# gnlpfjh/Scalable-E3-GNN

Hardware: AMD Instinct MI355X
Metric: particles/sec (octree build + SEGNN fwd), 1M pts l_max=2, 1/2/4/8 MI355X (higher is better)
Workload: dtype f32; 1 GPU; 1000000 particles/GPU uniform in unit box, radius graph k~24 (E=23519616), SEGNN l_max=2 4 layers H=32 f32 storage; particles_per_gpu=1000000, edges_per_gpu=23519616, hidden=32, layers=4, lmax=2, parallelism=single GPU

## Files before the change

include/e3gnn.h:

```cpp
#ifndef E3GNN_H
#define E3GNN_H

#include <stdint.h>

#ifdef __cplusplus
extern "C" {
#endif

#define E3GNN_ABI_VERSION 3

enum {
  E3_OK = 0,
  E3_ERR_INVALID_ARG = 1,
  E3_ERR_BAD_IRREPS = 2,
  E3_ERR_MISSING_WEIGHT = 3,
  E3_ERR_UNSUPPORTED = 4,
  E3_ERR_HIP = 5,
  E3_ERR_NO_DEVICE = 6
};

enum { E3_F32 = 0, E3_F64 = 1, E3_BF16 = 2 };

enum { E3_CLS_0E = 0, E3_CLS_0O = 1, E3_CLS_1E = 2, E3_CLS_1O = 3 };

typedef struct e3_l1tp_plan e3_l1tp_plan;

int         e3_abi_version(void);
const char* e3_status_string(int status);
const char* e3_last_hip_error(void);

int e3_l1tp_plan_create(const int32_t* in1_blocks, int n_in1,
                        const int32_t* out_blocks, int n_out,
                        e3_l1tp_plan** plan);
int e3_l1tp_plan_destroy(e3_l1tp_plan* plan);

int e3_l1tp_in1_dim(const e3_l1tp_plan* plan);
int e3_l1tp_out_dim(const e3_l1tp_plan* plan);
int e3_l1tp_weight_shape(const e3_l1tp_plan* plan, int cls, int* rows, int* cols);
int e3_l1tp_norm_len(const e3_l1tp_plan* plan, int cls);

int64_t e3_l1tp_packed_bytes(const e3_l1tp_plan* plan, int dtype);
int e3_l1tp_pack_weights(const e3_l1tp_plan* plan,
                         const void* const weights[4], const void* const norms[4],
                         int dtype, void* packed, void* stream);

int e3_l1tp_forward(const e3_l1tp_plan* plan,
                    const void* in1, int64_t ld_in1,
                    const void* in2, int64_t ld_in2,
                    const void* packed,
                    void* out, int64_t ld_out,
                    int64_t B, int dtype, int kernel, void* stream);

int64_t e3_l1tp_backward_workspace_bytes(const e3_l1tp_plan* plan, int64_t B, int dtype);
int e3_l1tp_backward(const e3_l1tp_plan* plan,
                     const void* in1, int64_t ld_in1,
                     const void* in2, int64_t ld_in2,
                     const void* const weights[4], const void* const norms[4],
                     const void* grad_out, int64_t ld_gout,
                     void* grad_in1, int64_t ld_gin1,
                     void* grad_in2,
                     void* const grad_weights[4],
                     void* workspace,
                     int64_t B, int dtype, void* stream);

typedef struct e3_rg_params {
  float lo[3], hi[3];
  float r;
  int32_t n[3];
  float inv[3];
  int32_t bits;
} e3_rg_params;

int     e3_rg_grid(e3_rg_params* prm);
int64_t e3_rg_workspace_bytes(int64_t N, const e3_rg_params* prm);
int e3_rg_sort_count(const float* pos, int64_t N, const e3_rg_params* prm,
                     int32_t* perm, float* sorted_pos4, int32_t* rowptr,
                     void* workspace, int64_t workspace_bytes, void* stream);
int e3_rg_fill(int64_t N, const e3_rg_params* prm, const float* sorted_pos4, const int32_t* rowptr,
               int32_t* src, void* workspace, int64_t workspace_bytes, void* stream);

int e3_rg_sort_count_pbc(const float* pos, int64_t N, const e3_rg_params* prm, int32_t periodic,
                         int32_t* perm, float* sorted_pos4, int32_t* rowptr,
                         void* workspace, int64_t workspace_bytes, void* stream);
int e3_rg_fill_pbc(int64_t N, const e3_rg_params* prm, int32_t periodic, const float* sorted_pos4,
                   const int32_t* rowptr, int32_t* src, void* workspace, int64_t workspace_bytes, void* stream);

int e3_cell_derive(const float cell[9], float ginv[9], float heights[3], float* volume);
int e3_rg_sort_count_cell(const float* pos, int64_t N, const e3_rg_params* prm, const float cell[9], const float origin[3],
                          int32_t* perm, float* sorted_pos4, int32_t* rowptr,
                          void* workspace, int64_t workspace_bytes, void* stream);
int e3_rg_fill_cell(int64_t N, const e3_rg_params* prm, const float cell[9], const float origin[3],
                    const float* sorted_pos4, const int32_t* rowptr, int32_t* src,
                    void* workspace, int64_t workspace_bytes, void* stream);

int e3_edge_geometry(const float* pos4, const int32_t* rowptr, const int32_t* src, int64_t N,
                     float* edge_y, float* edge_d, float* node_a, void* stream);
int e3_edge_geometry_pbc(const float* pos4, const int32_t* rowptr, const int32_t* src, int64_t N, const float box[3],
                         float* edge_y, float* edge_d, float* node_a, void* stream);
int e3_edge_geometry_cell(const float* pos4, const int32_t* rowptr, const int32_t* src, int64_t N, const float cell[9],
                          float* edge_y, float* edge_d, float* node_a, void* stream);
int e3_gather_concat(const float* h, int64_t ld_h, int D, const int32_t* rowptr, const int32_t* src, int64_t N,
                     const float* extra, int n_extra, float* out, int64_t ld_out, void* stream);
int e3_gate(const float* in, int64_t ld_in, float* out, int64_t ld_out, int64_t B, int ns, int nv, void* stream);
int e3_segment_sum(const float* msg, int64_t ld_msg, const int32_t* rowptr, int64_t N, int D,
                   float* agg, int64_t ld_agg, void* stream);

int64_t e3_split_edges_workspace_bytes(int64_t N);
int e3_split_edges(const int32_t* rowptr, const int32_t* src, const uint8_t* is_ghost, int64_t N, int64_t E,
                   int32_t* rowptr_kept, int32_t* src_kept, int32_t* dst_kept, int32_t* src_interior, int32_t* dst_interior,
                   int32_t* src_boundary, int32_t* dst_boundary, int32_t* counts, void* workspace, void* stream);

#define E3_HALO_MAX_ENTRIES 26
typedef struct e3_halo_entry {
  float lo[3], hi[3], shift[3];
} e3_halo_entry;
int64_t e3_halo_select_workspace_bytes(int64_t n, int n_entries);
int e3_halo_select_count(const float* pos, int64_t n, const float lo[3], const float hi[3], int32_t periodic, float r,
                         const e3_halo_entry* entries, int n_entries, float* pos_wrapped, int32_t* counts, void* workspace,
                         int64_t workspace_bytes, void* stream);
int e3_halo_select_fill(const float* pos_wrapped, int64_t n, const float lo[3], const float hi[3], int32_t periodic, float r,
                        const e3_halo_entry* entries, int n_entries, int64_t total, int32_t* idx, float* ghost_pos,
                        void* workspace, int64_t workspace_bytes, void* stream);

#define E3_MORTON_MAX_RANKS 64
int e3_morton_keys(const float* pos, int64_t n, const float lo[3], const float hi[3], const int32_t n_cells[3], int32_t* keys,
                   void* stream);
int64_t e3_morton_select_workspace_bytes(int64_t n, int n_ranks);
int e3_morton_select_count(const float* pos, int64_t n, const float lo[3], const float hi[3], const int32_t n_cells[3], float r,
                           const int32_t* splitters, int n_ranks, int self_rank, int32_t* counts, void* workspace,
                           int64_t workspace_bytes, void* stream);
int e3_morton_select_fill(const float* pos, int64_t n, const float lo[3], const float hi[3], const int32_t n_cells[3], float r,
                          const int32_t* splitters, int n_ranks, int self_rank, int64_t total, int32_t* idx, void* workspace,
                          int64_t workspace_bytes, void* stream);

typedef struct e3_tp_plan e3_tp_plan;
typedef struct e3_tp_segment {
  const void* base;
  int64_t ld;
  const int32_t* row_index;
  int32_t ncols;
  int32_t reserved;
} e3_tp_segment;
int e3_tp_plan_create(const int32_t* in1_blocks, int n_in1, int lmax_sh,
                      const int32_t* out_blocks, int n_out, e3_tp_plan** plan);
int e3_tp_plan_destroy(e3_tp_plan* plan);
int e3_tp_in1_dim(const e3_tp_plan* plan);
int e3_tp_in2_dim(const e3_tp_plan* plan);
int e3_tp_out_dim(const e3_tp_plan* plan);
int e3_tp_weight_shape(const e3_tp_plan* plan, int cls, int* rows, int* cols);
int e3_tp_norm_len(const e3_tp_plan* plan, int cls);
int64_t e3_tp_packed_bytes(const e3_tp_plan* plan, int dtype);
int e3_tp_pack_weights(const e3_tp_plan* plan, const void* const weights[6], const void* const norms[6],
                       int dtype, void* packed, void* stream);
int e3_tp_forward(const e3_tp_plan* plan, const void* in1, int64_t ld_in1, const void* in2, int64_t ld_in2,
                  const void* packed, void* out, int64_t ld_out, int64_t B, int dtype, const float* in_scale,
                  int exact, void* stream);
int e3_pow2_scale(const e3_tp_segment* segs, const int64_t* nrows, int nseg, int target_log2, float* out4,
                  void* stream);
int e3_add_pow2_scale(const float* h, const float* u, float* out, int64_t n, int target_log2, float* out4,
                      void* stream);
int e3_tp_forward_fused(const e3_tp_plan* plan, const e3_tp_segment* segs, int nseg,
                        const void* in2, int64_t ld_in2, const void* packed, void* out, int64_t ld_out,
                        int64_t B, int dtype, int gate, const float* in_scale, void* stream);
int e3_tp_forward_fused_epilogue(const e3_tp_plan* plan, const e3_tp_segment* segs, int nseg, const void* in2,
                                 int64_t ld_in2, const void* packed, void* out, int64_t ld_out, int64_t B, int dtype,
                                 int gate, const float* in_scale, const void* residual, int64_t ld_residual,
                                 float* out_scale4, int target_log2, void* stream);
int e3_tp_forward_update_pair(const e3_tp_plan* plan1, const e3_tp_plan* plan2, const e3_tp_segment* segs, int nseg,
                              const void* in2, int64_t ld_in2, const void* packed1, const void* packed2,
                              const float* in_scale, const void* residual, int64_t ld_residual, void* out,
                              int64_t ld_out, int64_t B, int dtype, float* out_scale4, int target_log2, void* stream);
int e3_tp_backward(const e3_tp_plan* plan, const void* in1, int64_t ld_in1, const void* in2, int64_t ld_in2,
                   const void* packed, const void* grad_out, int64_t ld_gout, void* grad_in1, int64_t ld_gin1,
                   void* grad_in2, int64_t ld_gin2, void* const grad_weights[6], int64_t B, int dtype, void* stream);
int e3_tp_backward_weights(const e3_tp_plan* plan, const void* in1, int64_t ld_in1, const void* in2, int64_t ld_in2,
                           const void* packed, const void* grad_out, int64_t ld_gout, void* const grad_weights[6],
                           int64_t B, int dtype, void* stream);
int e3_tp_backward_operands(const e3_tp_plan* plan, const void* in1, int64_t ld_in1, const void* in2, int64_t ld_in2,
                            const void* packed, const void* grad_out, int64_t ld_gout, void* const features[6],
                            void* const gout[6], int64_t B, int dtype, void* stream);
int e3_tp_backward_contract(const e3_tp_plan* plan, const void* in1, int64_t ld_in1, const void* in2, int64_t ld_in2,
                            void* const t[6], void* grad_in1, int64_t ld_gin1, void* grad_in2, int64_t ld_gin2,
                            int64_t B, int dtype, void* stream);
int e3_tp_fused_supported(const e3_tp_plan* plan, int gate);
const char* e3_tp_last_fused_kernel(void);
int e3_tp_forward_fused_scatter(const e3_tp_plan* plan, const e3_tp_segment* segs, int nseg,
                                const void* in2, int64_t ld_in2, const void* packed, const int32_t* row_node,
                                void* out_nodes, int64_t ld_out, int64_t B, int dtype, int gate,
                                const float* in_scale, void* stream);
typedef struct e3_msg_plan e3_msg_plan;
int e3_msg_plan_create(int lmax, int hidden, e3_msg_plan** plan);
int e3_msg_plan_destroy(e3_msg_plan* plan);
int64_t e3_msg_packed_bytes(const e3_msg_plan* plan);
int64_t e3_msg_premix_floats_per_node(const e3_msg_plan* plan);
int e3_msg_weight_shape(const e3_msg_plan* plan, int tp , int l3, int* rows, int* cols);
int e3_msg_supports(const e3_msg_plan* plan, int dtype);
int e3_msg_pack_weights(e3_msg_plan* plan, const void* const w1[3], const void* const n1[3],
                        const void* const w2[3], const void* const n2[3], int dtype, void* packed, void* stream);
int e3_msg_premix(e3_msg_plan* plan, const void* h, int64_t ld_h, int64_t N, const void* packed,
                  const float* in_scale, float* premix, int dtype, void* stream);
int e3_msg_forward(e3_msg_plan* plan, const void* h, int64_t ld_h, int64_t N, const float* pos4,
                   const int32_t* src, const int32_t* dst, int64_t E, const void* packed, const float* in_scale,
                   const float* premix, float* out, int64_t ld_out, int dtype, int accumulate, int tiles_per_block,
                   void* stream);
int e3_msg_forward_pbc(e3_msg_plan* plan, const void* h, int64_t ld_h, int64_t N, const float* pos4,
                       const int32_t* src, const int32_t* dst, int64_t E, const void* packed, const float* in_scale,
                       const float* premix, float* out, int64_t ld_out, int dtype, int accumulate, int tiles_per_block,
                       const float box[3], void* stream);
int e3_msg_forward_cell(e3_msg_plan* plan, const void* h, int64_t ld_h, int64_t N, const float* pos4,
                        const int32_t* src, const int32_t* dst, int64_t E, const void* packed, const float* in_scale,
                        const float* premix, float* out, int64_t ld_out, int dtype, int accumulate, int tiles_per_block,
                        const float cell[9], void* stream);
int e3_segment_sum_bf16(const void* msg, int64_t ld_msg, const int32_t* rowptr, int64_t N, int D,
                        void* agg, int64_t ld_agg, void* stream);
int e3_edge_geometry_l2(const float* pos4, const int32_t* rowptr, const int32_t* src, int64_t N,
                        float* edge_y, float* edge_d, float* node_a, void* stream);
int e3_edge_geometry_l2_pbc(const float* pos4, const int32_t* rowptr, const int32_t* src, int64_t N, const float box[3],
                            float* edge_y, float* edge_d, float* node_a, void* stream);
int e3_edge_geometry_l2_cell(const float* pos4, const int32_t* rowptr, const int32_t* src, int64_t N, const float cell[9],
                             float* edge_y, float* edge_d, float* node_a, void* stream);
int e3_gate_blocks(const float* in, int64_t ld_in, float* out, int64_t ld_out, int64_t B, int ns,
                   int nblocks, const int32_t* ls, const int32_t* muls, void* stream);

int e3_edge_geometry_backward(const float* pos4, const int32_t* rowptr, const int32_t* src, int64_t N, int lmax,
                              const float* g_edge_y, const float* g_edge_d, const float* g_node_a, float* g_pos,
                              void* stream);
int e3_edge_geometry_backward_pbc(const float* pos4, const int32_t* rowptr, const int32_t* src, int64_t N, int lmax,
                                  const float box[3], const float* g_edge_y, const float* g_edge_d,
                                  const float* g_node_a, float* g_pos, void* stream);
int e3_edge_geometry_backward_cell(const float* pos4, const int32_t* rowptr, const int32_t* src, int64_t N, int lmax,
                                   const float cell[9], const float* g_edge_y, const float* g_edge_d,
                                   const float* g_node_a, float* g_pos, void* stream);
int e3_gather_concat_backward(const float* g_out, int64_t ld_gout, int D, const int32_t* rowptr, const int32_t* src,
                              int64_t N, int n_extra, float* g_h, int64_t ld_gh, float* g_extra, void* stream);

int e3_edge_geometry_strained(const float* pos4, const int32_t* rowptr, const int32_t* src, int64_t N, int lmax,
                              const float* box, const float* strain, const int32_t* structure, int S, float* edge_y,
                              float* edge_d, float* node_a, void* stream);
int64_t e3_edge_geometry_backward_strained_workspace_bytes(int64_t N);
int e3_edge_geometry_backward_strained(const float* pos4, const int32_t* rowptr, const int32_t* src, int64_t N, int lmax,
                                       const float* box, const float* strain, const int32_t* structure, int S,
                                       const float* g_edge_y, const float* g_edge_d, const float* g_node_a, float* g_pos,
                                       float* g_strain, void* workspace, int64_t workspace_bytes, void* stream);
int e3_edge_geometry_strained_cell(const float* pos4, const int32_t* rowptr, const int32_t* src, int64_t N, int lmax,
                                   const float cell[9], const float* strain, const int32_t* structure, int S,
                                   float* edge_y, float* edge_d, float* node_a, void* stream);
int e3_edge_geometry_backward_strained_cell(const float* pos4, const int32_t* rowptr, const int32_t* src, int64_t N,
                                            int lmax, const float cell[9], const float* strain, const int32_t* structure,
                                            int S, const float* g_edge_y, const float* g_edge_d, const float* g_node_a,
                                            float* g_pos, float* g_strain, void* workspace, int64_t workspace_bytes,
                                            void* stream);
int e3_gate_blocks_backward(const float* in, int64_t ld_in, const float* g_out, int64_t ld_gout, float* g_in,
                            int64_t ld_gin, int64_t B, int ns, int nblocks, const int32_t* ls, const int32_t* muls,
                            void* stream);
int e3_segment_sum_backward(const float* g_agg, int64_t ld_gagg, const int32_t* rowptr, int64_t N, int D, float* g_msg,
                            int64_t ld_gmsg, void* stream);

int e3_cutoff_envelope(const float* edge_d, int64_t E, float r_c, int p, float* w, void* stream);
int e3_cutoff_envelope_backward(const float* edge_d, const float* g_w, int64_t E, float r_c, int p, float* g_d,
                                void* stream);
int e3_segment_sum_weighted(const float* msg, int64_t ld_msg, const float* w, const int32_t* rowptr, int64_t N, int D,
                            float* agg, int64_t ld_agg, void* stream);
int e3_segment_sum_weighted_backward(const float* g_agg, int64_t ld_gagg, const float* msg, int64_t ld_msg, const float* w,
                                     const int32_t* rowptr, int64_t N, int D, float* g_msg, int64_t ld_gmsg, float* g_w,
                                     void* stream);

int64_t e3_nl_workspace_bytes(int64_t N);
int e3_nl_update(const float* pos, const int32_t* perm, const float* ref_pos4, const int32_t* rowptr, const int32_t* src,
                 int64_t N, int64_t E, float r, float* pos4_out, int32_t* rowptr_out, int32_t* src_out, int32_t* dst_out,
                 uint32_t* stats, void* workspace, void* stream);
int e3_nl_update_pbc(const float* pos, const int32_t* perm, const float* ref_pos4, const int32_t* rowptr, const int32_t* src,
                     int64_t N, int64_t E, float r, const float box[3], float* pos4_out, int32_t* rowptr_out,
                     int32_t* src_out, int32_t* dst_out, uint32_t* stats, void* workspace, void* stream);
int e3_nl_update_cell(const float* pos, const int32_t* perm, const float* ref_pos4, const int32_t* rowptr, const int32_t* src,
                      int64_t N, int64_t E, float r, const float cell[9], float* pos4_out, int32_t* rowptr_out,
                      int32_t* src_out, int32_t* dst_out, uint32_t* stats, void* workspace, void* stream);

#ifdef __cplusplus
}
#endif
#endif
```

scalable-e3-gnn_amd/_lib.py:

```python
from __future__ import annotations

import ctypes
import os
from ctypes import POINTER, c_char_p, c_int, c_int32, c_int64, c_void_p

_HERE = os.path.dirname(os.path.abspath(__file__))
LIB_PATH = os.path.join(_HERE, "lib", "libe3gnn_hip.so")

E3_OK = 0
E3_F32, E3_F64, E3_BF16 = 0, 1, 2
CLS_NAMES = ("l0e", "l0o", "l1e", "l1o")

_lib = None

VoidP4 = c_void_p * 4
Float3 = ctypes.c_float * 3
Float9 = ctypes.c_float * 9
Int3 = c_int32 * 3


class HaloEntry(ctypes.Structure):
    _fields_ = [("lo", ctypes.c_float * 3), ("hi", ctypes.c_float * 3), ("shift", ctypes.c_float * 3)]


SIGNATURES = {
    "e3_abi_version": (c_int, []),
    "e3_status_string": (c_char_p, [c_int]),
    "e3_last_hip_error": (c_char_p, []),
    "e3_l1tp_plan_create": (c_int, [POINTER(c_int32), c_int, POINTER(c_int32), c_int, POINTER(c_void_p)]),
    "e3_l1tp_plan_destroy": (c_int, [c_void_p]),
    "e3_l1tp_in1_dim": (c_int, [c_void_p]),
    "e3_l1tp_out_dim": (c_int, [c_void_p]),
    "e3_l1tp_weight_shape": (c_int, [c_void_p, c_int, POINTER(c_int), POINTER(c_int)]),
    "e3_l1tp_norm_len": (c_int, [c_void_p, c_int]),
    "e3_l1tp_packed_bytes": (c_int64, [c_void_p, c_int]),
    "e3_l1tp_pack_weights": (c_int, [c_void_p, VoidP4, VoidP4, c_int, c_void_p, c_void_p]),
    "e3_l1tp_forward": (c_int, [c_void_p, c_void_p, c_int64, c_void_p, c_int64, c_void_p, c_void_p, c_int64,
                                c_int64, c_int, c_int, c_void_p]),
    "e3_l1tp_backward_workspace_bytes": (c_int64, [c_void_p, c_int64, c_int]),
    "e3_rg_grid": (c_int, [c_void_p]),
    "e3_rg_workspace_bytes": (c_int64, [c_int64, c_void_p]),
    "e3_rg_sort_count": (c_int, [c_void_p, c_int64, c_void_p, c_void_p, c_void_p, c_void_p, c_void_p, c_int64,
                                 c_void_p]),
    "e3_rg_fill": (c_int, [c_int64, c_void_p, c_void_p, c_void_p, c_void_p, c_void_p, c_int64, c_void_p]),
    "e3_edge_geometry": (c_int, [c_void_p, c_void_p, c_void_p, c_int64, c_void_p, c_void_p, c_void_p, c_void_p]),
    "e3_gather_concat": (c_int, [c_void_p, c_int64, c_int, c_void_p, c_void_p, c_int64, c_void_p, c_int, c_void_p,
                                 c_int64, c_void_p]),
    "e3_gate": (c_int, [c_void_p, c_int64, c_void_p, c_int64, c_int64, c_int, c_int, c_void_p]),
    "e3_segment_sum": (c_int, [c_void_p, c_int64, c_void_p, c_int64, c_int, c_void_p, c_int64, c_void_p]),
    "e3_split_edges_workspace_bytes": (c_int64, [c_int64]),
    "e3_split_edges": (c_int, [c_void_p, c_void_p, c_void_p, c_int64, c_int64, c_void_p, c_void_p, c_void_p, c_void_p,
                               c_void_p, c_void_p, c_void_p, c_void_p, c_void_p, c_void_p]),
    "e3_halo_select_workspace_bytes": (c_int64, [c_int64, c_int]),
    "e3_halo_select_count": (c_int, [c_void_p, c_int64, Float3, Float3, c_int32, ctypes.c_float, c_void_p, c_int, c_void_p,
                                     c_void_p, c_void_p, c_int64, c_void_p]),
    "e3_halo_select_fill": (c_int, [c_void_p, c_int64, Float3, Float3, c_int32, ctypes.c_float, c_void_p, c_int, c_int64,
                                    c_void_p, c_void_p, c_void_p, c_int64, c_void_p]),
    "e3_morton_keys": (c_int, [c_void_p, c_int64, Float3, Float3, Int3, c_void_p, c_void_p]),
    "e3_morton_select_workspace_bytes": (c_int64, [c_int64, c_int]),
    "e3_morton_select_count": (c_int, [c_void_p, c_int64, Float3, Float3, Int3, ctypes.c_float, POINTER(c_int32), c_int,
                                       c_int, c_void_p, c_void_p, c_int64, c_void_p]),
    "e3_morton_select_fill": (c_int, [c_void_p, c_int64, Float3, Float3, Int3, ctypes.c_float, POINTER(c_int32), c_int,
                                      c_int, c_int64, c_void_p, c_void_p, c_int64, c_void_p]),
    "e3_tp_plan_create": (c_int, [POINTER(c_int32), c_int, c_int, POINTER(c_int32), c_int, POINTER(c_void_p)]),
    "e3_tp_plan_destroy": (c_int, [c_void_p]),
    "e3_tp_in1_dim": (c_int, [c_void_p]),
    "e3_tp_in2_dim": (c_int, [c_void_p]),
    "e3_tp_out_dim": (c_int, [c_void_p]),
    "e3_tp_weight_shape": (c_int, [c_void_p, c_int, POINTER(c_int), POINTER(c_int)]),
    "e3_tp_norm_len": (c_int, [c_void_p, c_int]),
    "e3_tp_packed_bytes": (c_int64, [c_void_p, c_int]),
    "e3_tp_pack_weights": (c_int, [c_void_p, c_void_p * 6, c_void_p * 6, c_int, c_void_p, c_void_p]),
    "e3_tp_forward": (c_int, [c_void_p, c_void_p, c_int64, c_void_p, c_int64, c_void_p, c_void_p, c_int64, c_int64,
                              c_int, c_void_p, c_int, c_void_p]),
    "e3_tp_forward_fused": (c_int, [c_void_p, c_void_p, c_int, c_void_p, c_int64, c_void_p, c_void_p, c_int64, c_int64,
                                    c_int, c_int, c_void_p, c_void_p]),
    "e3_msg_plan_create": (c_int, [c_int, c_int, POINTER(c_void_p)]),
    "e3_msg_plan_destroy": (c_int, [c_void_p]),
    "e3_msg_packed_bytes": (c_int64, [c_void_p]),
    "e3_msg_premix_floats_per_node": (c_int64, [c_void_p]),
    "e3_msg_weight_shape": (c_int, [c_void_p, c_int, c_int, POINTER(c_int), POINTER(c_int)]),
    "e3_msg_supports": (c_int, [c_void_p, c_int]),
    "e3_msg_pack_weights": (c_int, [c_void_p, c_void_p * 3, c_void_p * 3, c_void_p * 3, c_void_p * 3, c_int, c_void_p,
                                    c_void_p]),
    "e3_msg_premix": (c_int, [c_void_p, c_void_p, c_int64, c_int64, c_void_p, c_void_p, c_void_p, c_int, c_void_p]),
    "e3_msg_forward": (c_int, [c_void_p, c_void_p, c_int64, c_int64, c_void_p, c_void_p, c_void_p, c_int64, c_void_p,
                               c_void_p, c_void_p, c_void_p, c_int64, c_int, c_int, c_int, c_void_p]),
    "e3_edge_geometry_backward": (c_int, [c_void_p, c_void_p, c_void_p, c_int64, c_int, c_void_p, c_void_p, c_void_p,
                                          c_void_p, c_void_p]),
    "e3_rg_sort_count_pbc": (c_int, [c_void_p, c_int64, c_void_p, c_int32, c_void_p, c_void_p, c_void_p, c_void_p,
                                     c_int64, c_void_p]),
    "e3_rg_fill_pbc": (c_int, [c_int64, c_void_p, c_int32, c_void_p, c_void_p, c_void_p, c_void_p, c_int64, c_void_p]),
    "e3_edge_geometry_pbc": (c_int, [c_void_p, c_void_p, c_void_p, c_int64, Float3, c_void_p, c_void_p, c_void_p,
                                     c_void_p]),
    "e3_edge_geometry_l2_pbc": (c_int, [c_void_p, c_void_p, c_void_p, c_int64, Float3, c_void_p, c_void_p, c_void_p,
                                        c_void_p]),
    "e3_edge_geometry_backward_pbc": (c_int, [c_void_p, c_void_p, c_void_p, c_int64, c_int, Float3, c_void_p, c_void_p,
                                              c_void_p, c_void_p, c_void_p]),
    "e3_msg_forward_pbc": (c_int, [c_void_p, c_void_p, c_int64, c_int64, c_void_p, c_void_p, c_void_p, c_int64,
                                   c_void_p, c_void_p, c_void_p, c_void_p, c_int64, c_int, c_int, c_int, Float3,
                                   c_void_p]),
    "e3_cell_derive": (c_int, [Float9, Float9, Float3, POINTER(ctypes.c_float)]),
    "e3_rg_sort_count_cell": (c_int, [c_void_p, c_int64, c_void_p, Float9, Float3, c_void_p, c_void_p, c_void_p, c_void_p,
                                      c_int64, c_void_p]),
    "e3_rg_fill_cell": (c_int, [c_int64, c_void_p, Float9, Float3, c_void_p, c_void_p, c_void_p, c_void_p, c_int64,
                                c_void_p]),
    "e3_edge_geometry_cell": (c_int, [c_void_p, c_void_p, c_void_p, c_int64, Float9, c_void_p, c_void_p, c_void_p,
                                      c_void_p]),
    "e3_edge_geometry_l2_cell": (c_int, [c_void_p, c_void_p, c_void_p, c_int64, Float9, c_void_p, c_void_p, c_void_p,
                                         c_void_p]),
    "e3_edge_geometry_backward_cell": (c_int, [c_void_p, c_void_p, c_void_p, c_int64, c_int, Float9, c_void_p, c_void_p,
                                               c_void_p, c_void_p, c_void_p]),
    "e3_msg_forward_cell": (c_int, [c_void_p, c_void_p, c_int64, c_int64, c_void_p, c_void_p, c_void_p, c_int64,
                                    c_void_p, c_void_p, c_void_p, c_void_p, c_int64, c_int, c_int, c_int, Float9,
                                    c_void_p]),
    "e3_edge_geometry_strained_cell": (c_int, [c_void_p, c_void_p, c_void_p, c_int64, c_int, Float9, c_void_p, c_void_p,
                                               c_int, c_void_p, c_void_p, c_void_p, c_void_p]),
    "e3_edge_geometry_backward_strained_cell": (c_int, [c_void_p, c_void_p, c_void_p, c_int64, c_int, Float9, c_void_p,
                                                        c_void_p, c_int, c_void_p, c_void_p, c_void_p, c_void_p, c_void_p,
                                                        c_void_p, c_int64, c_void_p]),
    "e3_gather_concat_backward": (c_int, [c_void_p, c_int64, c_int, c_void_p, c_void_p, c_int64, c_int, c_void_p, c_int64,
                                          c_void_p, c_void_p]),
    "e3_gate_blocks_backward": (c_int, [c_void_p, c_int64, c_void_p, c_int64, c_void_p, c_int64, c_int64, c_int, c_int,
                                        POINTER(c_int32), POINTER(c_int32), c_void_p]),
    "e3_segment_sum_backward": (c_int, [c_void_p, c_int64, c_void_p, c_int64, c_int, c_void_p, c_int64, c_void_p]),
    "e3_pow2_scale": (c_int, [c_void_p, POINTER(c_int64), c_int, c_int, c_void_p, c_void_p]),
    "e3_add_pow2_scale": (c_int, [c_void_p, c_void_p, c_void_p, c_int64, c_int, c_void_p, c_void_p]),
    "e3_tp_backward": (c_int, [c_void_p, c_void_p, c_int64, c_void_p, c_int64, c_void_p, c_void_p, c_int64, c_void_p,
                               c_int64, c_void_p, c_int64, c_void_p * 6, c_int64, c_int, c_void_p]),
    "e3_tp_backward_weights": (c_int, [c_void_p, c_void_p, c_int64, c_void_p, c_int64, c_void_p, c_void_p, c_int64, c_void_p,
                                       c_int64, c_int, c_void_p]),
    "e3_tp_backward_operands": (c_int, [c_void_p, c_void_p, c_int64, c_void_p, c_int64, c_void_p, c_void_p, c_int64, c_void_p,
                                        c_void_p, c_int64, c_int, c_void_p]),
    "e3_tp_backward_contract": (c_int, [c_void_p, c_void_p, c_int64, c_void_p, c_int64, c_void_p, c_void_p, c_int64, c_void_p,
                                        c_int64, c_int64, c_int, c_void_p]),
    "e3_tp_forward_fused_epilogue": (c_int, [c_void_p, c_void_p, c_int, c_void_p, c_int64, c_void_p, c_void_p, c_int64,
                                             c_int64, c_int, c_int, c_void_p, c_void_p, c_int64, c_void_p, c_int, c_void_p]),
    "e3_tp_forward_update_pair": (c_int, [c_void_p, c_void_p, c_void_p, c_int, c_void_p, c_int64, c_void_p, c_void_p,
                                          c_void_p, c_void_p, c_int64, c_void_p, c_int64, c_int64, c_int, c_void_p, c_int,
                                          c_void_p]),
    "e3_tp_fused_supported": (c_int, [c_void_p, c_int]),
    "e3_tp_last_fused_kernel": (ctypes.c_char_p, []),
    "e3_tp_forward_fused_scatter": (c_int, [c_void_p, c_void_p, c_int, c_void_p, c_int64, c_void_p, c_void_p, c_void_p,
                                            c_int64, c_int64, c_int, c_int, c_void_p, c_void_p]),
    "e3_segment_sum_bf16": (c_int, [c_void_p, c_int64, c_void_p, c_int64, c_int, c_void_p, c_int64, c_void_p]),
    "e3_edge_geometry_l2": (c_int, [c_void_p, c_void_p, c_void_p, c_int64, c_void_p, c_void_p, c_void_p, c_void_p]),
    "e3_gate_blocks": (c_int, [c_void_p, c_int64, c_void_p, c_int64, c_int64, c_int, c_int, POINTER(c_int32),
                               POINTER(c_int32), c_void_p]),
    "e3_l1tp_backward": (c_int, [c_void_p, c_void_p, c_int64, c_void_p, c_int64, VoidP4, VoidP4, c_void_p, c_int64,
                                 c_void_p, c_int64, c_void_p, VoidP4, c_void_p, c_int64, c_int, c_void_p]),
    "e3_edge_geometry_strained": (c_int, [c_void_p, c_void_p, c_void_p, c_int64, c_int, POINTER(ctypes.c_float), c_void_p,
                                          c_void_p, c_int, c_void_p, c_void_p, c_void_p, c_void_p]),
    "e3_edge_geometry_backward_strained_workspace_bytes": (c_int64, [c_int64]),
    "e3_edge_geometry_backward_strained": (c_int, [c_void_p, c_void_p, c_void_p, c_int64, c_int, POINTER(ctypes.c_float),
                                                   c_void_p, c_void_p, c_int, c_void_p, c_void_p, c_void_p, c_void_p,
                                                   c_void_p, c_void_p, c_int64, c_void_p]),
    "e3_cutoff_envelope": (c_int, [c_void_p, c_int64, ctypes.c_float, c_int, c_void_p, c_void_p]),
    "e3_cutoff_envelope_backward": (c_int, [c_void_p, c_void_p, c_int64, ctypes.c_float, c_int, c_void_p, c_void_p]),
    "e3_segment_sum_weighted": (c_int, [c_void_p, c_int64, c_void_p, c_void_p, c_int64, c_int, c_void_p, c_int64,
                                        c_void_p]),
    "e3_segment_sum_weighted_backward": (c_int, [c_void_p, c_int64, c_void_p, c_int64, c_void_p, c_void_p, c_int64, c_int,
                                                 c_void_p, c_int64, c_void_p, c_void_p]),
    "e3_nl_workspace_bytes": (c_int64, [c_int64]),
    "e3_nl_update": (c_int, [c_void_p, c_void_p, c_void_p, c_void_p, c_void_p, c_int64, c_int64, ctypes.c_float, c_void_p,
                             c_void_p, c_void_p, c_void_p, c_void_p, c_void_p, c_void_p]),
    "e3_nl_update_pbc": (c_int, [c_void_p, c_void_p, c_void_p, c_void_p, c_void_p, c_int64, c_int64, ctypes.c_float, Float3,
                                 c_void_p, c_void_p, c_void_p, c_void_p, c_void_p, c_void_p, c_void_p]),
    "e3_nl_update_cell": (c_int, [c_void_p, c_void_p, c_void_p, c_void_p, c_void_p, c_int64, c_int64, ctypes.c_float, Float9,
                                  c_void_p, c_void_p, c_void_p, c_void_p, c_void_p, c_void_p, c_void_p]),
}


def load():
    global _lib
    if _lib is not None:
        return _lib
    if not os.path.exists(LIB_PATH):
        raise RuntimeError(
            f"{LIB_PATH} is missing: the HIP library has not been built. Run "
            "`python -c 'import __graft_entry__ as g; g.build()'` (or `make -C scalable-e3-gnn_amd/csrc`). "
            "There is no CPU fallback.")
    import torch

    lib = ctypes.CDLL(LIB_PATH)
    for name, (res, args) in SIGNATURES.items():
        fn = getattr(lib, name, None)
        if fn is None:
            continue
        fn.restype = res
        fn.argtypes = args
    _lib = lib
    return lib


def check(status: int, what: str = ""):
    if status != E3_OK:
        lib = load()
        msg = lib.e3_status_string(status).decode()
        if status == 5:
            msg += " — " + lib.e3_last_hip_error().decode()
        raise RuntimeError(f"libe3gnn_hip: {what}: {msg} (status {status})")


def blocks_array(blocks):
    flat = [int(v) for b in blocks for v in b]
    return (c_int32 * len(flat))(*flat), len(blocks)


def ptr4(tensors):
    return VoidP4(*[(t.data_ptr() if (t is not None and t.numel() > 0) else None) for t in tensors])


def dtype_code(dtype) -> int:
    import torch

    try:
        return {torch.float32: E3_F32, torch.float64: E3_F64, torch.bfloat16: E3_BF16}[dtype]
    except KeyError:
        raise RuntimeError(f"libe3gnn_hip supports float32 / float64 / bfloat16, got {dtype}") from None


class DevicePlans:

    def __init__(self, create_name: str, destroy_name: str, *args):
        self._create, self._destroy_name, self._args = create_name, destroy_name, args
        self._handles = {}

    def _make(self):
        lib = load()
        cargs = []
        for a in self._args:
            if isinstance(a, (list, tuple)):
                arr, n = blocks_array(a)
                cargs += [arr, n]
            else:
                cargs.append(int(a))
        h = c_void_p()
        check(getattr(lib, self._create)(*cargs, ctypes.byref(h)), self._create)
        return h

    def handle(self, device=None) -> c_void_p:
        key = -1
        if device is not None:
            import torch
            key = torch.device(device).index
            if key is None:
                key = torch.cuda.current_device()
        h = self._handles.get(key)
        if h is None:
            h = self._handles[key] = self._make()
        return h

    def __deepcopy__(self, memo):
        return DevicePlans(self._create, self._destroy_name, *self._args)

    def __reduce__(self):
        return (DevicePlans, (self._create, self._destroy_name) + tuple(self._args))

    def __del__(self):
        try:
            lib = load()
            for h in self._handles.values():
                if h:
                    getattr(lib, self._destroy_name)(h)
            self._handles = {}
        except Exception:
            pass
```

scalable-e3-gnn_amd/csrc/e3_msg_common.h:

```cpp
#pragma once

template <int LMAX, int TT>
struct MsgGeom {
  static constexpr int H = 16 * TT;
  static constexpr int KS = (H + 31) / 32;
  static constexpr int D = H * (LMAX + 1) * (LMAX + 1);
  static constexpr int T(int l3) { return l3 == 0 ? TT * (1 + LMAX) : TT; }
  static constexpr int col0(int l) { return H * l * l; }
  static constexpr bool ok(int l1, int l2, int l3) {
    return l1 >= 0 && l2 >= 0 && l3 >= 0 && l1 <= LMAX && l2 <= LMAX && l3 <= LMAX && ((l1 + l2 + l3) % 2 == 0) &&
           l3 >= (l1 > l2 ? l1 - l2 : l2 - l1) && l3 <= l1 + l2;
  }
  static constexpr int blk(int l1, int l2, int l3) {
    int n = 0;
    for (int a = 0; a <= LMAX; ++a)
      for (int c = 0; c <= LMAX; ++c)
        for (int b = 0; b <= LMAX; ++b) {
          if (a == l1 && b == l2 && c == l3) return n;
          if (ok(a, b, c)) n += KS * T(c);
        }
    return n;
  }
  static constexpr int nblk() { return blk(LMAX + 1, 0, 0); }
  static constexpr int uoff(int l1, int l2, int l3) {
    int n = 0;
    for (int a = 0; a <= LMAX; ++a)
      for (int c = 0; c <= LMAX; ++c)
        for (int b = 0; b <= LMAX; ++b) {
          if (a == l1 && b == l2 && c == l3) return n;
          if (ok(a, b, c)) n += (2 * a + 1) * T(c) * 16;
        }
    return n;
  }
  static constexpr int UD = uoff(LMAX + 1, 0, 0);
  static constexpr int slot0(int l3) { return l3 == 0 ? 0 : l3 == 1 ? T(0) : T(0) + 3 * TT; }
  static constexpr int NS = T(0) + 3 * TT + (LMAX == 2 ? 5 * TT : 0);
  static constexpr int wdoff(int l) { return l == 0 ? 0 : l == 1 ? T(0) * 16 : (T(0) + TT) * 16; }
  static constexpr int WD = (T(0) + LMAX * TT) * 16;
  static constexpr int o_norm1 = 64, o_norm2 = o_norm1 + NS * 16, o_wd = o_norm2 + NS * 16;
  static constexpr int o_w = (o_wd + WD + 63) / 64 * 64;
  static constexpr int blk_floats = 64 * 8;
  static constexpr int64_t total_floats = (int64_t)o_w + 3LL * nblk() * blk_floats;
  static constexpr int lds_tab = 2 * NS * 16 + WD;
  static constexpr int lds_wave = 16 * (D + 4);
};

__host__ __device__ constexpr int kperm(int g, int jj) { return 16 * (jj >> 2) + 4 * g + (jj & 3); }


template <int L1, int L2, int L3>
__device__ __forceinline__ void make_z(const float (&y)[9], float (&z)[2 * L1 + 1][2 * L3 + 1]) {
  using C = CG<L1, L2, L3>;
#pragma unroll
  for (int a = 0; a < 2 * L1 + 1; ++a)
#pragma unroll
    for (int c = 0; c < 2 * L3 + 1; ++c) {
      float s = 0.f;
      bool have = false;
#pragma unroll
      for (int b = 0; b < 2 * L2 + 1; ++b)
        if (C::v[a][b][c] != 0.0) {
          s = have ? __builtin_fmaf((float)C::v[a][b][c], y[L2 * L2 + b], s) : (float)C::v[a][b][c] * y[L2 * L2 + b];
          have = true;
        }
      z[a][c] = s;
    }
}
template <int L1, int L2, int L3>
__host__ __device__ constexpr bool z_nonzero(int a, int c) {
  for (int b = 0; b < 2 * L2 + 1; ++b)
    if (CG<L1, L2, L3>::v[a][b][c] != 0.0) return true;
  return false;
}

template <bool IO16>
__device__ __forceinline__ f32x4 mma3(const uint4 ah, const uint4 al, const uint4 bh, const uint4 bl, f32x4 c) {
  if constexpr (IO16) {
    return mfma16(__builtin_bit_cast(bf16x8, ah), __builtin_bit_cast(bf16x8, bh), c);
  } else {
    c = mfma16h(__builtin_bit_cast(f16x8, ah), __builtin_bit_cast(f16x8, bh), c);
    c = mfma16h(__builtin_bit_cast(f16x8, ah), __builtin_bit_cast(f16x8, bl), c);
    c = mfma16h(__builtin_bit_cast(f16x8, al), __builtin_bit_cast(f16x8, bh), c);
    return c;
  }
}

template <bool IO16>
__device__ __forceinline__ void split8(const float (&f)[8], uint4& bh, uint4& bl) {
  uint32_t ph[4], pl[4] = {0, 0, 0, 0};
#pragma unroll
  for (int q = 0; q < 4; ++q) {
    if constexpr (IO16) ph[q] = __builtin_bit_cast(uint32_t, __builtin_convertvector(f32x2_t{f[2 * q], f[2 * q + 1]}, bf16x2_t));
    else split2_f16(f[2 * q], f[2 * q + 1], ph[q], pl[q]);
  }
  bh = uint4{ph[0], ph[1], ph[2], ph[3]};
  bl = uint4{pl[0], pl[1], pl[2], pl[3]};
}

template <int PBC = kOpen>
__device__ __forceinline__ void edge_sh(const float4 ps, const float4 pd, float (&y)[9], float& dist,
                                        const typename PbcArg<PBC>::type& box = {}) {
  float rx, ry, rz;
  edge_rel<PBC>(ps, pd, box, rx, ry, rz);
  const float d = sqrtf(rx * rx + ry * ry + rz * rz);
  const float inv = d > 0.f ? 1.0f / d : 0.f;
  const float x = rx * inv, yy = ry * inv, z = rz * inv;
  constexpr float s3 = 1.7320508075688772f, s5 = 2.2360679774997896f;
  y[0] = 1.0f;
  y[1] = s3 * x; y[2] = s3 * yy; y[3] = s3 * z;
  y[4] = s5 * s3 * x * yy;
  y[5] = s5 * s3 * yy * z;
  y[6] = s5 * 0.5f * (2.f * z * z - x * x - yy * yy);
  y[7] = s5 * s3 * z * x;
  y[8] = s5 * 0.5f * s3 * (x * x - yy * yy);
  dist = d;
}
template <int PBC = kOpen>
__device__ __forceinline__ void edge_sh1(const float4 ps, const float4 pd, float (&y)[9], float& dist,
                                        const typename PbcArg<PBC>::type& box = {}) {
  float rx, ry, rz;
  edge_rel<PBC>(ps, pd, box, rx, ry, rz);
  const float d = sqrtf(rx * rx + ry * ry + rz * rz);
  const float s = d > 0.f ? 1.7320508075688772f / d : 0.f;
  y[0] = 1.0f; y[1] = s * rx; y[2] = s * ry; y[3] = s * rz;
#pragma unroll
  for (int q = 4; q < 9; ++q) y[q] = 0.f;
  dist = d;
}

template <int D1, bool IO16>
__device__ __forceinline__ void read_piece(const void* piece, const int p, const float xs, float (&x)[8][D1]) {
  float q[4 * D1];
  if constexpr (IO16) {
    const uint2* sp = reinterpret_cast<const uint2*>(piece);
#pragma unroll
    for (int u = 0; u < D1; ++u) {
      const uint2 v = sp[u];
      q[4 * u + 0] = __builtin_bit_cast(float, v.x << 16); q[4 * u + 1] = __builtin_bit_cast(float, v.x & 0xffff0000u);
      q[4 * u + 2] = __builtin_bit_cast(float, v.y << 16); q[4 * u + 3] = __builtin_bit_cast(float, v.y & 0xffff0000u);
    }
  } else {
    const float4* sp = reinterpret_cast<const float4*>(piece);
#pragma unroll
    for (int u = 0; u < D1; ++u) {
      const float4 v = sp[u];
      q[4 * u] = v.x * xs; q[4 * u + 1] = v.y * xs; q[4 * u + 2] = v.z * xs; q[4 * u + 3] = v.w * xs;
    }
  }
#pragma unroll
  for (int r = 0; r < 4; ++r)
#pragma unroll
    for (int a = 0; a < D1; ++a) x[4 * p + r][a] = q[r * D1 + a];
}
template <int D1>
__device__ __forceinline__ void zero_piece(const int p, float (&x)[8][D1]) {
#pragma unroll
  for (int r = 0; r < 4; ++r)
#pragma unroll
    for (int a = 0; a < D1; ++a) x[4 * p + r][a] = 0.f;
}
```

scalable-e3-gnn_amd/csrc/e3_msg_fused.hip:

```cpp
#include "e3_common.h"
#include "cg_tables.h"
#include "e3_msg_ws.h"

#include <algorithm>
#include <cstddef>
#include <mutex>
#include <type_traits>
#include <utility>
#include <vector>

#ifndef E3_MSG_WD
#define E3_MSG_WD 1
#endif
#ifndef E3_MSG_UDP
#define E3_MSG_UDP 1
#endif
#ifndef E3_MSG_WPS
#define E3_MSG_WPS 2
#endif

#ifndef E3_MSG_STAMP
#define E3_MSG_STAMP 0
#endif

namespace e3 {
#if E3_MSG_STAMP
__device__ unsigned long long g_msg_stamps[8];
#endif

#include "e3_tp_mfma_core.h"

#include "e3_msg_common.h"

struct MsgPackDesc {
  int role;
  int mat;
  int rowbase;
  int nvalid;
  int M, colbase;
  int blk;
};
struct MsgPackArgs {
  const void* w1[3];
  const void* w2[3];
  const void* n1[3];
  const void* n2[3];
  int64_t nw1[3], nw2[3];
  int rowd[3];
  int M0, H, LMAX, TT, NS, WD, o_norm1, o_norm2, o_wd, o_w, nblk;
};

__global__ void msg_absmax_kernel(MsgPackArgs a, uint32_t* hdr) {
  float m1 = 0.f, m2 = 0.f;
  for (int c = 0; c < 3; ++c) {
    for (int64_t i = blockIdx.x * (int64_t)blockDim.x + threadIdx.x; i < a.nw1[c]; i += (int64_t)gridDim.x * blockDim.x)
      m1 = fmax_finite(m1, static_cast<const float*>(a.w1[c])[i]);
    for (int64_t i = blockIdx.x * (int64_t)blockDim.x + threadIdx.x; i < a.nw2[c]; i += (int64_t)gridDim.x * blockDim.x)
      m2 = fmax_finite(m2, static_cast<const float*>(a.w2[c])[i]);
  }
  for (int o = 32; o > 0; o >>= 1) { m1 = fmaxf(m1, __shfl_xor(m1, o)); m2 = fmaxf(m2, __shfl_xor(m2, o)); }
  if ((threadIdx.x & 63) == 0) {
    if (m1 > 0.f) atomicMax(hdr + 0, __builtin_bit_cast(uint32_t, m1));
    if (m2 > 0.f) atomicMax(hdr + 3, __builtin_bit_cast(uint32_t, m2));
  }
}

template <typename T>
__global__ void msg_pack_kernel(MsgPackArgs a, const MsgPackDesc* desc, int ndesc, float* packed) {
  constexpr bool IO16 = std::is_same<T, bf16>::value;
  const uint32_t* hb = reinterpret_cast<const uint32_t*>(packed);
  const float sw1 = IO16 ? 1.0f : pow2_scale_from_bits(hb[0], 13), sw2 = IO16 ? 1.0f : pow2_scale_from_bits(hb[3], 13);
  auto rd = [](const void* p, int64_t i) { return to_acc(static_cast<const T*>(p)[i]); };
  for (int r = blockIdx.x; r < ndesc; r += gridDim.x) {
    const MsgPackDesc q = desc[r];
    const void* W = q.role == 1 ? a.w2[q.mat] : a.w1[q.mat];
    const float sw = q.role == 1 ? sw2 : sw1;
    uint16_t* dst = reinterpret_cast<uint16_t*>(packed + a.o_w + ((size_t)q.role * a.nblk + q.blk) * 512);
    for (int i = threadIdx.x; i < 512; i += blockDim.x) {
      const int lane = i >> 3, jj = i & 7, ch = lane & 15, g = lane >> 4;
      const int k = kperm(g, jj);
      float v = 0.f;
      if (k < q.nvalid && q.colbase + ch < q.M) v = rd(W, (int64_t)(q.rowbase + k) * q.M + q.colbase + ch) * sw;
      if constexpr (IO16) {
        dst[lane * 8 + jj] = __builtin_bit_cast(uint16_t, (__bf16)v);
        dst[512 + lane * 8 + jj] = 0;
      } else {
        const _Float16 hi = (_Float16)v;
        const _Float16 lo = (_Float16)(v - (float)hi);
        dst[lane * 8 + jj] = __builtin_bit_cast(uint16_t, hi);
        dst[512 + lane * 8 + jj] = __builtin_bit_cast(uint16_t, lo);
      }
    }
  }
  if (blockIdx.x == 0) {
    for (int i = threadIdx.x; i < a.NS * 16; i += blockDim.x) {
      const int s = i >> 4, ch = i & 15;
      const int T0 = a.TT * (1 + a.LMAX);
      int l3, t, c;
      if (s < T0) { l3 = 0; t = s; c = 0; }
      else if (s < T0 + 3 * a.TT) { l3 = 1; t = (s - T0) / 3; c = (s - T0) % 3; }
      else { l3 = 2; t = (s - T0 - 3 * a.TT) / 5; c = (s - T0 - 3 * a.TT) % 5; }
      const int idx = (16 * t + ch) * (2 * l3 + 1) + c;
      packed[a.o_norm1 + i] = (a.n1[l3] ? rd(a.n1[l3], idx) : 1.0f) / sw1;
      packed[a.o_norm2 + i] = (a.n2[l3] ? rd(a.n2[l3], idx) : 1.0f) / sw2;
    }
    for (int i = threadIdx.x; i < a.WD; i += blockDim.x) {
      const int T0 = a.TT * (1 + a.LMAX);
      int l, rem;
      if (i < T0 * 16) { l = 0; rem = i; }
      else if (i < (T0 + a.TT) * 16) { l = 1; rem = i - T0 * 16; }
      else { l = 2; rem = i - (T0 + a.TT) * 16; }
      const int M = l == 0 ? a.M0 : a.H;
      packed[a.o_wd + i] = rd(a.w1[l], (int64_t)a.rowd[l] * M + rem) * sw1;
    }
    if (threadIdx.x == 0) {
      packed[1] = sw1; packed[2] = 1.0f / sw1;
      packed[4] = sw2; packed[5] = 1.0f / sw2;
    }
    __shared__ uint32_t red[2];
    float bw = 0.f;
    for (int l = 0; l <= a.LMAX; ++l) {
      const int M = l == 0 ? a.M0 : a.H;
      const int rows = (int)(a.nw1[l] / M);
      if (threadIdx.x < 2) red[threadIdx.x] = 0u;
      __syncthreads();
      float cs = 0.f, nm = 0.f;
      for (int col = threadIdx.x; col < M; col += blockDim.x) {
        float sum = 0.f;
        for (int r = 0; r < rows; ++r) sum += fabsf(rd(a.w1[l], (int64_t)r * M + col));
        cs = fmaxf(cs, sum);
      }
      for (int i = threadIdx.x; i < M * (2 * l + 1); i += blockDim.x) nm = fmaxf(nm, a.n1[l] ? fabsf(rd(a.n1[l], i)) : 1.0f);
      if (cs > 0.f && cs < INFINITY) atomicMax(&red[0], __builtin_bit_cast(uint32_t, cs));
      if (nm > 0.f && nm < INFINITY) atomicMax(&red[1], __builtin_bit_cast(uint32_t, nm));
      __syncthreads();
      bw = fmaxf(bw, 5.0f * __builtin_bit_cast(float, red[0]) * __builtin_bit_cast(float, red[1]));
      __syncthreads();
    }
    if (threadIdx.x == 0) packed[6] = bw;
  }
}


typedef uint32_t u32x4 __attribute__((ext_vector_type(4)));
struct TpCtx {
  __amdgpu_buffer_rsrc_t w;
  uint32_t wrole;
  uint32_t woff;
  const float* ud;
  const float* wd;
  float dsc;
};

template <bool IO16>
__device__ __forceinline__ void load_w(const TpCtx& cx, const int blk, uint4& hi, uint4& lo) {
  const uint32_t so = cx.wrole + (uint32_t)blk * 2048u;
  const u32x4 h = __builtin_amdgcn_raw_buffer_load_b128(cx.w, cx.woff, so, 0);
  hi = uint4{h[0], h[1], h[2], h[3]};
  if constexpr (!IO16) {
    const u32x4 l = __builtin_amdgcn_raw_buffer_load_b128(cx.w, cx.woff + 1024u, so, 0);
    lo = uint4{l[0], l[1], l[2], l[3]};
  }
}

struct BlkDesc {
  int l1, l2, l3, t;
  bool ff;
  bool first_of_l1;
  bool first_of_path;
};
template <int LMAX, int TT>
struct BlkList {
  using G = MsgGeom<LMAX, TT>;
  static constexpr BlkDesc at(int idx) {
    int n = 0;
    for (int l1 = 0; l1 <= LMAX; ++l1) {
      bool first = true;
      for (int pass = 0; pass < 2; ++pass)
        for (int l3 = 0; l3 <= LMAX; ++l3)
          for (int l2 = 0; l2 <= LMAX; ++l2) {
            if (!G::ok(l1, l2, l3)) continue;
            const bool ff = l3 == 0 && l1 > 0;
            if (ff != (pass == 0)) continue;
            for (int t = 0; t < G::T(l3); ++t) {
              if (n == idx) return BlkDesc{l1, l2, l3, t, ff, first, t == 0};
              first = false;
              ++n;
            }
          }
    }
    return BlkDesc{-1, 0, 0, 0, false, false, false};
  }
  static constexpr int count() {
    int n = 0;
    while (at(n).l1 >= 0) ++n;
    return n;
  }
};

template <int KS>
struct TpState {
  uint4 xh[KS][5], xl[KS][5];
  uint4 fh[KS], fl[KS];
  float z[5][5];
  uint4 wh[E3_MSG_WD + 1][KS], wl[E3_MSG_WD + 1][KS];
  f32x4 uin[E3_MSG_UDP + 1][5];
};

template <int LMAX, int TT, bool IO16, int IDX>
__device__ __forceinline__ void tp_prefetch_w(const TpCtx& cx, uint4 (&wh)[MsgGeom<LMAX, TT>::KS],
                                              uint4 (&wl)[MsgGeom<LMAX, TT>::KS]) {
  using G = MsgGeom<LMAX, TT>;
  if constexpr (IDX < BlkList<LMAX, TT>::count()) {
    constexpr BlkDesc B = BlkList<LMAX, TT>::at(IDX);
    constexpr int T = G::T(B.l3), B0 = G::blk(B.l1, B.l2, B.l3);
#pragma unroll
    for (int ks = 0; ks < G::KS; ++ks) load_w<IO16>(cx, B0 + ks * T + B.t, wh[ks], wl[ks]);
  }
}
template <int LMAX, int TT, bool FIRST, int IDX>
__device__ __forceinline__ void tp_prefetch_u(const TpCtx& cx, f32x4 (&uin)[5]) {
  using G = MsgGeom<LMAX, TT>;
  if constexpr (FIRST && IDX < BlkList<LMAX, TT>::count()) {
    constexpr BlkDesc B = BlkList<LMAX, TT>::at(IDX);
    constexpr int T = G::T(B.l3), U0 = G::uoff(B.l1, B.l2, B.l3);
#pragma unroll
    for (int a = 0; a < 2 * B.l1 + 1; ++a) uin[a] = *reinterpret_cast<const f32x4*>(cx.ud + U0 + (a * T + B.t) * 16);
  }
}

template <int LMAX, int TT, bool FIRST, bool IO16, int IDX, class XLOAD>
__device__ __forceinline__ void tp_block(const TpCtx& cx, const float (&y)[9], XLOAD& xload,
                                         TpState<MsgGeom<LMAX, TT>::KS>& st, f32x4 (&acc0)[MsgGeom<LMAX, TT>::T(0)],
                                         f32x4 (&acc1)[TT][3], f32x4 (&acc2)[LMAX == 2 ? TT : 1][5]) {
  using G = MsgGeom<LMAX, TT>;
  using BL = BlkList<LMAX, TT>;
  constexpr int KS = G::KS;
  constexpr BlkDesc B = BL::at(IDX);
  constexpr int L1 = B.l1, L2 = B.l2, L3 = B.l3, t = B.t;
  constexpr int D1 = 2 * L1 + 1, D3 = 2 * L3 + 1;
  tp_prefetch_w<LMAX, TT, IO16, IDX + E3_MSG_WD>(cx, st.wh[(IDX + E3_MSG_WD) % (E3_MSG_WD + 1)], st.wl[(IDX + E3_MSG_WD) % (E3_MSG_WD + 1)]);
  tp_prefetch_u<LMAX, TT, FIRST, IDX + E3_MSG_UDP>(cx, st.uin[(IDX + E3_MSG_UDP) % (E3_MSG_UDP + 1)]);
  const uint4 (&wh)[KS] = st.wh[IDX % (E3_MSG_WD + 1)];
  const uint4 (&wl)[KS] = st.wl[IDX % (E3_MSG_WD + 1)];
  const f32x4 (&uin)[5] = st.uin[IDX % (E3_MSG_UDP + 1)];
  if constexpr (B.first_of_l1) {
    float x[KS][8][D1];
#pragma unroll
    for (int ks = 0; ks < KS; ++ks) xload(std::integral_constant<int, L1>{}, ks, x[ks]);
    if constexpr (L1 > 0 && G::ok(L1, L1, 0)) {
      float zz[D1][1];
      make_z<L1, L1, 0>(y, zz);
#pragma unroll
      for (int a = 0; a < D1; ++a) st.z[a][0] = zz[a][0];
#pragma unroll
      for (int ks = 0; ks < KS; ++ks) {
        float f[8];
#pragma unroll
        for (int i = 0; i < 8; ++i) {
          float sum = zz[0][0] * x[ks][i][0];
#pragma unroll
          for (int a = 1; a < D1; ++a) sum = __builtin_fmaf(zz[a][0], x[ks][i][a], sum);
          f[i] = sum;
        }
        split8<IO16>(f, st.fh[ks], st.fl[ks]);
      }
    }
#pragma unroll
    for (int ks = 0; ks < KS; ++ks)
#pragma unroll
      for (int a = 0; a < D1; ++a) {
        float f[8];
#pragma unroll
        for (int i = 0; i < 8; ++i) f[i] = x[ks][i][a];
        split8<IO16>(f, st.xh[ks][a], st.xl[ks][a]);
      }
  }
  if constexpr (B.first_of_path && !B.ff) {
    float zz[D1][D3];
    make_z<L1, L2, L3>(y, zz);
#pragma unroll
    for (int a = 0; a < D1; ++a)
#pragma unroll
      for (int c = 0; c < D3; ++c) st.z[a][c] = zz[a][c];
  }
  if constexpr (B.ff) {
    f32x4 o = acc0[t];
#pragma unroll
    for (int ks = 0; ks < KS; ++ks) o = mma3<IO16>(wh[ks], wl[ks], st.fh[ks], st.fl[ks], o);
    if constexpr (FIRST) {
#pragma unroll
      for (int a = 0; a < D1; ++a)
#pragma unroll
        for (int r = 0; r < 4; ++r) o[r] = __builtin_fmaf(uin[a][r], st.z[a][0], o[r]);
    }
    acc0[t] = o;
  } else {
    f32x4 u[D1];
#pragma unroll
    for (int a = 0; a < D1; ++a) {
      if constexpr (FIRST) u[a] = uin[a];
      else u[a] = f32x4{0.f, 0.f, 0.f, 0.f};
    }
    if constexpr (FIRST && L1 == 0) {
      const f32x4 wdv = *reinterpret_cast<const f32x4*>(cx.wd + G::wdoff(L3) + t * 16);
#pragma unroll
      for (int r = 0; r < 4; ++r) u[0][r] = __builtin_fmaf(wdv[r], cx.dsc, u[0][r]);
    }
#pragma unroll
    for (int ks = 0; ks < KS; ++ks)
#pragma unroll
      for (int a = 0; a < D1; ++a) u[a] = mma3<IO16>(wh[ks], wl[ks], st.xh[ks][a], st.xl[ks][a], u[a]);
#pragma unroll
    for (int c = 0; c < D3; ++c)
#pragma unroll
      for (int a = 0; a < D1; ++a)
        if (z_nonzero<L1, L2, L3>(a, c)) {
#pragma unroll
          for (int r = 0; r < 4; ++r) {
            if constexpr (L3 == 0) acc0[t][r] = __builtin_fmaf(u[a][r], st.z[a][c], acc0[t][r]);
            else if constexpr (L3 == 1) acc1[t][c][r] = __builtin_fmaf(u[a][r], st.z[a][c], acc1[t][c][r]);
            else acc2[t][c][r] = __builtin_fmaf(u[a][r], st.z[a][c], acc2[t][c][r]);
          }
        }
  }
  if constexpr (IDX + 1 < BL::count())
    tp_block<LMAX, TT, FIRST, IO16, IDX + 1>(cx, y, xload, st, acc0, acc1, acc2);
}

template <int LMAX, int TT, bool FIRST, bool IO16, class XLOAD>
__device__ __forceinline__ void tp_core(const TpCtx& cx, const float (&y)[9], XLOAD&& xload,
                                        f32x4 (&acc0)[MsgGeom<LMAX, TT>::T(0)], f32x4 (&acc1)[TT][3],
                                        f32x4 (&acc2)[LMAX == 2 ? TT : 1][5]) {
  constexpr int KS = MsgGeom<LMAX, TT>::KS;
  TpState<KS> st;
  auto prime = [&](auto itag) {
    constexpr int I = decltype(itag)::value;
    if constexpr (I < E3_MSG_WD) tp_prefetch_w<LMAX, TT, IO16, I>(cx, st.wh[I % (E3_MSG_WD + 1)], st.wl[I % (E3_MSG_WD + 1)]);
    if constexpr (I < E3_MSG_UDP) tp_prefetch_u<LMAX, TT, FIRST, I>(cx, st.uin[I % (E3_MSG_UDP + 1)]);
  };
  prime(std::integral_constant<int, 0>{}); prime(std::integral_constant<int, 1>{});
  prime(std::integral_constant<int, 2>{}); prime(std::integral_constant<int, 3>{});
  static_assert(E3_MSG_WD <= 4 && E3_MSG_UDP <= 4, "ring prologue");
  tp_block<LMAX, TT, FIRST, IO16, 0>(cx, y, xload, st, acc0, acc1, acc2);
}


template <int LMAX, int TT, bool IO16>
__global__ __launch_bounds__(256) void msg_premix_kernel(const void* __restrict__ hv, int64_t ldh, int64_t N,
                                                         const float* __restrict__ packed,
                                                         const float* __restrict__ in_scale, float* __restrict__ U,
                                                         float* __restrict__ hmax) {
  using G = MsgGeom<LMAX, TT>;
  constexpr int ES = IO16 ? 2 : 4;
  const int lane = threadIdx.x & 63, j = lane & 15, g = lane >> 4;
  const int64_t wave0 = (blockIdx.x * (int64_t)blockDim.x + threadIdx.x) >> 6;
  const int64_t nw = ((int64_t)gridDim.x * blockDim.x) >> 6;
  const float xs = (!IO16 && in_scale) ? in_scale[0] : 1.0f;
  constexpr bool STAGE = G::KS == 1;
  __shared__ __align__(16) float stage_all[STAGE ? 4 * 16 * (6 * 16 + 4) : 4];
  float* stage = stage_all + (STAGE ? ((threadIdx.x >> 6) * 16 * (6 * 16 + 4)) : 0);
  TpCtx cx;
  cx.w = __builtin_amdgcn_make_buffer_rsrc(const_cast<float*>(packed + G::o_w), 0, 3 * G::nblk() * 2048, 0x00020000);
  cx.wrole = 2 * G::nblk() * 2048;
  cx.woff = lane * 16; cx.ud = nullptr; cx.wd = nullptr; cx.dsc = 0.f;
  const int64_t ntiles = (N + 15) / 16;
  for (int64_t tile = wave0; tile < ntiles; tile += nw) {
    const int64_t n = tile * 16 + j;
    const bool ok = n < N;
    const char* row = reinterpret_cast<const char*>(hv) + (ok ? n : N - 1) * ldh * ES;
    float* urow = U + (ok ? n : N - 1) * (int64_t)G::UD + 4 * g;
    float rowmax = 0.f;
    auto per_l1 = [&](auto l1tag) {
      constexpr int L1 = decltype(l1tag)::value, D1 = 2 * L1 + 1;
      uint4 xh[G::KS][D1], xl[G::KS][D1];
#pragma unroll
      for (int ks = 0; ks < G::KS; ++ks) {
        float x[8][D1];
#pragma unroll
        for (int p = 0; p < 2; ++p) {
          if (16 * (2 * ks + p) < G::H)
            read_piece<D1, IO16>(row + (G::col0(L1) + (32 * ks + 16 * p + 4 * g) * D1) * ES, p, xs, x);
          else
            zero_piece<D1>(p, x);
        }
#pragma unroll
        for (int i = 0; i < 8; ++i)
#pragma unroll
          for (int aa = 0; aa < D1; ++aa) rowmax = fmaxf(rowmax, fabsf(x[i][aa]));
#pragma unroll
        for (int a = 0; a < D1; ++a) {
          float f[8];
#pragma unroll
          for (int i = 0; i < 8; ++i) f[i] = x[i][a];
          split8<IO16>(f, xh[ks][a], xl[ks][a]);
        }
      }
      auto per_path = [&](auto l2tag, auto l3tag) {
        constexpr int L2 = decltype(l2tag)::value, L3 = decltype(l3tag)::value;
        if constexpr (G::ok(L1, L2, L3)) {
          constexpr int T = G::T(L3), B0 = G::blk(L1, L2, L3), U0 = G::uoff(L1, L2, L3);
          if constexpr (STAGE) {
            uint4 wh[T][G::KS], wl[T][G::KS];
#pragma unroll
            for (int t = 0; t < T; ++t)
#pragma unroll
              for (int ks = 0; ks < G::KS; ++ks) load_w<IO16>(cx, B0 + ks * T + t, wh[t][ks], wl[t][ks]);
            constexpr int RSP = T * 16 + 4, UPR = T * 4;
#pragma unroll
            for (int a = 0; a < D1; ++a) {
#pragma unroll
              for (int t = 0; t < T; ++t) {
                f32x4 u = f32x4{0.f, 0.f, 0.f, 0.f};
#pragma unroll
                for (int ks = 0; ks < G::KS; ++ks) u = mma3<IO16>(wh[t][ks], wl[t][ks], xh[ks][a], xl[ks][a], u);
                *reinterpret_cast<f32x4*>(stage + j * RSP + t * 16 + 4 * g) = u;
              }
              wave_sync_lds();
#pragma unroll
              for (int it = 0; it < (16 * UPR + 63) / 64; ++it) {
                const int unit = it * 64 + lane, row = unit / UPR, col = unit - row * UPR;
                const int64_t nn = tile * 16 + row;
                if (unit < 16 * UPR && nn < N)
                  *reinterpret_cast<f32x4*>(U + nn * (int64_t)G::UD + U0 + a * T * 16 + col * 4) =
                      *reinterpret_cast<const f32x4*>(stage + row * RSP + col * 4);
              }
              wave_sync_lds();
            }
          } else {
#pragma unroll
            for (int t = 0; t < T; ++t) {
              f32x4 u[D1];
#pragma unroll
              for (int a = 0; a < D1; ++a) u[a] = f32x4{0.f, 0.f, 0.f, 0.f};
#pragma unroll
              for (int ks = 0; ks < G::KS; ++ks) {
                uint4 ah, al;
                load_w<IO16>(cx, B0 + ks * T + t, ah, al);
#pragma unroll
                for (int a = 0; a < D1; ++a) u[a] = mma3<IO16>(ah, al, xh[ks][a], xl[ks][a], u[a]);
              }
              if (ok) {
#pragma unroll
                for (int a = 0; a < D1; ++a) *reinterpret_cast<f32x4*>(urow + U0 + (a * T + t) * 16) = u[a];
              }
            }
          }
        }
      };
      using I0 = std::integral_constant<int, 0>;
      using I1 = std::integral_constant<int, 1>;
      using I2 = std::integral_constant<int, 2>;
      per_path(I0{}, I0{}); per_path(I1{}, I0{}); per_path(I2{}, I0{});
      per_path(I0{}, I1{}); per_path(I1{}, I1{}); per_path(I2{}, I1{});
      per_path(I0{}, I2{}); per_path(I1{}, I2{}); per_path(I2{}, I2{});
    };
    per_l1(std::integral_constant<int, 0>{});
    per_l1(std::integral_constant<int, 1>{});
    if constexpr (LMAX == 2) per_l1(std::integral_constant<int, 2>{});
    rowmax = fmaxf(rowmax, __shfl_xor(rowmax, 16));
    rowmax = fmaxf(rowmax, __shfl_xor(rowmax, 32));
    if (hmax && ok && lane < 16) hmax[n] = rowmax;
  }
}

constexpr int msg_waves_per_simd(int lmax, int tt) {
  return (lmax == 2 ? 44 : 20) * tt <= 96 ? ((lmax == 2 && tt == 2) ? E3_MSG_WPS : 2) : 1;
}

struct MsgFusedKernarg {
  const void* hv; int64_t ldh; const float4* pos4; const int32_t *src, *dst; int64_t E; const float *packed, *U, *in_scale;
  float* out; int64_t ldo; int blk;
  PbcCell cell;
};
template <int LMAX, int TT, bool IO16, int PBC>
__global__ __launch_bounds__(256, msg_waves_per_simd(LMAX, TT))
__attribute__((amdgpu_waves_per_eu(msg_waves_per_simd(LMAX, TT), msg_waves_per_simd(LMAX, TT)))) void msg_fused_kernel(
    const void* __restrict__ hv, int64_t ldh, const float4* __restrict__ pos4, const int32_t* __restrict__ src,
    const int32_t* __restrict__ dst, int64_t E, const float* __restrict__ packed, const float* __restrict__ U,
    const float* __restrict__ in_scale, float* __restrict__ out, int64_t ldo, int blk,
    const typename PbcArg<PBC>::type box) {
  using G = MsgGeom<LMAX, TT>;
  constexpr int H = G::H, D = G::D, T0 = G::T(0), NS = G::NS;
  extern __shared__ __align__(16) unsigned char smem_raw[];
  float* lds = reinterpret_cast<float*>(smem_raw);
  const int tid = threadIdx.x, lane = tid & 63;
  const int wave = __builtin_amdgcn_readfirstlane(tid >> 6);

  float* n1tab = lds;
  float* n2tab = n1tab + NS * 16;
  float* wdtab = n2tab + NS * 16;
  float* wbuf = wdtab + G::WD + (size_t)wave * G::lds_wave;
  int* idbuf = reinterpret_cast<int*>(wdtab + G::WD + (size_t)4 * G::lds_wave) + wave * 64;
  constexpr int ES = IO16 ? 2 : 4;
  const char* h = reinterpret_cast<const char*>(hv);
  const float xs = (!IO16 && in_scale) ? in_scale[0] : 1.0f, ixs = (!IO16 && in_scale) ? in_scale[1] : 1.0f;
  for (int i = tid; i < NS * 16; i += blockDim.x) {
    n1tab[i] = packed[G::o_norm1 + i] * ixs;
    n2tab[i] = packed[G::o_norm2 + i];
  }
  for (int i = tid; i < G::WD; i += blockDim.x) wdtab[i] = packed[G::o_wd + i];
  __syncthreads();

  const __amdgpu_buffer_rsrc_t wrsrc = __builtin_amdgcn_make_buffer_rsrc(
      const_cast<float*>(packed + G::o_w), 0, 3 * G::nblk() * 2048, 0x00020000);

  const int ntiles = (int)((E + 15) / 16);
  const int per_xcd = (int)(gridDim.x >> 3);
  const int tiles_per_xcd = (ntiles + 7) / 8;
  const int xcd_lo = (int)(blockIdx.x & 7) * tiles_per_xcd;
  const int xcd_hi = xcd_lo + tiles_per_xcd < ntiles ? xcd_lo + tiles_per_xcd : ntiles;
  const int wg_idx = (int)(blockIdx.x >> 3);
  const int Ei = (int)E;

  constexpr int NQ = (D + 63) / 64;
  constexpr int RS = D + 4;
#if E3_MSG_STAMP
  uint32_t st_acc[8] = {0, 0, 0, 0, 0, 0, 0, 0}, st_t = (uint32_t)__builtin_readcyclecounter();
#define E3_STAMP(i) { const uint32_t t_ = (uint32_t)__builtin_readcyclecounter(); st_acc[i] += t_ - st_t; st_t = t_; }
#else
#define E3_STAMP(i)
#endif
  int cur = -1;
  float carry[NQ];
#pragma unroll
  for (int q = 0; q < NQ; ++q) carry[q] = 0.f;
  auto flush = [&]() {
    if (cur >= 0) {
      int ln;
      asm volatile("v_mbcnt_lo_u32_b32 %0, -1, 0\n\tv_mbcnt_hi_u32_b32 %0, -1, %0" : "=v"(ln));
      float* o = out + (int64_t)cur * ldo;
#pragma unroll
      for (int q = 0; q < NQ; ++q)
        if (64 * q + ln < D) __builtin_amdgcn_global_atomic_fadd_f32(o + (64 * q + ln), carry[q]);
    }
#pragma unroll
    for (int q = 0; q < NQ; ++q) carry[q] = 0.f;
  };

  auto copy_ids = [&](int tile, int ln) {
    const int row0 = __builtin_amdgcn_readfirstlane(tile * 16);
    const int nrows = __builtin_amdgcn_readfirstlane(Ei - row0 < 16 ? Ei - row0 : 16);
    const int jl = ln & 15;
    const int e = row0 + (jl < nrows ? jl : nrows - 1);
    if (ln < 16) __builtin_amdgcn_global_load_lds((glb_void_t*)(src + e), (lds_void_t*)idbuf, 4, 0, 0);
    else if (ln < 32) __builtin_amdgcn_global_load_lds((glb_void_t*)(dst + e), (lds_void_t*)idbuf, 4, 0, 0);
  };
  const int chunk = 4 * blk;
  const int n_outer = (tiles_per_xcd + chunk * per_xcd - 1) / (chunk * per_xcd);
  for (int ob = 0; ob < n_outer; ++ob) {
    const int b0 = __builtin_amdgcn_readfirstlane(xcd_lo + (ob * per_xcd + wg_idx) * chunk + wave * blk);
    const int b1 = __builtin_amdgcn_readfirstlane(b0 + blk < xcd_hi ? b0 + blk : xcd_hi);
    if (b0 < b1) {
      asm volatile("s_waitcnt lgkmcnt(0)" ::: "memory");
      wave_sync_lds();
      copy_ids(b0, lane);
      wait_vm0();
      wave_sync_lds();
    }
    for (int tile = b0; tile < b1; ++tile) {
      const int row0 = __builtin_amdgcn_readfirstlane(tile * 16);
      const int nrows = __builtin_amdgcn_readfirstlane(Ei - row0 < 16 ? Ei - row0 : 16);
      int lt;
      asm volatile("v_mbcnt_lo_u32_b32 %0, -1, 0\n\tv_mbcnt_hi_u32_b32 %0, -1, %0" : "=v"(lt));
      const int sid = idbuf[lt & 15], did = idbuf[16 + (lt & 15)];
      uint32_t woff = lt * 16;
      int tab0 = 0;
      asm volatile("" : "+v"(woff), "+v"(tab0));
      const float *n1p = n1tab + tab0, *n2p = n2tab + tab0, *wdp = wdtab + tab0;
      const int sd = (lt & 15) < nrows ? did : -1;

      asm volatile("s_waitcnt lgkmcnt(0)" ::: "memory");
      wave_sync_lds();
      E3_STAMP(5)
      {
        int ls;
        asm volatile("v_mbcnt_lo_u32_b32 %0, -1, 0\n\tv_mbcnt_hi_u32_b32 %0, -1, %0" : "=v"(ls));
        auto stage_region = [&](auto utag, auto otag, char* dstb) {
          constexpr int UNITS = decltype(utag)::value, SRCOFF = decltype(otag)::value;
          if constexpr (UNITS >= 64) {
#pragma unroll
            for (int r = 0; r < 16; ++r) {
              const int rid = __builtin_amdgcn_readlane(sid, r);
              const char* rowp = h + ((int64_t)rid * ldh + SRCOFF) * ES;
#pragma unroll
              for (int k = 0; k < UNITS / 64; ++k)
                __builtin_amdgcn_global_load_lds((glb_void_t*)(rowp + (k * 64 + ls) * 16),
                                                 (lds_void_t*)(dstb + (r * UNITS + k * 64) * 16), 16, 0, 0);
            }
          } else {
            constexpr int RPI = 64 / UNITS;
            static_assert(RPI <= 16, "region rows shorter than 4 units are not supported");
            const int u = ls & (UNITS - 1), rl = ls / UNITS;
            int rid[16 / RPI];
#pragma unroll
            for (int it = 0; it < 16 / RPI; ++it) rid[it] = __shfl(sid, it * RPI + rl);
#pragma unroll
            for (int it = 0; it < 16 / RPI; ++it)
              __builtin_amdgcn_global_load_lds((glb_void_t*)(h + ((int64_t)rid[it] * ldh + SRCOFF) * ES + u * 16),
                                               (lds_void_t*)(dstb + it * 1024), 16, 0, 0);
          }
        };
        char* wb = reinterpret_cast<char*>(wbuf);
        if (tile + 1 < b1) copy_ids(tile + 1, ls);
        if constexpr (LMAX == 2) {
          stage_region(std::integral_constant<int, 8 * H * ES / 16>{}, std::integral_constant<int, H>{}, wb);
          stage_region(std::integral_constant<int, H * ES / 16>{}, std::integral_constant<int, 0>{}, wb + 16 * 8 * H * ES);
        } else {
          stage_region(std::integral_constant<int, 4 * H * ES / 16>{}, std::integral_constant<int, 0>{}, wb);
        }
      }
      float y[9], dist;
      {
        const float4 ps = pos4[sid], pd = pos4[did];
        if constexpr (PBC == kCell) {
          typedef const __attribute__((address_space(4))) char* karg_ptr_t;
          const karg_ptr_t ka = (karg_ptr_t)__builtin_amdgcn_kernarg_segment_ptr();
          int off = offsetof(MsgFusedKernarg, cell);
          asm volatile("" : "+s"(off));
          const __attribute__((address_space(4))) float* cp = (const __attribute__((address_space(4))) float*)(ka + off);
          PbcCell c;
#pragma unroll
          for (int k = 0; k < 9; ++k) {
            c.h[k] = cp[k];
            c.g[k] = cp[9 + k];
          }
          if constexpr (LMAX == 2) edge_sh<PBC>(ps, pd, y, dist, c); else edge_sh1<PBC>(ps, pd, y, dist, c);
        } else {
          if constexpr (LMAX == 2) edge_sh<PBC>(ps, pd, y, dist, box); else edge_sh1<PBC>(ps, pd, y, dist, box);
        }
      }
      f32x4 a0[T0], a1[TT][3], a2[LMAX == 2 ? TT : 1][5];
      const f32x4 zero4 = {0.f, 0.f, 0.f, 0.f};
#pragma unroll
      for (int t = 0; t < T0; ++t) a0[t] = zero4;
#pragma unroll
      for (int t = 0; t < TT; ++t)
#pragma unroll
        for (int c = 0; c < 3; ++c) a1[t][c] = zero4;
#pragma unroll
      for (int t = 0; t < (LMAX == 2 ? TT : 1); ++t)
#pragma unroll
        for (int c = 0; c < 5; ++c) a2[t][c] = zero4;

      E3_STAMP(0)
      wait_vm0();
      wave_sync_lds();
      E3_STAMP(1)

      {
        int LL;
        asm volatile("v_mbcnt_lo_u32_b32 %0, -1, 0\n\tv_mbcnt_hi_u32_b32 %0, -1, %0" : "=v"(LL));
        const int j = LL & 15, g = LL >> 4;
        TpCtx cx;
        cx.w = wrsrc;
        cx.wrole = 0;
        cx.woff = woff;
        cx.ud = U + (int64_t)did * G::UD + 4 * g;
        cx.wd = wdp + 4 * g;
        cx.dsc = dist * xs;
        auto xload = [&](auto l1tag, int ks, auto& x) {
          constexpr int L1 = decltype(l1tag)::value, D1 = 2 * L1 + 1;
          const int e0 = LMAX == 2 ? (L1 == 0 ? 16 * 8 * H + j * H : j * 8 * H + (L1 == 1 ? 0 : 3 * H))
                                   : j * 4 * H + (L1 == 0 ? 0 : H);
          const char* xrow = reinterpret_cast<const char*>(wbuf) + e0 * ES;
#pragma unroll
          for (int p = 0; p < 2; ++p) {
            if (16 * (2 * ks + p) < H) read_piece<D1, IO16>(xrow + (32 * ks + 16 * p + 4 * g) * D1 * ES, p, xs, x);
            else zero_piece<D1>(p, x);
          }
        };
        tp_core<LMAX, TT, true, IO16>(cx, y, xload, a0, a1, a2);
      }

      E3_STAMP(2)
      float amax = 0.f;
      {
        int LL;
        asm volatile("v_mbcnt_lo_u32_b32 %0, -1, 0\n\tv_mbcnt_hi_u32_b32 %0, -1, %0" : "=v"(LL));
        const int g = LL >> 4;
        const f32x4* nt = reinterpret_cast<const f32x4*>(n1p) + g;
        auto gate_block = [&](auto dtag, auto& acc, const int slot, const int gslot) {
          constexpr int Dc = decltype(dtag)::value;
#pragma unroll
          for (int t = 0; t < TT; ++t) {
            const f32x4 gn = nt[4 * (gslot + t)];
            float gt[4];
#pragma unroll
            for (int r = 0; r < 4; ++r) gt[r] = sigmoid_(a0[gslot + t][r] * gn[r]);
#pragma unroll
            for (int c = 0; c < Dc; ++c) {
              const f32x4 nv = nt[4 * (slot + Dc * t + c)];
#pragma unroll
              for (int r = 0; r < 4; ++r) {
                const float v = acc[t][c][r] * nv[r] * gt[r];
                acc[t][c][r] = v;
                amax = fmaxf(amax, fabsf(v));
              }
            }
          }
        };
#pragma unroll
        for (int t = 0; t < TT; ++t) {
          const f32x4 nv = nt[4 * t];
#pragma unroll
          for (int r = 0; r < 4; ++r) {
            const float sv = a0[t][r] * nv[r];
            const float v = sv * sigmoid_(sv);
            a0[t][r] = v;
            amax = fmaxf(amax, fabsf(v));
          }
        }
        gate_block(std::integral_constant<int, 3>{}, a1, G::slot0(1), TT);
        if constexpr (LMAX == 2) gate_block(std::integral_constant<int, 5>{}, a2, G::slot0(2), 2 * TT);
      }
      float srow = 1.0f, isrow = 1.0f;
      if constexpr (!IO16) {
        amax = fmaxf(amax, __shfl_xor(amax, 16));
        amax = fmaxf(amax, __shfl_xor(amax, 32));
        srow = pow2_scale_from_bits(__builtin_bit_cast(uint32_t, amax), 10);
        isrow = 1.0f / srow;
      }

      wave_sync_lds();
      {
        int LL;
        asm volatile("v_mbcnt_lo_u32_b32 %0, -1, 0\n\tv_mbcnt_hi_u32_b32 %0, -1, %0" : "=v"(LL));
        f32x4* pk = reinterpret_cast<f32x4*>(wbuf) + LL;
        auto sc4 = [&](const f32x4 v) {
          if constexpr (IO16) {
            f32x4 o;
            for (int r = 0; r < 4; ++r) o[r] = (float)(__bf16)v[r];
            return o;
          } else {
            return f32x4{v[0] * srow, v[1] * srow, v[2] * srow, v[3] * srow};
          }
        };
#pragma unroll
        for (int t = 0; t < TT; ++t) pk[64 * t] = sc4(a0[t]);
#pragma unroll
        for (int t = 0; t < TT; ++t)
#pragma unroll
          for (int c = 0; c < 3; ++c) pk[64 * (TT + 3 * t + c)] = sc4(a1[t][c]);
        if constexpr (LMAX == 2) {
#pragma unroll
          for (int t = 0; t < TT; ++t)
#pragma unroll
            for (int c = 0; c < 5; ++c) pk[64 * (4 * TT + 5 * t + c)] = sc4(a2[t][c]);
        }
      }
      wave_sync_lds();

      E3_STAMP(3)
#pragma unroll
      for (int t = 0; t < T0; ++t) a0[t] = zero4;
#pragma unroll
      for (int t = 0; t < TT; ++t)
#pragma unroll
        for (int c = 0; c < 3; ++c) a1[t][c] = zero4;
#pragma unroll
      for (int t = 0; t < (LMAX == 2 ? TT : 1); ++t)
#pragma unroll
        for (int c = 0; c < 5; ++c) a2[t][c] = zero4;
      {
        TpCtx cx;
        cx.w = wrsrc; cx.wrole = G::nblk() * 2048; cx.woff = woff; cx.ud = nullptr; cx.wd = nullptr; cx.dsc = 0.f;
        int LL;
        asm volatile("v_mbcnt_lo_u32_b32 %0, -1, 0\n\tv_mbcnt_hi_u32_b32 %0, -1, %0" : "=v"(LL));
        const f32x4* pk = reinterpret_cast<const f32x4*>(wbuf) + LL;
        auto xload = [&](auto l1tag, int ks, auto& x) {
          constexpr int L1 = decltype(l1tag)::value, D1 = 2 * L1 + 1;
          constexpr int S0 = L1 == 0 ? 0 : L1 == 1 ? TT : 4 * TT;
#pragma unroll
          for (int p = 0; p < 2; ++p) {
            const int t = 2 * ks + p;
#pragma unroll
            for (int a = 0; a < D1; ++a) {
              f32x4 v = zero4;
              if (t < TT) v = pk[64 * (S0 + D1 * t + a)];
#pragma unroll
              for (int r = 0; r < 4; ++r) x[4 * p + r][a] = v[r];
            }
          }
        };
        tp_core<LMAX, TT, false, IO16>(cx, y, xload, a0, a1, a2);
      }

      E3_STAMP(4)
      {
        int LL;
        asm volatile("v_mbcnt_lo_u32_b32 %0, -1, 0\n\tv_mbcnt_hi_u32_b32 %0, -1, %0" : "=v"(LL));
        const int j = LL & 15, g = LL >> 4;
        const f32x4* nt2 = reinterpret_cast<const f32x4*>(n2p) + g;
        wave_sync_lds();
        float* wp = wbuf + j * RS + 4 * g;
#pragma unroll
        for (int t = 0; t < TT; ++t) {
          const f32x4 nv = nt2[4 * t];
          f32x4 o;
#pragma unroll
          for (int r = 0; r < 4; ++r) {
            const float sv = a0[t][r] * nv[r] * isrow;
            o[r] = sv * sigmoid_(sv);
          }
          *reinterpret_cast<f32x4*>(wp + 16 * t) = o;
        }
        auto put_block = [&](auto dtag, auto& acc, const int slot, const int gslot, float* wq) {
          constexpr int Dc = decltype(dtag)::value;
#pragma unroll
          for (int t = 0; t < TT; ++t) {
            const f32x4 gn = nt2[4 * (gslot + t)];
            float gt[4];
#pragma unroll
            for (int r = 0; r < 4; ++r) gt[r] = sigmoid_(a0[gslot + t][r] * gn[r] * isrow) * isrow;
            float o[4 * Dc];
#pragma unroll
            for (int c = 0; c < Dc; ++c) {
              const f32x4 nv = nt2[4 * (slot + Dc * t + c)];
#pragma unroll
              for (int r = 0; r < 4; ++r) o[r * Dc + c] = acc[t][c][r] * nv[r] * gt[r];
            }
            f32x4* dq = reinterpret_cast<f32x4*>(wq + 16 * t * Dc);
#pragma unroll
            for (int k = 0; k < Dc; ++k) dq[k] = f32x4{o[4 * k], o[4 * k + 1], o[4 * k + 2], o[4 * k + 3]};
          }
        };
        put_block(std::integral_constant<int, 3>{}, a1, G::slot0(1), TT, wbuf + j * RS + H + 12 * g);
        if constexpr (LMAX == 2) put_block(std::integral_constant<int, 5>{}, a2, G::slot0(2), 2 * TT, wbuf + j * RS + 4 * H + 20 * g);
        wave_sync_lds();
        E3_STAMP(6)
        int ln;
        asm volatile("v_mbcnt_lo_u32_b32 %0, -1, 0\n\tv_mbcnt_hi_u32_b32 %0, -1, %0" : "=v"(ln));
        const float* sp = wbuf + ln;
#pragma unroll
        for (int rb = 0; rb < 16; rb += 4) {
          float v[4][NQ];
#pragma unroll
          for (int rr = 0; rr < 4; ++rr)
#pragma unroll
            for (int q = 0; q < NQ; ++q) v[rr][q] = (64 * q + ln < D) ? sp[(rb + rr) * RS + 64 * q] : 0.f;
#pragma unroll
          for (int rr = 0; rr < 4; ++rr) {
            const int dn = __builtin_amdgcn_readlane(sd, rb + rr);
            if (dn >= 0) {
              if (dn != cur) {
                flush();
                cur = dn;
              }
#pragma unroll
              for (int q = 0; q < NQ; ++q) carry[q] += v[rr][q];
            }
          }
        }
      }
      E3_STAMP(7)
    }
    flush();
    cur = -1;
  }
#if E3_MSG_STAMP
  if (lane == 0)
    for (int i = 0; i < 8; ++i) atomicAdd(&g_msg_stamps[i], (unsigned long long)st_acc[i]);
#endif
#undef E3_STAMP
}

static_assert(std::is_same_v<decltype(&msg_fused_kernel<1, 1, false, kCell>),
                             void (*)(decltype(MsgFusedKernarg::hv), decltype(MsgFusedKernarg::ldh), decltype(MsgFusedKernarg::pos4),
                                      decltype(MsgFusedKernarg::src), decltype(MsgFusedKernarg::dst), decltype(MsgFusedKernarg::E),
                                      decltype(MsgFusedKernarg::packed), decltype(MsgFusedKernarg::U),
                                      decltype(MsgFusedKernarg::in_scale), decltype(MsgFusedKernarg::out),
                                      decltype(MsgFusedKernarg::ldo), decltype(MsgFusedKernarg::blk),
                                      decltype(MsgFusedKernarg::cell))>,
              "MsgFusedKernarg must list the parameters of msg_fused_kernel in order");
static_assert(offsetof(MsgFusedKernarg, cell) == 92 && sizeof(PbcCell) == 72, "the cell follows `int blk` at byte 92");

struct MsgKernels {
  int lmax, tt;
  const void* fused[2];
  const void* fused_pbc[2];
  const void* fused_cell[2];
  const void* premix[2];
  int64_t total_floats;
  int UD, D, lds_tab, lds_wave, nblk, NS, WD, o_norm1, o_norm2, o_wd, o_w, waves_per_simd;
};
template <int LMAX, int TT>
static MsgKernels make_entry() {
  using G = MsgGeom<LMAX, TT>;
  MsgKernels k = {LMAX, TT, {(const void*)msg_fused_kernel<LMAX, TT, false, kOpen>, nullptr},
                  {(const void*)msg_fused_kernel<LMAX, TT, false, kBox>, nullptr},
                  {(const void*)msg_fused_kernel<LMAX, TT, false, kCell>, nullptr},
                  {(const void*)msg_premix_kernel<LMAX, TT, false>, nullptr}, G::total_floats,
                  G::UD, G::D, G::lds_tab, G::lds_wave, G::nblk(), G::NS, G::WD, G::o_norm1, G::o_norm2, G::o_wd, G::o_w,
                  msg_waves_per_simd(LMAX, TT)};
  if constexpr (TT >= 2) {
    k.fused[1] = (const void*)msg_fused_kernel<LMAX, TT, true, kOpen>;
    k.fused_pbc[1] = (const void*)msg_fused_kernel<LMAX, TT, true, kBox>;
    k.fused_cell[1] = (const void*)msg_fused_kernel<LMAX, TT, true, kCell>;
    k.premix[1] = (const void*)msg_premix_kernel<LMAX, TT, true>;
  }
  return k;
}
static const std::vector<MsgKernels>& msg_kernels() {
  static const std::vector<MsgKernels> k = {make_entry<2, 2>(), make_entry<1, 2>(), make_entry<2, 1>(), make_entry<1, 1>(),
                                            make_entry<2, 4>(), make_entry<1, 4>()};
  return k;
}

}

using namespace e3;

struct e3_msg_plan {
  int lmax, H;
  const MsgKernels* k;
  std::vector<MsgPackDesc> desc;
  int rowd[3];
  int K1[3], K2[3], M[3];
  MsgPackDesc* d_desc = nullptr;
  int device = -1;
  int grid[2] = {0, 0};
  int grid_pbc[2] = {0, 0};
  int grid_cell[2] = {0, 0};
  std::mutex mu;
};

static int msg_ensure_device(e3_msg_plan* P) {
  std::lock_guard<std::mutex> lock(P->mu);
  int cur = -1;
  if (hipGetDevice(&cur) != hipSuccess) return E3_ERR_NO_DEVICE;
  if (P->d_desc) return cur == P->device ? E3_OK : E3_ERR_INVALID_ARG;
  MsgPackDesc* d = nullptr;
  E3_HIP_CHECK(hipMalloc((void**)&d, P->desc.size() * sizeof(MsgPackDesc)));
  if (hipMemcpy(d, P->desc.data(), P->desc.size() * sizeof(MsgPackDesc), hipMemcpyHostToDevice) != hipSuccess) {
    (void)hipFree(d);
    return E3_ERR_HIP;
  }
  const size_t lds = (size_t)(P->k->lds_tab + 4 * P->k->lds_wave) * 4 + 4 * 256;
  int cus = 0;
  if (hipDeviceGetAttribute(&cus, hipDeviceAttributeMultiprocessorCount, cur) != hipSuccess || cus <= 0) cus = 256;
  for (int io = 0; io < 2; ++io) {
    if (!P->k->fused[io]) continue;
    for (int pb = 0; pb < 2; ++pb) {
      const void* kern = pb ? P->k->fused_pbc[io] : P->k->fused[io];
      int per_cu = 0;
      if (hipFuncSetAttribute(kern, hipFuncAttributeMaxDynamicSharedMemorySize, (int)lds) != hipSuccess ||
          hipOccupancyMaxActiveBlocksPerMultiprocessor(&per_cu, kern, 256, lds) != hipSuccess || per_cu < 1) {
        (void)hipFree(d);
        return E3_ERR_HIP;
      }
      (pb ? P->grid_pbc : P->grid)[io] = cus * (per_cu < 4 ? per_cu : 4);
    }
  }
  P->device = cur;
  P->d_desc = d;
  return E3_OK;
}

static int msg_ensure_cell(e3_msg_plan* P, int io) {
  std::lock_guard<std::mutex> lock(P->mu);
  if (P->grid_cell[io]) return E3_OK;
  const size_t lds = (size_t)(P->k->lds_tab + 4 * P->k->lds_wave) * 4 + 4 * 256;
  int cus = 0, per_cu = 0;
  if (hipDeviceGetAttribute(&cus, hipDeviceAttributeMultiprocessorCount, P->device) != hipSuccess || cus <= 0) cus = 256;
  const void* kern = P->k->fused_cell[io];
  if (!kern || hipFuncSetAttribute(kern, hipFuncAttributeMaxDynamicSharedMemorySize, (int)lds) != hipSuccess ||
      hipOccupancyMaxActiveBlocksPerMultiprocessor(&per_cu, kern, 256, lds) != hipSuccess || per_cu < 1)
    return E3_ERR_HIP;
  P->grid_cell[io] = cus * (per_cu < 4 ? per_cu : 4);
  return E3_OK;
}

extern "C" {

int e3_msg_plan_create(int lmax, int hidden, e3_msg_plan** plan_out) {
  if (!plan_out || lmax < 1 || lmax > 2) return E3_ERR_INVALID_ARG;
  const MsgKernels* k = nullptr;
  for (auto& e : msg_kernels())
    if (e.lmax == lmax && 16 * e.tt == hidden) k = &e;
  if (!k) return E3_ERR_UNSUPPORTED;
  auto* P = new e3_msg_plan();
  P->lmax = lmax; P->H = hidden; P->k = k;
  const int H = hidden, TT = k->tt, KS = (H + 31) / 32;
  auto ok = [&](int l1, int l2, int l3) {
    return l1 <= lmax && l2 <= lmax && l3 <= lmax && ((l1 + l2 + l3) % 2 == 0) && l3 >= std::abs(l1 - l2) && l3 <= l1 + l2;
  };
  auto T = [&](int l3) { return l3 == 0 ? TT * (1 + lmax) : TT; };
  const int n1[3] = {2 * H + 1, 2 * H, 2 * H}, n2[3] = {H, H, H};
  int wrow1[3][3][3], wrow2[3][3][3];
  for (int l3 = 0; l3 <= 2; ++l3) {
    int r1 = 0, r2 = 0;
    for (int l1 = 0; l1 <= 2; ++l1)
      for (int l2 = 0; l2 <= 2; ++l2) {
        wrow1[l1][l2][l3] = wrow2[l1][l2][l3] = -1;
        if (l3 > lmax || !ok(l1, l2, l3)) continue;
        wrow1[l1][l2][l3] = r1; r1 += n1[l1];
        wrow2[l1][l2][l3] = r2; r2 += n2[l1];
      }
    P->K1[l3] = l3 <= lmax ? r1 : 0;
    P->K2[l3] = l3 <= lmax ? r2 : 0;
    P->M[l3] = l3 <= lmax ? 16 * T(l3) : 0;
    P->rowd[l3] = (l3 <= lmax) ? wrow1[0][l3][l3] + 2 * H : 0;
  }
  int b = 0;
  for (int l1 = 0; l1 <= lmax; ++l1)
    for (int l3 = 0; l3 <= lmax; ++l3)
      for (int l2 = 0; l2 <= lmax; ++l2) {
        if (!ok(l1, l2, l3)) continue;
        for (int ks = 0; ks < KS; ++ks)
          for (int t = 0; t < T(l3); ++t) {
            const int nvalid = std::min(32, H - 32 * ks);
            const int M = 16 * T(l3);
            P->desc.push_back({0, l3, wrow1[l1][l2][l3] + H + 32 * ks, nvalid, M, 16 * t, b + ks * T(l3) + t});
            P->desc.push_back({2, l3, wrow1[l1][l2][l3] + 32 * ks, nvalid, M, 16 * t, b + ks * T(l3) + t});
            P->desc.push_back({1, l3, wrow2[l1][l2][l3] + 32 * ks, nvalid, M, 16 * t, b + ks * T(l3) + t});
          }
        b += KS * T(l3);
      }
  if (b != k->nblk) { delete P; return E3_ERR_INVALID_ARG; }
  *plan_out = P;
  return E3_OK;
}

int e3_msg_plan_destroy(e3_msg_plan* P) {
  if (!P) return E3_OK;
  if (P->d_desc) (void)hipFree(P->d_desc);
  delete P;
  return E3_OK;
}

int64_t e3_msg_packed_bytes(const e3_msg_plan* P) { return P ? (P->k->total_floats * 4 + 255) / 256 * 256 : -1; }
int64_t e3_msg_premix_floats_per_node(const e3_msg_plan* P) { return P ? P->k->UD + 1 : -1; }
int e3_msg_weight_shape(const e3_msg_plan* P, int tp, int l3, int* rows, int* cols) {
  if (!P || !rows || !cols || l3 < 0 || l3 > 2 || (tp != 1 && tp != 2)) return E3_ERR_INVALID_ARG;
  *rows = tp == 1 ? P->K1[l3] : P->K2[l3];
  *cols = P->M[l3];
  return E3_OK;
}

int e3_msg_supports(const e3_msg_plan* P, int dtype) {
  if (!P) return 0;
  return dtype == E3_F32 ? 1 : (dtype == E3_BF16 && P->k->fused[1] != nullptr) ? 1 : 0;
}

int e3_msg_pack_weights(e3_msg_plan* P, const void* const w1[3], const void* const n1[3], const void* const w2[3],
                        const void* const n2[3], int dtype, void* packed, void* stream) {
  if (!P || !w1 || !w2 || !packed) return E3_ERR_INVALID_ARG;
  if (!e3_msg_supports(P, dtype)) return E3_ERR_UNSUPPORTED;
  for (int l = 0; l <= P->lmax; ++l)
    if (!w1[l] || !w2[l]) return E3_ERR_MISSING_WEIGHT;
  int st = msg_ensure_device(P);
  if (st != E3_OK) return st;
  const MsgKernels& k = *P->k;
  MsgPackArgs a;
  for (int l = 0; l < 3; ++l) {
    const bool on = l <= P->lmax;
    a.w1[l] = on ? w1[l] : nullptr; a.w2[l] = on ? w2[l] : nullptr;
    a.n1[l] = (on && n1) ? n1[l] : nullptr; a.n2[l] = (on && n2) ? n2[l] : nullptr;
    a.nw1[l] = on ? (int64_t)P->K1[l] * P->M[l] : 0;
    a.nw2[l] = on ? (int64_t)P->K2[l] * P->M[l] : 0;
    a.rowd[l] = P->rowd[l];
  }
  a.M0 = P->M[0]; a.H = P->H; a.LMAX = P->lmax; a.TT = k.tt; a.NS = k.NS; a.WD = k.WD;
  a.o_norm1 = k.o_norm1; a.o_norm2 = k.o_norm2; a.o_wd = k.o_wd; a.o_w = k.o_w; a.nblk = k.nblk;
  hipStream_t s = (hipStream_t)stream;
  E3_HIP_CHECK(hipMemsetAsync(packed, 0, 256, s));
  const dim3 grid(std::min<int>((int)P->desc.size(), 512));
  if (dtype == E3_F32) {
    hipLaunchKernelGGL(msg_absmax_kernel, dim3(64), dim3(256), 0, s, a, (uint32_t*)packed);
    hipLaunchKernelGGL(msg_pack_kernel<float>, grid, dim3(256), 0, s, a, P->d_desc, (int)P->desc.size(), (float*)packed);
  } else {
    hipLaunchKernelGGL(msg_pack_kernel<bf16>, grid, dim3(256), 0, s, a, P->d_desc, (int)P->desc.size(), (float*)packed);
  }
  E3_HIP_CHECK(hipGetLastError());
  return E3_OK;
}

int e3_msg_premix(e3_msg_plan* P, const void* h, int64_t ld_h, int64_t N, const void* packed, const float* in_scale,
                  float* premix, int dtype, void* stream) {
  if (!P || N < 0) return E3_ERR_INVALID_ARG;
  if (!e3_msg_supports(P, dtype)) return E3_ERR_UNSUPPORTED;
  const MsgKernels& k = *P->k;
  const int io = dtype == E3_BF16 ? 1 : 0, es = io ? 2 : 4;
  if (N == 0) return E3_OK;
  if (!h || !packed || !premix || ld_h < k.D) return E3_ERR_INVALID_ARG;
  if ((ld_h * es & 15) || ((uintptr_t)h & 15) || ((uintptr_t)premix & 15)) return E3_ERR_INVALID_ARG;
  int st = msg_ensure_device(P);
  if (st != E3_OK) return st;
  const int64_t ntiles = (N + 15) / 16;
  const int grid = (int)std::min<int64_t>((ntiles + 3) / 4, 2048);
  float* hmax = premix + (size_t)N * k.UD;
  void* args[] = {&h, &ld_h, &N, &packed, &in_scale, &premix, &hmax};
  if (hipLaunchKernel(k.premix[io], dim3(grid), dim3(256), args, 0, (hipStream_t)stream) != hipSuccess) return E3_ERR_HIP;
  return E3_OK;
}

}

static int msg_forward(e3_msg_plan* P, const void* h, int64_t ld_h, int64_t N, const float* pos4, const int32_t* src,
                       const int32_t* dst, int64_t E, const void* packed, const float* in_scale, const float* premix,
                       float* out, int64_t ld_out, int dtype, int accumulate, int tiles_per_block, void* stream,
                       const float* box, const PbcCell* cell = nullptr) {
  if (!P || N < 0 || E < 0 || E > 0x7fffffffLL - 16) return E3_ERR_INVALID_ARG;
  if (!e3_msg_supports(P, dtype)) return E3_ERR_UNSUPPORTED;
  const MsgKernels& k = *P->k;
  const int io = dtype == E3_BF16 ? 1 : 0, es = io ? 2 : 4;
  if (N == 0) return E3_OK;
  if (!h || !pos4 || !packed || !premix || !out || ld_h < k.D || ld_out < k.D || (E > 0 && (!src || !dst)))
    return E3_ERR_INVALID_ARG;
  if ((ld_h * es & 15) || ((uintptr_t)h & 15) || ((uintptr_t)premix & 15)) return E3_ERR_INVALID_ARG;
  int st = msg_ensure_device(P);
  if (st != E3_OK) return st;
  hipStream_t s = (hipStream_t)stream;
  if (!accumulate) E3_HIP_CHECK(hipMemset2DAsync(out, (size_t)ld_out * 4, 0, (size_t)k.D * 4, (size_t)N, s));
  if (E == 0) return E3_OK;
  if (tiles_per_block >= 0 && msg_ws_supported(P->lmax, P->H, dtype)) {
    st = msg_ws_launch(P->lmax, P->H, dtype, h, ld_h, N, pos4, src, dst, E, packed, in_scale, premix, out, ld_out,
                       tiles_per_block > (1 << 20) ? (1 << 24) : tiles_per_block * 16, s, box, cell);
    if (st != E3_ERR_UNSUPPORTED) return st;
  }
  if (tiles_per_block < 0) tiles_per_block = -tiles_per_block;
  if (cell && (st = msg_ensure_cell(P, io)) != E3_OK) return st;
  const int64_t ntiles = (E + 15) / 16;
  int nwg = (cell ? P->grid_cell : (box ? P->grid_pbc : P->grid))[io];
  nwg = (int)std::min<int64_t>(nwg, (ntiles + 3) / 4);
  nwg = std::max(8, (nwg + 7) / 8 * 8);
  int blk = tiles_per_block > 0 ? tiles_per_block : 4;
  if (blk > (1 << 16)) blk = 1 << 16;
  const size_t lds = (size_t)(k.lds_tab + 4 * k.lds_wave) * 4 + 4 * 256;
  PbcBox pbox;
  if (!cell) pbox = make_box(box);
  void* args[] = {&h, &ld_h, &pos4, &src, &dst, &E, &packed, &premix, &in_scale, &out, &ld_out, &blk,
                  cell ? (void*)cell : (void*)&pbox};
  if (hipLaunchKernel(cell ? k.fused_cell[io] : (box ? k.fused_pbc[io] : k.fused[io]), dim3(nwg), dim3(256), args, lds,
                      s) != hipSuccess)
    return E3_ERR_HIP;
  return E3_OK;
}

extern "C" {

int e3_msg_forward(e3_msg_plan* P, const void* h, int64_t ld_h, int64_t N, const float* pos4, const int32_t* src,
                   const int32_t* dst, int64_t E, const void* packed, const float* in_scale, const float* premix,
                   float* out, int64_t ld_out, int dtype, int accumulate, int tiles_per_block, void* stream) {
  return msg_forward(P, h, ld_h, N, pos4, src, dst, E, packed, in_scale, premix, out, ld_out, dtype, accumulate,
                     tiles_per_block, stream, nullptr);
}

int e3_msg_forward_pbc(e3_msg_plan* P, const void* h, int64_t ld_h, int64_t N, const float* pos4, const int32_t* src,
                       const int32_t* dst, int64_t E, const void* packed, const float* in_scale, const float* premix,
                       float* out, int64_t ld_out, int dtype, int accumulate, int tiles_per_block, const float box[3],
                       void* stream) {
  if (!box_valid(box, 0.0f)) return E3_ERR_INVALID_ARG;
  return msg_forward(P, h, ld_h, N, pos4, src, dst, E, packed, in_scale, premix, out, ld_out, dtype, accumulate,
                     tiles_per_block, stream, box);
}

int e3_msg_forward_cell(e3_msg_plan* P, const void* h, int64_t ld_h, int64_t N, const float* pos4, const int32_t* src,
                        const int32_t* dst, int64_t E, const void* packed, const float* in_scale, const float* premix,
                        float* out, int64_t ld_out, int dtype, int accumulate, int tiles_per_block, const float cell[9],
                        void* stream) {
  PbcCell c;
  if (!make_cell(cell, 0.0f, &c)) return E3_ERR_INVALID_ARG;
  return msg_forward(P, h, ld_h, N, pos4, src, dst, E, packed, in_scale, premix, out, ld_out, dtype, accumulate,
                     tiles_per_block, stream, nullptr, &c);
}

#if E3_MSG_STAMP
int e3_msg_debug_stamps(unsigned long long* out8, int reset) {
  if (out8 && hipMemcpyFromSymbol(out8, HIP_SYMBOL(e3::g_msg_stamps), 64) != hipSuccess) return E3_ERR_HIP;
  if (reset) {
    unsigned long long z[8] = {0, 0, 0, 0, 0, 0, 0, 0};
    if (hipMemcpyToSymbol(HIP_SYMBOL(e3::g_msg_stamps), z, 64) != hipSuccess) return E3_ERR_HIP;
  }
  return E3_OK;
}
#endif
}
```

scalable-e3-gnn_amd/csrc/e3_msg_ws.h:

```cpp
#pragma once
#include <hip/hip_runtime.h>
#include <stdint.h>
namespace e3 {
struct PbcCell;
bool msg_ws_supported(int lmax, int hidden, int dtype);
int msg_ws_launch(int lmax, int hidden, int dtype, const void* h, int64_t ldh, int64_t N, const float* pos4, const int32_t* src,
                  const int32_t* dst, int64_t E, const void* packed, const float* in_scale, const float* premix, float* out,
                  int64_t ldo, int chunk_edges, hipStream_t stream, const float* box = nullptr,
                  const PbcCell* cell = nullptr);
}
```

scalable-e3-gnn_amd/csrc/e3_msg_ws.hip:

```cpp
#include "e3_common.h"
#include "cg_tables.h"
#include "e3_msg_ws.h"

#include <algorithm>
#include <type_traits>

#ifndef E3_WS_STAMP
#define E3_WS_STAMP 0
#endif

namespace e3 {
#include "e3_tp_mfma_core.h"
#include "e3_msg_common.h"

#if E3_WS_STAMP
__device__ unsigned long long g_ws_stamps[8][4];
__device__ unsigned long long g_ws_tp[8][8];
#define WS_TPMARK(i) { if (tpm) { const uint32_t t_ = (uint32_t)__builtin_readcyclecounter(); tpm[i] += t_ - tpm0; tpm0 = t_; } }
#else
#define WS_TPMARK(i)
#endif

template <int LMAX, int TT, bool IO16>
struct Ws {
  using G = MsgGeom<LMAX, TT>;
  static_assert(TT == 2 && (LMAX == 1 || LMAX == 2), "instantiated for H = 32, l_max = 1 / 2");
  static constexpr int H = G::H, D = G::D, NS = G::NS, UD = G::UD;
  static constexpr int ES = IO16 ? 2 : 4;
  static constexpr int NC = (LMAX + 1) * (LMAX + 1);
  static constexpr int NFR = NC + LMAX;
  static constexpr int FRB = IO16 ? 1024 : 2048;
  static constexpr int frag(int l, int a) { return l * l + a; }
  static constexpr int frag_ff(int l) { return NC + l - 1; }
  static constexpr int GA_ROW = (NC - 1) * H * ES;
  static constexpr int GA_STRIDE = GA_ROW + 16;
  static constexpr int GA_BYTES = 16 * GA_STRIDE;
  static constexpr int GB_ROW = H * ES;
  static constexpr int GB_BYTES = 16 * GB_ROW;
  static constexpr int G_BYTES = GA_BYTES + GB_BYTES;
  static constexpr int RS = D + 4;
  static constexpr int U_ROW = UD * 4;
  static constexpr int U_PIECES = (U_ROW + 1023) / 1024, U_LAST = (U_ROW - (U_PIECES - 1) * 1024) / 16;
  static_assert(U_ROW % 16 == 0, "pre-mix rows are copied in 16-byte units");
  static constexpr int o_tab = 0;
  static constexpr int o_tinfo = (o_tab + (2 * NS * 16 + G::WD) * 4 + 15) / 16 * 16;
  static constexpr int o_ids = o_tinfo + 4 * 32;
  static constexpr int o_idok = o_ids + 4 * 128;
  static constexpr int o_pos = o_idok + 16;
  static constexpr int o_hmx = o_pos + 2 * 512;
  static constexpr int o_srow = o_hmx + 2 * 128;
  static constexpr int z_y = 0, z_112 = 12, z_121 = 28, z_211 = 40, z_222 = 56, ZT = LMAX == 2 ? 84 : 12;
  static constexpr int o_zt = o_srow + 2 * 64;
  static constexpr int o_init = o_zt + 2 * 16 * ZT * 4;
  static constexpr int o_g = o_init + G::T(0) * 1024;
  static constexpr int o_b1 = o_g + G_BYTES;
  static constexpr int o_b2 = o_b1 + NFR * FRB;
  static constexpr int o_o = o_b2 + NFR * FRB;
  static constexpr int o_u = o_o + 16 * RS * 4;
  static constexpr int total = o_u + 4 * U_ROW;
  static_assert(total <= 160 * 1024, "LDS image exceeds the CU");
};

struct TileInfo { int e0, n, n0, node0, node1, sl0, sl1; };

__device__ __forceinline__ void dma16(const void* gsrc, uint32_t lds_dst) {
  uint32_t keep;
  asm volatile("s_mov_b32 %0, m0\n\ts_mov_b32 m0, %2\n\ts_nop 0\n\tglobal_load_lds_dwordx4 %1, off\n\ts_mov_b32 m0, %0"
               : "=&s"(keep) : "v"(gsrc), "s"(lds_dst) : "memory");
}
#ifndef WS_UNT
#define WS_UNT 1
#endif
__device__ __forceinline__ void dma16_stream(const void* gsrc, uint32_t lds_dst) {
#if WS_UNT
  uint32_t keep;
  asm volatile("s_mov_b32 %0, m0\n\ts_mov_b32 m0, %2\n\ts_nop 0\n\tglobal_load_lds_dwordx4 %1, off nt\n\ts_mov_b32 m0, %0"
               : "=&s"(keep) : "v"(gsrc), "s"(lds_dst) : "memory");
#else
  dma16(gsrc, lds_dst);
#endif
}
__device__ __forceinline__ void dma4(const void* gsrc, uint32_t lds_dst) {
  uint32_t keep;
  asm volatile("s_mov_b32 %0, m0\n\ts_mov_b32 m0, %2\n\ts_nop 0\n\tglobal_load_lds_dword %1, off\n\ts_mov_b32 m0, %0"
               : "=&s"(keep) : "v"(gsrc), "s"(lds_dst) : "memory");
}
__device__ __forceinline__ void ws_wait_vm0() { asm volatile("s_waitcnt vmcnt(0)" ::: "memory"); }
__device__ __forceinline__ void ws_barrier() { asm volatile("s_waitcnt lgkmcnt(0)\n\ts_barrier" ::: "memory"); }
__device__ __forceinline__ int sgpr(int v) { return __builtin_amdgcn_readfirstlane(v); }
__device__ __forceinline__ void split2_f16_scaled(const float v0, const float v1, const float s, uint32_t& hi, uint32_t& lo) {
  uint32_t h, l;
  asm("v_fma_mixlo_f16 %0, %1, %2, 0 op_sel_hi:[0,0,0]" : "=v"(h) : "v"(s), "v"(v0));
  asm("v_fma_mixhi_f16 %0, %1, %2, 0 op_sel_hi:[0,0,0]" : "+v"(h) : "v"(s), "v"(v1));
  asm("v_fma_mixlo_f16 %0, %1, %2, -%3 op_sel:[0,0,0] op_sel_hi:[0,0,1]" : "=v"(l) : "v"(s), "v"(v0), "v"(h));
  asm("v_fma_mixhi_f16 %0, %1, %2, -%3 op_sel:[0,0,1] op_sel_hi:[0,0,1]" : "+v"(l) : "v"(s), "v"(v1), "v"(h));
  hi = h; lo = l;
}
template <bool IO16>
__device__ __forceinline__ void ws_put4(unsigned char* dst, const float (&f)[4], const float s) {
  if constexpr (IO16) {
    const uint32_t a = __builtin_bit_cast(uint32_t, __builtin_convertvector(f32x2_t{f[0], f[1]}, bf16x2_t));
    const uint32_t b = __builtin_bit_cast(uint32_t, __builtin_convertvector(f32x2_t{f[2], f[3]}, bf16x2_t));
    *reinterpret_cast<uint2*>(dst) = uint2{a, b};
  } else {
    uint32_t h0, l0, h1, l1;
    split2_f16_scaled(f[0], f[1], s, h0, l0);
    split2_f16_scaled(f[2], f[3], s, h1, l1);
    *reinterpret_cast<uint2*>(dst) = uint2{h0, h1};
    *reinterpret_cast<uint2*>(dst + 1024) = uint2{l0, l1};
  }
}
template <class F>
__device__ __forceinline__ void sfor3(F&& f) {
  f(std::integral_constant<int, 0>{}); f(std::integral_constant<int, 1>{}); f(std::integral_constant<int, 2>{});
}

template <int LMAX, int TT, int ROLE>
struct Own {
  using G = MsgGeom<LMAX, TT>;
  static constexpr int t = ROLE & 1;
  static constexpr int LV = ROLE < 2 ? LMAX : LMAX - 1;
  static constexpr int tG = LV > 0 ? TT * LV + t : -1;
  static constexpr int tS = ROLE >= 2 ? t : -1;
  static constexpr int sl3(int s) { return s == 0 ? LV : 0; }
  static constexpr int stile(int s) { return s == 0 ? t : s == 1 ? tG : tS; }
  static constexpr bool shas(int s) { return s == 0 ? LV > 0 : stile(s) >= 0; }
  static constexpr bool has(int s, int l1, int l2) { return shas(s) && G::ok(l1, l2, sl3(s)); }
  static constexpr int widx(int s, int l1, int l2) {
    int n = 0;
    for (int ss = 0; ss < 3; ++ss)
      for (int a = 0; a <= LMAX; ++a)
        for (int b = 0; b <= LMAX; ++b) {
          if (ss == s && a == l1 && b == l2) return has(ss, a, b) ? n : -1;
          if (has(ss, a, b)) ++n;
        }
    return n;
  }
  static constexpr int NW = widx(3, 0, 0);
};

template <int NW>
struct RoleW { uint4 h[NW], l[NW]; };

template <int LMAX, int TT, int ROLE, bool IO16>
__device__ __forceinline__ void ws_load_w(const float* packed, const int prod , const int lane,
                                          RoleW<Own<LMAX, TT, ROLE>::NW>& w) {
  using G = MsgGeom<LMAX, TT>;
  using O = Own<LMAX, TT, ROLE>;
  const unsigned char* base = reinterpret_cast<const unsigned char*>(packed + G::o_w) + (size_t)prod * G::nblk() * 2048 + lane * 16;
  auto one = [&](auto stag, auto atag, auto btag) {
    constexpr int s = decltype(stag)::value, l1 = decltype(atag)::value, l2 = decltype(btag)::value;
    if constexpr (l1 <= LMAX && l2 <= LMAX && O::has(s, l1, l2)) {
      constexpr int i = O::widx(s, l1, l2), blk = G::blk(l1, l2, O::sl3(s)) + O::stile(s);
      w.h[i] = *reinterpret_cast<const uint4*>(base + (size_t)blk * 2048);
      if constexpr (!IO16) w.l[i] = *reinterpret_cast<const uint4*>(base + (size_t)blk * 2048 + 1024);
      else w.l[i] = uint4{0, 0, 0, 0};
    }
  };
  using I0 = std::integral_constant<int, 0>; using I1 = std::integral_constant<int, 1>; using I2 = std::integral_constant<int, 2>;
  auto slot = [&](auto stag) {
    one(stag, I0{}, I0{}); one(stag, I0{}, I1{}); one(stag, I0{}, I2{});
    one(stag, I1{}, I0{}); one(stag, I1{}, I1{}); one(stag, I1{}, I2{});
    one(stag, I2{}, I0{}); one(stag, I2{}, I1{}); one(stag, I2{}, I2{});
  };
  slot(I0{}); slot(I1{}); slot(I2{});
}

#ifndef WS_XROT
#define WS_XROT 2
#endif
#ifndef WS_NREG
#define WS_NREG 1
#endif
#ifndef WS_PRIO1
#define WS_PRIO1 WS_PRIO
#endif
#ifndef WS_LMAX1
#define WS_LMAX1 0
#endif
#ifndef WS_INITMAP
#define WS_INITMAP 0
#endif
#ifndef WS_YROT
#define WS_YROT 0
#endif
#ifndef WS_PF
#define WS_PF 2
#endif
#ifndef WS_PKT
#define WS_PKT 15
#endif
#ifndef WS_PKZ
#define WS_PKZ 11
#endif
#ifndef WS_PRIO
#define WS_PRIO 0
#endif
template <int LMAX>
struct TpItems {
  static constexpr int N = (LMAX + 1) * (LMAX + 1) + LMAX;
  static constexpr int len(int l) { return 2 * l + 1 + (l > 0 ? 1 : 0); }
  static constexpr int start(int l) { int n = 0; for (int k = LMAX; k > l; --k) n += len(k); return n; }
  static constexpr int l1(int i) { int l = LMAX; while (l > 0 && i >= start(l) + len(l)) --l; return l; }
  static constexpr int a(int i) { const int l = l1(i), k = i - start(l); return k < 2 * l + 1 ? k : -1; }
  static constexpr bool first(int i) { return i == start(l1(i)); }
};

template <int LMAX, int TT, int ROLE, bool FIRST, bool IO16>
struct TpRun {
  using G = MsgGeom<LMAX, TT>;
  using O = Own<LMAX, TT, ROLE>;
  using L = Ws<LMAX, TT, IO16>;
  using IT = TpItems<LMAX>;
  static constexpr int LV = O::LV, t = O::t, tG = O::tG, tS = O::tS;
  static constexpr bool SC = tG >= 0 || tS >= 0;

  const RoleW<O::NW>& w;
  const unsigned char* bfr;
  const float* zt;
  const float* urow;
  const float* wd;
  const f32x4* init;
  f32x4 (&accV)[5];
  f32x4& accG;
  f32x4& accS;
  float dsc;
  uint4 bh[WS_PF + 1], bl[WS_PF + 1];
  f32x4 uV[3][3][5];
  f32x4 wdV;
  f32x4 yv[3];
  f32x4 zq[3][3][7];
#if E3_WS_STAMP
  uint32_t* tpm = nullptr;
  uint32_t tpm0 = 0;
#endif
  static constexpr int zoff(int l1, int l2) {
    return (l1 == 1 && l2 == 1 && LV == 2) ? L::z_112 : (l1 == 1 && l2 == 2 && LV == 1) ? L::z_121
         : (l1 == 2 && l2 == 1 && LV == 1) ? L::z_211 : (l1 == 2 && l2 == 2 && LV == 2) ? L::z_222 : -1;
  }
  __device__ __forceinline__ float yy(const int i) const { return yv[i >> 2][i & 3]; }

  template <int I>
  __device__ __forceinline__ void request() {
    if constexpr (I < IT::N) {
      constexpr int L1 = IT::l1(I), a = IT::a(I), slot = I % (WS_PF + 1);
      constexpr int fr = a >= 0 ? L::frag(L1, a) : L::frag_ff(L1);
      if constexpr (a >= 0 || SC) {
        bh[slot] = *reinterpret_cast<const uint4*>(bfr + fr * L::FRB);
        if constexpr (!IO16) bl[slot] = *reinterpret_cast<const uint4*>(bfr + fr * L::FRB + 1024);
        else bl[slot] = uint4{0, 0, 0, 0};
      }
      const f32x4 zero4 = {0.f, 0.f, 0.f, 0.f};
      if constexpr (a >= 0) {
        sfor3([&](auto l2tag) {
          constexpr int L2 = decltype(l2tag)::value;
          if constexpr (LV > 0 && G::ok(L1, L2, LV)) {
            if constexpr (FIRST) uV[L1][L2][a] = *reinterpret_cast<const f32x4*>(urow + G::uoff(L1, L2, LV) + (a * G::T(LV) + t) * 16);
            else uV[L1][L2][a] = zero4;
            if constexpr (a == 0 && zoff(L1, L2) >= 0) {
              constexpr int NZ = ((2 * L1 + 1) * (2 * LV + 1) + 3) / 4;
#pragma unroll
              for (int q = 0; q < NZ; ++q) zq[L1][L2][q] = *reinterpret_cast<const f32x4*>(zt + zoff(L1, L2) + 4 * q);
            }
          }
        });
        if constexpr (L1 == 0 && FIRST && LV > 0) wdV = *reinterpret_cast<const f32x4*>(wd + G::wdoff(LV) + t * 16);
      }
    }
  }

  template <int I>
  __device__ __forceinline__ void compute() {
    constexpr int L1 = IT::l1(I), a = IT::a(I), slot = I % (WS_PF + 1);
    const uint4 xh = bh[slot], xl = bl[slot];
    if constexpr (a >= 0) {
      if constexpr (L1 == 0 && FIRST && LV > 0) {
        uV[0][LV][0] = __builtin_elementwise_fma(wdV, f32x4{dsc, dsc, dsc, dsc}, uV[0][LV][0]);
      }
      sfor3([&](auto l2tag) {
        constexpr int L2 = decltype(l2tag)::value;
        if constexpr (LV > 0 && G::ok(L1, L2, LV)) {
          constexpr int i = O::widx(0, L1, L2);
          uV[L1][L2][a] = mma3<IO16>(w.h[i], w.l[i], xh, xl, uV[L1][L2][a]);
        }
      });
      if constexpr (L1 == 0) {
        if constexpr (tG >= 0) accG = mma3<IO16>(w.h[O::widx(1, 0, 0)], w.l[O::widx(1, 0, 0)], xh, xl, accG);
        if constexpr (tS >= 0) accS = mma3<IO16>(w.h[O::widx(2, 0, 0)], w.l[O::widx(2, 0, 0)], xh, xl, accS);
      }
    } else if constexpr (SC) {
      if constexpr (tG >= 0) accG = mma3<IO16>(w.h[O::widx(1, L1, L1)], w.l[O::widx(1, L1, L1)], xh, xl, accG);
      if constexpr (tS >= 0) accS = mma3<IO16>(w.h[O::widx(2, L1, L1)], w.l[O::widx(2, L1, L1)], xh, xl, accS);
    }
  }

  template <int L1>
  __device__ __forceinline__ void fold() {
    constexpr int D1 = 2 * L1 + 1;
    sfor3([&](auto l2tag) {
      constexpr int L2 = decltype(l2tag)::value;
      if constexpr (LV > 0 && G::ok(L1, L2, LV)) {
        constexpr int D3 = 2 * LV + 1;
        if constexpr (zoff(L1, L2) >= 0) {
#pragma unroll
          for (int c = 0; c < D3; ++c)
#pragma unroll
            for (int aa = 0; aa < D1; ++aa)
              if (z_nonzero<L1, L2, LV>(aa, c)) {
                const float z = zq[L1][L2][(aa * D3 + c) >> 2][(aa * D3 + c) & 3];
                constexpr int zi = (L1 == 1 && L2 == 1) ? 0 : (L1 == 1 && L2 == 2) ? 1 : (L1 == 2 && L2 == 1) ? 2 : 3;
                if constexpr (!IO16 && (WS_PKT & 1) && ((WS_PKZ >> zi) & 1)) {
                  accV[c] = __builtin_elementwise_fma(uV[L1][L2][aa], f32x4{z, z, z, z}, accV[c]);
                } else {
#pragma unroll
                  for (int r = 0; r < 4; ++r) accV[c][r] = __builtin_fmaf(uV[L1][L2][aa][r], z, accV[c][r]);
                }
              }
        } else {
          float y9[9];
#pragma unroll
          for (int i = 0; i < 9; ++i) y9[i] = yy(i);
          float zz[D1][D3];
          make_z<L1, L2, LV>(y9, zz);
#pragma unroll
          for (int c = 0; c < D3; ++c)
#pragma unroll
            for (int aa = 0; aa < D1; ++aa)
              if (z_nonzero<L1, L2, LV>(aa, c)) {
                if constexpr (!IO16 && (WS_PKT & 2)) {
                  accV[c] = __builtin_elementwise_fma(uV[L1][L2][aa], f32x4{zz[aa][c], zz[aa][c], zz[aa][c], zz[aa][c]}, accV[c]);
                } else {
#pragma unroll
                  for (int r = 0; r < 4; ++r) accV[c][r] = __builtin_fmaf(uV[L1][L2][aa][r], zz[aa][c], accV[c][r]);
                }
              }
        }
      }
    });
  }

  template <int I>
  __device__ __forceinline__ void step() {
    request<I + WS_PF>();
    __builtin_amdgcn_sched_barrier(0);
    compute<I>();
    if constexpr (IT::first(I) && IT::l1(I) < LMAX) fold<IT::l1(I) + 1>();
    if constexpr (I + 1 < IT::N && IT::first(I + 1)) { WS_TPMARK(1 + LMAX - IT::l1(I)) }
    if constexpr (I + 1 < IT::N) step<I + 1>();
    else { WS_TPMARK(1 + LMAX) fold<0>(); WS_TPMARK(2 + LMAX) }
  }

  __device__ __forceinline__ void run() {
    const f32x4 zero4 = {0.f, 0.f, 0.f, 0.f};
#pragma unroll
    for (int c = 0; c < 5; ++c) accV[c] = zero4;
#pragma unroll
    for (int q = 0; q < 3; ++q) yv[q] = *reinterpret_cast<const f32x4*>(zt + L::z_y + 4 * q);
    accG = zero4; accS = zero4;
    if constexpr (FIRST) {
      if constexpr (tG >= 0) accG = init[64 * tG];
      if constexpr (tS >= 0) accS = init[64 * tS];
    }
    request<0>();
    if constexpr (WS_PF >= 2) request<1>();
    if constexpr (WS_PF >= 3) request<2>();
    static_assert(WS_PF >= 1 && WS_PF <= 3, "prefetch distance");
    __builtin_amdgcn_sched_barrier(0);
    dsc = yv[2][1];
    WS_TPMARK(0)
    step<0>();
  }
};

template <int LMAX, int TT, int ROLE, bool FIRST, bool IO16>
__device__ __forceinline__ void ws_tp(const RoleW<Own<LMAX, TT, ROLE>::NW>& w, const unsigned char* bfr, const float* zt,
                                      const float* urow, const float* wd, const f32x4* init,
                                      f32x4 (&accV)[5], f32x4& accG, f32x4& accS, float (&y)[10], uint32_t* tpmarks = nullptr) {
  TpRun<LMAX, TT, ROLE, FIRST, IO16> r{w, bfr, zt, urow, wd, init, accV, accG, accS};
#if E3_WS_STAMP
  r.tpm = tpmarks;
  r.tpm0 = (uint32_t)__builtin_readcyclecounter();
#endif
  r.run();
#pragma unroll
  for (int i = 0; i < 10; ++i) y[i] = r.yy(i);
}

template <class BOX>
struct WsArgsT {
  const void* h; int64_t ldh;
  const float4* pos4; const int32_t* src; const int32_t* dst; int64_t E;
  const float* packed; const float* U; const float* hmax; const float* in_scale; float* out; int64_t ldo;
  int chunk;
  BOX box;
};
using WsArgs = WsArgsT<PbcBox>;

template <int LMAX, int TT, bool IO16, int W, int PBC>
__device__ __forceinline__ void ws_run(const WsArgsT<typename PbcArg<PBC>::type>& A, unsigned char* smem) {
  using G = MsgGeom<LMAX, TT>;
  using L = Ws<LMAX, TT, IO16>;
  constexpr int H = G::H, D = G::D, ES = L::ES;
  constexpr bool TEAM1 = W >= 4;
  constexpr int ROLE = W & 3;
  constexpr int SX = TEAM1 ? -1 : ((W + WS_XROT) & 3);
  constexpr int ITB = SX < 0 ? 0 : (WS_INITMAP ? (SX == 3 ? 0 : 4) : 2 * SX);
  constexpr int ITE0 = SX < 0 ? 0 : (WS_INITMAP ? (SX == 3 ? 4 : (SX == 2 ? 6 : 4)) : (SX <= 2 ? 2 * SX + 2 : 2 * SX));
  constexpr int ITE = ITE0 < G::T(0) ? ITE0 : G::T(0);
  constexpr int SY = TEAM1 ? ((W + WS_YROT) & 3) : -1;
  using O = Own<LMAX, TT, ROLE>;
  using I0 = std::integral_constant<int, 0>; using I1 = std::integral_constant<int, 1>; using I2 = std::integral_constant<int, 2>;
  const int lane = threadIdx.x & 63, j = lane & 15, g = lane >> 4;
  const uint32_t lds0 = (uint32_t)(uintptr_t)smem;
  const float* n1tab = reinterpret_cast<const float*>(smem + L::o_tab);
  const float* n2tab = n1tab + G::NS * 16;
  const float* wdtab = n2tab + G::NS * 16;
  const float xs = (!IO16 && A.in_scale) ? A.in_scale[0] : 1.0f;
  const float bwx = A.packed[6] * ((!IO16 && A.in_scale) ? A.in_scale[1] : 1.0f);
  const char* hb = reinterpret_cast<const char*>(A.h);

  auto tinfo = [&](const int tile) -> TileInfo {
    TileInfo ti = {0, 0, 0, -1, -1, 0, 0};
    if (tile >= 0) {
      const int4* p = reinterpret_cast<const int4*>(smem + L::o_tinfo + (tile & 3) * 32);
      const int4 a = p[0], b = p[1];
      ti.e0 = sgpr(a.x); ti.n = sgpr(a.y); ti.n0 = sgpr(a.z); ti.node0 = sgpr(a.w);
      ti.node1 = sgpr(b.x); ti.sl0 = sgpr(b.y); ti.sl1 = sgpr(b.z);
    }
    return ti;
  };

  RoleW<O::NW> w;
  ws_load_w<LMAX, TT, ROLE, IO16>(A.packed, TEAM1 ? 1 : 0, lane, w);
  wait_vm0();
  f32x4 nrS = {0.f, 0.f, 0.f, 0.f}, nrG = {0.f, 0.f, 0.f, 0.f}, nrV[5];
  {
    const f32x4* ntq = reinterpret_cast<const f32x4*>(TEAM1 ? n2tab : n1tab) + g;
    if constexpr (O::tS >= 0) nrS = ntq[4 * O::tS];
#pragma unroll
    for (int c = 0; c < 5; ++c) nrV[c] = f32x4{0.f, 0.f, 0.f, 0.f};
    if constexpr (O::LV > 0) {
      nrG = ntq[4 * O::tG];
#pragma unroll
      for (int c = 0; c < 2 * O::LV + 1; ++c) nrV[c] = ntq[4 * (G::slot0(O::LV) + (2 * O::LV + 1) * O::t + c)];
    }
  }

  const int Ei = (int)A.E;
  const int per_xcd = (int)(gridDim.x >> 3), wg_idx = (int)(blockIdx.x >> 3);
  const int e_per_xcd = ((Ei + 7) / 8 + 15) / 16 * 16;
  const int xlo = (int)(blockIdx.x & 7) * e_per_xcd;
  const int xhi = xlo + e_per_xcd < Ei ? xlo + e_per_xcd : Ei;

  auto gather_part = [&](const int tile, const int part) {
    const int* ids = reinterpret_cast<const int*>(smem + L::o_ids) + (tile & 3) * 32;
    const uint32_t gb = lds0 + L::o_g;
    static_assert(L::GA_ROW % 16 == 0 && L::GA_ROW <= 1024 && (L::GB_ROW == 128 || L::GB_ROW == 64), "copy shapes of the image");
    constexpr int LA = L::GA_ROW / 16;
    constexpr int UPR = L::GB_ROW / 16;
    constexpr int RPC = 64 / UPR;
    const int myid = ids[lane & 15];
    const int ridb = ids[(RPC == 8 ? 8 * part : 0) + lane / UPR];
    asm volatile("s_waitcnt lgkmcnt(0)" ::: "memory");
#pragma unroll
    for (int k = 0; k < 8; ++k) {
      const int r = 8 * part + k;
      const int rid = part == 0 ? __builtin_amdgcn_readlane(myid, k) : __builtin_amdgcn_readlane(myid, 8 + k);
      const char* rowp = hb + ((int64_t)rid * A.ldh + H) * ES;
      if (LA >= 64 || lane < LA) dma16(rowp + lane * 16, sgpr((int)(gb + r * L::GA_STRIDE)));
    }
    if (RPC == 8 || part == 0)
      dma16(hb + (int64_t)ridb * A.ldh * ES + (lane % UPR) * 16, sgpr((int)(gb + L::GA_BYTES + (RPC == 8 ? part * 1024 : 0))));
  };
  auto ids_requested = [&](const int tile) -> bool {
    return sgpr(reinterpret_cast<const int*>(smem + L::o_idok)[tile & 3]) != 0;
  };

  int pci = 0, pe0 = 0, pcend = 0, psl0 = -1, psl1 = -1, plast_node = -1, plast_slot = 0, pnext = 0;
  bool pok = false;
  auto chunk_start = [&](const int ci) {
    pe0 = sgpr(xlo + (ci * per_xcd + wg_idx) * A.chunk);
    pok = pe0 < xhi;
    pcend = sgpr(pe0 + A.chunk < xhi ? pe0 + A.chunk : xhi);
  };
  auto issue_ids = [&](const int tile) {
    if (lane == 0) reinterpret_cast<int*>(smem + L::o_idok)[tile & 3] = pok ? 1 : 0;
    if (pok && lane < 32) {
      int e = pe0 + (lane & 15);
      e = e < Ei ? e : Ei - 1;
      const int32_t* p = (lane < 16 ? A.src : A.dst) + e;
      dma4(p, sgpr((int)(lds0 + L::o_ids + (tile & 3) * 128)));
    }
  };
  auto cut = [&](const int tile) {
    int* tip = reinterpret_cast<int*>(smem + L::o_tinfo) + (tile & 3) * 8;
    if (!pok) {
      if (lane < 8) tip[lane] = lane < 3 ? 0 : (lane < 5 ? -1 : 0);
      issue_ids(tile + 1);
      return;
    }
    const int* ids = reinterpret_cast<const int*>(smem + L::o_ids) + (tile & 3) * 32;
    const int nmax = sgpr(pcend - pe0 < 16 ? pcend - pe0 : 16);
    const int did = ids[16 + j], dprev = ids[16 + (j > 0 ? j - 1 : 0)];
    const unsigned long long m = __ballot(lane >= 1 && lane < nmax && did != dprev);
    const unsigned long long m2 = m & (m - 1);
    const int n0 = sgpr(m ? (int)__builtin_ctzll(m) : nmax);
    const int n = sgpr(m2 ? (int)__builtin_ctzll(m2) : nmax);
    const int node0 = __builtin_amdgcn_readlane(did, 0);
    const int node1 = n0 < n ? __builtin_amdgcn_readlane(did, n0) : -1;
    const int myid = ids[(lane & 16) + ((lane & 15) < n ? (lane & 15) : n - 1)];
    asm volatile("s_waitcnt lgkmcnt(0)" ::: "memory");
    auto alloc = [&](const int avoid) {
      int sl = pnext;
#pragma unroll
      for (int k = 0; k < 3; ++k)
        if (sl == psl0 || sl == psl1 || sl == avoid) sl = (sl + 1) & 3;
      pnext = (sl + 1) & 3;
      return sl;
    };
    auto urow_copy = [&](const int node, const int slot) {
      const char* up = reinterpret_cast<const char*>(A.U) + (int64_t)node * L::U_ROW + lane * 16;
      const uint32_t dstb = lds0 + L::o_u + slot * L::U_ROW;
#pragma unroll
      for (int i = 0; i < L::U_PIECES; ++i)
        if (i + 1 < L::U_PIECES || lane < L::U_LAST) dma16_stream(up + i * 1024, sgpr((int)(dstb + i * 1024)));
    };
    int sl0, sl1 = -1;
    if (node0 == plast_node) sl0 = plast_slot;
    else { sl0 = sgpr(alloc(-1)); urow_copy(node0, sl0); }
    if (node1 >= 0) { sl1 = sgpr(alloc(sl0)); urow_copy(node1, sl1); }
    psl0 = sl0; psl1 = sl1;
    plast_node = node1 >= 0 ? node1 : node0;
    plast_slot = node1 >= 0 ? sl1 : sl0;
    if (lane == 0) {
      tip[0] = pe0; tip[1] = n; tip[2] = n0; tip[3] = node0; tip[4] = node1; tip[5] = sl0; tip[6] = sl1 >= 0 ? sl1 : sl0;
    }
    if (lane < 32) {
      dma16(A.pos4 + myid, sgpr((int)(lds0 + L::o_pos + (tile & 1) * 512)));
      dma4(A.hmax + myid, sgpr((int)(lds0 + L::o_hmx + (tile & 1) * 128)));
    }
    pe0 = sgpr(pe0 + n);
    if (pe0 >= pcend) chunk_start(++pci);
    issue_ids(tile + 1);
  };

  if constexpr (SX == 3) {
    chunk_start(0);
    issue_ids(0);
    ws_wait_vm0();
    asm volatile("s_waitcnt lgkmcnt(0)" ::: "memory");
    const bool ok0 = pok;
    cut(0);
    asm volatile("s_waitcnt lgkmcnt(0)" ::: "memory");
    if (ok0) { gather_part(0, 0); gather_part(0, 1); }
    ws_wait_vm0();
  }
  ws_barrier();

  constexpr int NQ = (D + 63) / 64;
  constexpr bool RSW = SY == 0 || SY == 1;
  constexpr int Q0 = !RSW ? 0 : (SY == 0 ? 0 : (NQ + 1) / 2), Q1 = !RSW ? 0 : (SY == 0 ? (NQ + 1) / 2 : NQ);
  constexpr int NQW = Q1 - Q0 > 0 ? Q1 - Q0 : 1;
  int cur = -1;
  float carry[NQW];
#pragma unroll
  for (int q = 0; q < NQW; ++q) carry[q] = 0.f;
  auto flush = [&]() {
    if (cur >= 0) {
      float* o = A.out + (int64_t)cur * A.ldo;
#pragma unroll
      for (int q = 0; q < Q1 - Q0; ++q)
        if (64 * (Q0 + q) + lane < D) __builtin_amdgcn_global_atomic_fadd_f32(o + 64 * (Q0 + q) + lane, carry[q]);
    }
#pragma unroll
    for (int q = 0; q < NQW; ++q) carry[q] = 0.f;
  };
#if E3_WS_STAMP
  uint32_t tpmk[8] = {0, 0, 0, 0, 0, 0, 0, 0};
  uint32_t st_acc[4] = {0, 0, 0, 0}, st_t = (uint32_t)__builtin_readcyclecounter();
#define WS_STAMP(i) { const uint32_t t_ = (uint32_t)__builtin_readcyclecounter(); st_acc[i] += t_ - st_t; st_t = t_; }
  uint32_t pm_t = 0;
#define WS_PM0 { pm_t = (uint32_t)__builtin_readcyclecounter(); }
#define WS_PM(i) { const uint32_t t_ = (uint32_t)__builtin_readcyclecounter(); tpmk[i] += t_ - pm_t; pm_t = t_; }
#else
  uint32_t* const tpmk = nullptr;
#define WS_STAMP(i)
#define WS_PM0
#define WS_PM(i)
#endif
  TileInfo t0 = tinfo(0), t1 = tinfo(-1);
  for (int s = 0;; ++s) {
    if (s >= 1 && t1.n == 0) break;
    WS_STAMP(3)
    WS_PM0
    if constexpr (SX == 3) cut(s + 1);
    if constexpr (!TEAM1) {
      if (SX <= 1 && t0.n > 0) {
        const int j8 = lane & 7, gg = (lane >> 3) & 3, pc = lane >> 5, row = 8 * SX + j8;
        const unsigned char* gimg = smem + L::o_g;
        unsigned char* b1 = smem + L::o_b1 + (16 * gg + row) * 16 + 8 * pc;
        const float4* pp = reinterpret_cast<const float4*>(smem + L::o_pos + (s & 1) * 512);
        const float4 ps = pp[row], pd = pp[16 + row];
        float q2[20], q1[12], q0[4];
        {
          const unsigned char* r2 = gimg + row * L::GA_STRIDE + (LMAX == 2 ? (3 * H + (16 * pc + 4 * gg) * 5) * ES : 0);
          const unsigned char* r1 = gimg + row * L::GA_STRIDE + (16 * pc + 4 * gg) * 3 * ES;
          const unsigned char* r0 = gimg + L::GA_BYTES + row * L::GB_ROW + (16 * pc + 4 * gg) * ES;
          if constexpr (!IO16) {
#pragma unroll
            for (int u = 0; u < (LMAX == 2 ? 5 : 0); ++u) { const f32x4 v = reinterpret_cast<const f32x4*>(r2)[u]; q2[4 * u] = v[0]; q2[4 * u + 1] = v[1]; q2[4 * u + 2] = v[2]; q2[4 * u + 3] = v[3]; }
#pragma unroll
            for (int u = 0; u < 3; ++u) { const f32x4 v = reinterpret_cast<const f32x4*>(r1)[u]; q1[4 * u] = v[0]; q1[4 * u + 1] = v[1]; q1[4 * u + 2] = v[2]; q1[4 * u + 3] = v[3]; }
            { const f32x4 v = reinterpret_cast<const f32x4*>(r0)[0]; q0[0] = v[0]; q0[1] = v[1]; q0[2] = v[2]; q0[3] = v[3]; }
          } else {
            auto widen = [](const uint2 v, float* o) {
              o[0] = __builtin_bit_cast(float, v.x << 16); o[1] = __builtin_bit_cast(float, v.x & 0xffff0000u);
              o[2] = __builtin_bit_cast(float, v.y << 16); o[3] = __builtin_bit_cast(float, v.y & 0xffff0000u);
            };
#pragma unroll
            for (int u = 0; u < (LMAX == 2 ? 5 : 0); ++u) widen(reinterpret_cast<const uint2*>(r2)[u], q2 + 4 * u);
#pragma unroll
            for (int u = 0; u < 3; ++u) widen(reinterpret_cast<const uint2*>(r1)[u], q1 + 4 * u);
            widen(reinterpret_cast<const uint2*>(r0)[0], q0);
          }
        }
        __builtin_amdgcn_sched_barrier(0);
        float y[9], dist;
        if constexpr (LMAX == 2) edge_sh<PBC>(ps, pd, y, dist, A.box); else edge_sh1<PBC>(ps, pd, y, dist, A.box);
        auto put4 = [&](const int fr, const float (&f)[4]) { ws_put4<IO16>(b1 + fr * L::FRB, f, xs); };
        auto degree = [&](auto ltag, float* q) {
          constexpr int L1 = decltype(ltag)::value, D1 = 2 * L1 + 1;
#pragma unroll
          for (int a = 0; a < D1; ++a) {
            const float f[4] = {q[a], q[D1 + a], q[2 * D1 + a], q[3 * D1 + a]};
            put4(L::frag(L1, a), f);
          }
          if constexpr (L1 > 0) {
            float zz[D1][1];
            make_z<L1, L1, 0>(y, zz);
            float f[4];
#pragma unroll
            for (int r = 0; r < 4; ++r) {
              float sum = zz[0][0] * q[r * D1];
#pragma unroll
              for (int a = 1; a < D1; ++a) sum = __builtin_fmaf(zz[a][0], q[r * D1 + a], sum);
              f[r] = sum;
            }
            put4(L::frag_ff(L1), f);
          }
        };
        if constexpr (LMAX == 2) degree(I2{}, q2);
        degree(I1{}, q1);
        degree(I0{}, q0);
      }
      if ((ITB < ITE || SX == 2) && t0.n > 0) {
        const float4* pp = reinterpret_cast<const float4*>(smem + L::o_pos + (s & 1) * 512);
        const float4 ps = pp[j], pd = pp[16 + j];
        const int slot = (j >= t0.n0 && j < t0.n) ? t0.sl1 : t0.sl0;
        const float* urow = reinterpret_cast<const float*>(smem + L::o_u + slot * L::U_ROW) + 4 * g;
        constexpr int T0 = G::T(0);
        float y[9], dist;
        if constexpr (LMAX == 2) edge_sh<PBC>(ps, pd, y, dist, A.box); else edge_sh1<PBC>(ps, pd, y, dist, A.box);
        const float dsc = dist * xs;
        float z110[3][1], z220[5][1];
        make_z<1, 1, 0>(y, z110);
        if constexpr (LMAX == 2) make_z<2, 2, 0>(y, z220);
        f32x4* ip = reinterpret_cast<f32x4*>(smem + L::o_init) + lane;
        static_assert(T0 == 6 || T0 == 4, "two scalar-type tiles per wave (0, 1, 2 / 0, 1)");
#pragma unroll
        for (int t2 = ITB; t2 < ITE; t2 += 2) {
          f32x4 u0[2], u1[3][2], u2[5][2], wv[2];
#pragma unroll
          for (int k = 0; k < 2; ++k) {
            const int tt = t2 + k;
            u0[k] = *reinterpret_cast<const f32x4*>(urow + G::uoff(0, 0, 0) + tt * 16);
            wv[k] = *reinterpret_cast<const f32x4*>(wdtab + 4 * g + G::wdoff(0) + tt * 16);
#pragma unroll
            for (int a = 0; a < 3; ++a) u1[a][k] = *reinterpret_cast<const f32x4*>(urow + G::uoff(1, 1, 0) + (a * T0 + tt) * 16);
            if constexpr (LMAX == 2) {
#pragma unroll
              for (int a = 0; a < 5; ++a) u2[a][k] = *reinterpret_cast<const f32x4*>(urow + G::uoff(2, 2, 0) + (a * T0 + tt) * 16);
            }
          }
          __builtin_amdgcn_sched_barrier(0);
#pragma unroll
          for (int k = 0; k < 2; ++k) {
            f32x4 v = u0[k];
#pragma unroll
            for (int r = 0; r < 4; ++r) {
              v[r] = __builtin_fmaf(wv[k][r], dsc, v[r]);
#pragma unroll
              for (int a = 0; a < 3; ++a) v[r] = __builtin_fmaf(u1[a][k][r], z110[a][0], v[r]);
              if constexpr (LMAX == 2) {
#pragma unroll
                for (int a = 0; a < 5; ++a) v[r] = __builtin_fmaf(u2[a][k][r], z220[a][0], v[r]);
              }
            }
            ip[64 * (t2 + k)] = v;
          }
          __builtin_amdgcn_sched_barrier(0);
        }
        if constexpr (SX == 2) {
        float* zr = reinterpret_cast<float*>(smem + L::o_zt + (s & 1) * 16 * L::ZT * 4) + j * L::ZT;
        auto store_dense = [&](auto atag, auto btag, auto ctag, float* dstp) {
          constexpr int A1 = decltype(atag)::value, B1 = decltype(btag)::value, C1 = decltype(ctag)::value;
          constexpr int Da = 2 * A1 + 1, Dc = 2 * C1 + 1, NE = Da * Dc;
          float zz[Da][Dc];
          make_z<A1, B1, C1>(y, zz);
          float flat[(NE + 3) / 4 * 4];
#pragma unroll
          for (int i = 0; i < (NE + 3) / 4 * 4; ++i) flat[i] = i < NE ? zz[i / Dc][i % Dc] : 0.f;
#pragma unroll
          for (int q = 0; q < (NE + 3) / 4; ++q)
            *reinterpret_cast<f32x4*>(dstp + 4 * q) = f32x4{flat[4 * q], flat[4 * q + 1], flat[4 * q + 2], flat[4 * q + 3]};
        };
        if (g == 0) {
          *reinterpret_cast<f32x4*>(zr + L::z_y) = f32x4{y[0], y[1], y[2], y[3]};
          *reinterpret_cast<f32x4*>(zr + L::z_y + 4) = f32x4{y[4], y[5], y[6], y[7]};
          *reinterpret_cast<f32x4*>(zr + L::z_y + 8) = f32x4{y[8], dsc, 0.f, 0.f};
          if constexpr (LMAX == 2) store_dense(I1{}, I1{}, I2{}, zr + L::z_112);
        } else if constexpr (LMAX == 2) {
          if (g == 1) {
            store_dense(I1{}, I2{}, I1{}, zr + L::z_121);
          } else if (g == 2) {
            store_dense(I2{}, I1{}, I1{}, zr + L::z_211);
          } else {
            store_dense(I2{}, I2{}, I2{}, zr + L::z_222);
          }
        }
        }
      }
    } else {
      if (t1.n > 0) {
        float y[10];
        const float* ztr = reinterpret_cast<const float*>(smem + L::o_zt + ((s - 1) & 1) * 16 * L::ZT * 4) + j * L::ZT;
        const uint32_t sb = reinterpret_cast<const uint32_t*>(smem + L::o_srow)[((s - 1) & 1) * 16 + j];
        const float isrow = IO16 ? 1.0f : __builtin_bit_cast(float, 0x7F000000u - sb);
        f32x4 accV[5], accG, accS;
        __builtin_amdgcn_s_setprio(WS_PRIO);
        WS_PM(5)
        ws_tp<LMAX, TT, ROLE, false, IO16>(w, smem + L::o_b2 + lane * 16, ztr, nullptr, nullptr, nullptr, accV, accG, accS, y, tpmk);
        WS_PM0
        const f32x4* nt = reinterpret_cast<const f32x4*>(n2tab) + g;
        float* orow = reinterpret_cast<float*>(smem + L::o_o) + j * L::RS;
        if constexpr (O::tS >= 0) {
          const f32x4 nv = WS_NREG ? nrS : nt[4 * O::tS];
          f32x4 o;
#pragma unroll
          for (int r = 0; r < 4; ++r) {
            const float sv = accS[r] * nv[r] * isrow;
            o[r] = sv * sigmoid_(sv);
          }
          *reinterpret_cast<f32x4*>(orow + 16 * O::t + 4 * g) = o;
        }
        if constexpr (O::LV > 0) {
          constexpr int Dc = 2 * O::LV + 1;
          const f32x4 gn = WS_NREG ? nrG : nt[4 * O::tG];
          f32x4 gt;
#pragma unroll
          for (int r = 0; r < 4; ++r) gt[r] = sigmoid_(accG[r] * gn[r] * isrow) * isrow;
          float o[4 * Dc];
#pragma unroll
          for (int c = 0; c < Dc; ++c) {
            const f32x4 nv = WS_NREG ? nrV[c] : nt[4 * (G::slot0(O::LV) + Dc * O::t + c)];
            f32x4 oc;
            if constexpr (!IO16 && (WS_PKT & 4)) {
              oc = accV[c] * nv * gt;
            } else {
#pragma unroll
              for (int r = 0; r < 4; ++r) oc[r] = accV[c][r] * nv[r] * gt[r];
            }
#pragma unroll
            for (int r = 0; r < 4; ++r) o[r * Dc + c] = oc[r];
          }
          f32x4* dq = reinterpret_cast<f32x4*>(orow + G::col0(O::LV) + (16 * O::t + 4 * g) * Dc);
#pragma unroll
          for (int k = 0; k < Dc; ++k) dq[k] = f32x4{o[4 * k], o[4 * k + 1], o[4 * k + 2], o[4 * k + 3]};
        }
      }
    }
    if constexpr (TEAM1) __builtin_amdgcn_s_setprio(0);
    WS_PM(6)
    WS_STAMP(0)
    ws_barrier();
    WS_STAMP(1)
    WS_PM0
    if constexpr (!TEAM1) {
      if (t0.n > 0) {
        float y[10];
        const float* ztr = reinterpret_cast<const float*>(smem + L::o_zt + (s & 1) * 16 * L::ZT * 4) + j * L::ZT;
        const float* hm = reinterpret_cast<const float*>(smem + L::o_hmx + (s & 1) * 128);
        const float hs = hm[j], hd = hm[16 + j];
        const int slot = (j >= t0.n0 && j < t0.n) ? t0.sl1 : t0.sl0;
        const float* urow = reinterpret_cast<const float*>(smem + L::o_u + slot * L::U_ROW) + 4 * g;
        f32x4 accV[5], accG, accS;
        __builtin_amdgcn_s_setprio(WS_PRIO1);
        WS_PM(5)
        ws_tp<LMAX, TT, ROLE, true, IO16>(w, smem + L::o_b1 + lane * 16, ztr, urow, wdtab + 4 * g,
                                          reinterpret_cast<const f32x4*>(smem + L::o_init) + lane, accV, accG, accS, y, tpmk);
        WS_PM0
        const float dsc = y[9];
        float srow = 1.0f;
        if constexpr (!IO16) srow = pow2_scale_from_bits(__builtin_bit_cast(uint32_t, bwx * fmaxf(fmaxf(hs, hd), dsc)), 12);
        const f32x4* nt = reinterpret_cast<const f32x4*>(n1tab) + g;
        unsigned char* b2 = smem + L::o_b2 + lane * 16 + 8 * O::t;
        auto put4 = [&](const int fr, const float (&f)[4]) { ws_put4<IO16>(b2 + fr * L::FRB, f, srow); };
        if constexpr (O::tS >= 0) {
          const f32x4 nv = WS_NREG ? nrS : nt[4 * O::tS];
          float f[4];
#pragma unroll
          for (int r = 0; r < 4; ++r) {
            const float sv = accS[r] * nv[r];
            f[r] = sv * sigmoid_(sv);
          }
          put4(L::frag(0, 0), f);
        }
        if constexpr (O::LV > 0) {
          constexpr int Dc = 2 * O::LV + 1;
          const f32x4 gn = WS_NREG ? nrG : nt[4 * O::tG];
          f32x4 gt;
#pragma unroll
          for (int r = 0; r < 4; ++r) gt[r] = sigmoid_(accG[r] * gn[r]);
          float y9[9];
#pragma unroll
          for (int i = 0; i < 9; ++i) y9[i] = y[i];
          float zz[Dc][1];
          make_z<O::LV, O::LV, 0>(y9, zz);
          f32x4 fsv = {0.f, 0.f, 0.f, 0.f};
#pragma unroll
          for (int c = 0; c < Dc; ++c) {
            const f32x4 nv = WS_NREG ? nrV[c] : nt[4 * (G::slot0(O::LV) + Dc * O::t + c)];
            f32x4 fv;
            if constexpr (!IO16 && (WS_PKT & 8)) {
              fv = accV[c] * nv * gt;
              const f32x4 zc = {zz[c][0], zz[c][0], zz[c][0], zz[c][0]};
              fsv = c == 0 ? zc * fv : __builtin_elementwise_fma(zc, fv, fsv);
            } else {
#pragma unroll
              for (int r = 0; r < 4; ++r) {
                fv[r] = accV[c][r] * nv[r] * gt[r];
                fsv[r] = c == 0 ? zz[0][0] * fv[r] : __builtin_fmaf(zz[c][0], fv[r], fsv[r]);
              }
            }
            const float f[4] = {fv[0], fv[1], fv[2], fv[3]};
            put4(L::frag(O::LV, c), f);
          }
          const float fs[4] = {fsv[0], fsv[1], fsv[2], fsv[3]};
          put4(L::frag_ff(O::LV), fs);
        }
        if constexpr (ROLE == 3 && !IO16) {
          if (lane < 16) reinterpret_cast<float*>(smem + L::o_srow)[(s & 1) * 16 + lane] = srow;
        }
      }
      if constexpr (SX == 3) ws_wait_vm0();
    } else if constexpr (RSW) {
      if (t1.n > 0) {
        const float* op = reinterpret_cast<const float*>(smem + L::o_o) + lane;
        float s0[NQW], s1[NQW];
#pragma unroll
        for (int q = 0; q < NQW; ++q) { s0[q] = 0.f; s1[q] = 0.f; }
        float v[16][NQW];
#pragma unroll
        for (int r = 0; r < 16; ++r)
#pragma unroll
          for (int q = 0; q < Q1 - Q0; ++q) v[r][q] = (64 * (Q0 + q) + lane < D) ? op[r * L::RS + 64 * (Q0 + q)] : 0.f;
        __builtin_amdgcn_sched_barrier(0);
        if (t1.n0 == 16) {
#pragma unroll
          for (int r = 0; r < 16; ++r)
#pragma unroll
            for (int q = 0; q < Q1 - Q0; ++q) s0[q] += v[r][q];
        } else {
#pragma unroll
          for (int r = 0; r < 16; ++r) {
#pragma unroll
            for (int q = 0; q < Q1 - Q0; ++q) {
              s0[q] += r < t1.n0 ? v[r][q] : 0.f;
              s1[q] += (r >= t1.n0 && r < t1.n) ? v[r][q] : 0.f;
            }
          }
        }
        if (t1.node0 != cur) { flush(); cur = t1.node0; }
#pragma unroll
        for (int q = 0; q < NQW; ++q) carry[q] += s0[q];
        if (t1.node1 >= 0) {
          flush();
          cur = t1.node1;
#pragma unroll
          for (int q = 0; q < NQW; ++q) carry[q] = s1[q];
        }
      }
    } else {
      if (ids_requested(s + 1)) gather_part(s + 1, SY - 2);
      ws_wait_vm0();
    }
    if constexpr (!TEAM1) __builtin_amdgcn_s_setprio(0);
    const TileInfo tn = tinfo(s + 1);
    WS_PM(7)
    WS_STAMP(2)
    ws_barrier();
    t1 = t0; t0 = tn;
  }
  if constexpr (RSW) flush();
#if E3_WS_STAMP
  if (lane == 0) {
    for (int i = 0; i < 4; ++i) atomicAdd(&g_ws_stamps[W][i], (unsigned long long)st_acc[i]);
    for (int i = 0; i < 8; ++i) atomicAdd(&g_ws_tp[W][i], (unsigned long long)tpmk[i]);
  }
#endif
#undef WS_STAMP
}

template <int LMAX, int TT, bool IO16, int PBC>
__global__ __launch_bounds__(512, 2) __attribute__((amdgpu_waves_per_eu(2, 2))) void msg_ws_kernel(
    const WsArgsT<typename PbcArg<PBC>::type> A) {
  using G = MsgGeom<LMAX, TT>;
  using L = Ws<LMAX, TT, IO16>;
  extern __shared__ __align__(16) unsigned char ws_smem[];
  {
    float* n1tab = reinterpret_cast<float*>(ws_smem + L::o_tab);
    float* n2tab = n1tab + G::NS * 16;
    float* wdtab = n2tab + G::NS * 16;
    const float ixs = (!IO16 && A.in_scale) ? A.in_scale[1] : 1.0f;
    for (int i = threadIdx.x; i < G::NS * 16; i += blockDim.x) {
      n1tab[i] = A.packed[G::o_norm1 + i] * ixs;
      n2tab[i] = A.packed[G::o_norm2 + i];
    }
    for (int i = threadIdx.x; i < G::WD; i += blockDim.x) wdtab[i] = A.packed[G::o_wd + i];
  }
  __syncthreads();
  const int wave = __builtin_amdgcn_readfirstlane((int)(threadIdx.x >> 6));
  switch (wave) {
    case 0: ws_run<LMAX, TT, IO16, 0, PBC>(A, ws_smem); break;
    case 1: ws_run<LMAX, TT, IO16, 1, PBC>(A, ws_smem); break;
    case 2: ws_run<LMAX, TT, IO16, 2, PBC>(A, ws_smem); break;
    case 3: ws_run<LMAX, TT, IO16, 3, PBC>(A, ws_smem); break;
    case 4: ws_run<LMAX, TT, IO16, 4, PBC>(A, ws_smem); break;
    case 5: ws_run<LMAX, TT, IO16, 5, PBC>(A, ws_smem); break;
    case 6: ws_run<LMAX, TT, IO16, 6, PBC>(A, ws_smem); break;
    default: ws_run<LMAX, TT, IO16, 7, PBC>(A, ws_smem); break;
  }
}

bool msg_ws_supported(int lmax, int hidden, int dtype) {
  return (lmax == 2 || (lmax == 1 && WS_LMAX1)) && hidden == 32 && (dtype == E3_F32 || dtype == E3_BF16);
}

int msg_ws_launch(int lmax, int hidden, int dtype, const void* h, int64_t ldh, int64_t N, const float* pos4, const int32_t* src,
                  const int32_t* dst, int64_t E, const void* packed, const float* in_scale, const float* premix, float* out,
                  int64_t ldo, int chunk_edges, hipStream_t stream, const float* box, const PbcCell* cell) {
  if (!msg_ws_supported(lmax, hidden, dtype)) return E3_ERR_UNSUPPORTED;
  const int pb = cell ? kCell : (box ? kBox : kOpen);
  if (E > 0x7fffffffLL - 65536) return E3_ERR_UNSUPPORTED;
  const int io = dtype == E3_BF16 ? 1 : 0;
  const int li = lmax == 2 ? 1 : 0;
#if WS_LMAX1
  const void* kern =
      pb == kCell
          ? (li ? (io ? (const void*)msg_ws_kernel<2, 2, true, kCell> : (const void*)msg_ws_kernel<2, 2, false, kCell>)
                : (io ? (const void*)msg_ws_kernel<1, 2, true, kCell> : (const void*)msg_ws_kernel<1, 2, false, kCell>))
      : pb ? (li ? (io ? (const void*)msg_ws_kernel<2, 2, true, kBox> : (const void*)msg_ws_kernel<2, 2, false, kBox>)
                 : (io ? (const void*)msg_ws_kernel<1, 2, true, kBox> : (const void*)msg_ws_kernel<1, 2, false, kBox>))
           : (li ? (io ? (const void*)msg_ws_kernel<2, 2, true, kOpen> : (const void*)msg_ws_kernel<2, 2, false, kOpen>)
                 : (io ? (const void*)msg_ws_kernel<1, 2, true, kOpen> : (const void*)msg_ws_kernel<1, 2, false, kOpen>));
  const int lds = li ? (io ? Ws<2, 2, true>::total : Ws<2, 2, false>::total) : (io ? Ws<1, 2, true>::total : Ws<1, 2, false>::total);
  const int ud = li ? MsgGeom<2, 2>::UD : MsgGeom<1, 2>::UD;
#else
  const void* kern =
      pb == kCell ? (io ? (const void*)msg_ws_kernel<2, 2, true, kCell> : (const void*)msg_ws_kernel<2, 2, false, kCell>)
      : pb        ? (io ? (const void*)msg_ws_kernel<2, 2, true, kBox> : (const void*)msg_ws_kernel<2, 2, false, kBox>)
                  : (io ? (const void*)msg_ws_kernel<2, 2, true, kOpen> : (const void*)msg_ws_kernel<2, 2, false, kOpen>);
  const int lds = io ? Ws<2, 2, true>::total : Ws<2, 2, false>::total;
  const int ud = MsgGeom<2, 2>::UD;
#endif
  int dev = 0;
  E3_HIP_CHECK(hipGetDevice(&dev));
  static std::mutex mu;
  static int cus_of[64][2][2][3];
  int cus = 0;
  {
    std::lock_guard<std::mutex> lock(mu);
    if (dev < 0 || dev >= 64) return E3_ERR_INVALID_ARG;
    if (cus_of[dev][io][li][pb] == 0) {
      E3_HIP_CHECK(hipFuncSetAttribute(kern, hipFuncAttributeMaxDynamicSharedMemorySize, lds));
      int n = 0;
      if (hipDeviceGetAttribute(&n, hipDeviceAttributeMultiprocessorCount, dev) != hipSuccess || n <= 0) n = 256;
      cus_of[dev][io][li][pb] = n;
    }
    cus = cus_of[dev][io][li][pb];
  }
  int chunk = chunk_edges > 0 ? (chunk_edges + 15) / 16 * 16 : 256;
  const int64_t nchunks = (E + chunk - 1) / chunk;
  int nwg = (int)std::min<int64_t>(cus, nchunks);
  nwg = std::max(8, (nwg + 7) / 8 * 8);
  const float* hmax = premix + (size_t)N * ud;
  auto launch = [&](const auto& pbc) {
    WsArgsT<std::decay_t<decltype(pbc)>> a = {h, ldh, reinterpret_cast<const float4*>(pos4), src, dst, E,
                                              static_cast<const float*>(packed), premix, hmax, in_scale, out, ldo, chunk, pbc};
    void* args[] = {&a};
    return hipLaunchKernel(kern, dim3(nwg), dim3(512), args, lds, stream) == hipSuccess ? E3_OK : E3_ERR_HIP;
  };
  return cell ? launch(*cell) : launch(make_box(box));
}

}

#if E3_WS_STAMP
extern "C" int e3_msg_ws_debug_stamps(unsigned long long* out96, int reset) {
  if (out96 && hipMemcpyFromSymbol(out96, HIP_SYMBOL(e3::g_ws_stamps), 256) != hipSuccess) return E3_ERR_HIP;
  if (out96 && hipMemcpyFromSymbol(out96 + 32, HIP_SYMBOL(e3::g_ws_tp), 512) != hipSuccess) return E3_ERR_HIP;
  if (reset) {
    unsigned long long z[64] = {0};
    if (hipMemcpyToSymbol(HIP_SYMBOL(e3::g_ws_stamps), z, 256) != hipSuccess) return E3_ERR_HIP;
    if (hipMemcpyToSymbol(HIP_SYMBOL(e3::g_ws_tp), z, 512) != hipSuccess) return E3_ERR_HIP;
  }
  return E3_OK;
}
#endif
```

scalable-e3-gnn_amd/message.py:

```python
from __future__ import annotations

import ctypes

import torch

from . import _lib, profiling
from .radius_graph import RadiusGraph

_NAT = ("l0e", "l1o", "l2e")


class FusedMessage:

    def __init__(self, lmax: int, hidden: int):
        self.lmax, self.hidden = int(lmax), int(hidden)
        self._plans = _lib.DevicePlans("e3_msg_plan_create", "e3_msg_plan_destroy", self.lmax, self.hidden)
        self._packed = {}
        self.tiles_per_block = 0

    def __deepcopy__(self, memo):
        return FusedMessage(self.lmax, self.hidden)

    def __reduce__(self):
        return (FusedMessage, (self.lmax, self.hidden))

    @staticmethod
    def supported(lmax: int, hidden: int) -> bool:
        return lmax in (1, 2) and hidden in (16, 32, 64)

    @property
    def width(self) -> int:
        return self.hidden * (self.lmax + 1) ** 2

    def _tensors(self, tp):
        ws = [getattr(tp, "weights_" + c, None) for c in _NAT]
        ns = [getattr(tp, "norm_" + c, None) for c in _NAT]
        return ws, ns

    def supports(self, dtype) -> bool:
        if dtype == torch.float32:
            return True
        return dtype == torch.bfloat16 and bool(_lib.load().e3_msg_supports(self._plans.handle(None), _lib.E3_BF16))

    def packed(self, msg1, msg2, device, dtype=torch.float32) -> torch.Tensor:
        lib = _lib.load()
        w1, n1 = self._tensors(msg1)
        w2, n2 = self._tensors(msg2)
        ts = w1 + n1 + w2 + n2
        key = tuple((t.data_ptr(), t._version) if t is not None else None for t in ts)
        hit = self._packed.get((device, dtype))
        stream = torch.cuda.current_stream(device)
        if hit is not None and hit[0] == key:
            if hit[2] != stream.cuda_stream:
                stream.wait_event(hit[3])
            return hit[1]
        h = self._plans.handle(device)
        for tpi, ws in ((1, w1), (2, w2)):
            for l in range(self.lmax + 1):
                rows, cols = ctypes.c_int(), ctypes.c_int()
                lib.e3_msg_weight_shape(h, tpi, l, ctypes.byref(rows), ctypes.byref(cols))
                w = ws[l]
                if w is None or tuple(w.shape) != (rows.value, cols.value) or w.dtype != dtype or w.device != device:
                    raise RuntimeError(f"fused message: TP #{tpi} weights of degree {l} must be {dtype} "
                                       f"[{rows.value}, {cols.value}] on {device}, got "
                                       f"{None if w is None else (tuple(w.shape), w.dtype, w.device)}")
        P3 = ctypes.c_void_p * 3
        keep = [t.detach().contiguous() if t is not None else None for t in ts]
        ptr = lambda t: t.data_ptr() if (t is not None and t.numel()) else None
        packed = torch.empty(int(lib.e3_msg_packed_bytes(h)), dtype=torch.uint8, device=device)
        with torch.cuda.device(device):
            for t in keep[3:6] + keep[9:12]:
                if t is not None and t.numel() and t.dtype != dtype:
                    raise RuntimeError(f"fused message: norm buffers must be {dtype} (cast the module), got {t.dtype}")
            _lib.check(lib.e3_msg_pack_weights(h, P3(*map(ptr, keep[0:3])), P3(*map(ptr, keep[3:6])),
                                               P3(*map(ptr, keep[6:9])), P3(*map(ptr, keep[9:12])), _lib.dtype_code(dtype),
                                               packed.data_ptr(), stream.cuda_stream), "e3_msg_pack_weights")
        ev = torch.cuda.Event()
        ev.record(stream)
        self._packed[(device, dtype)] = (key, packed, stream.cuda_stream, ev)
        return packed

    def flops_per_edge(self) -> int:
        H, L = self.hidden, self.lmax
        fl = 0
        for tp, n in ((1, [2 * H + 1, 2 * H, 2 * H]), (2, [H, H, H])):
            for l3 in range(L + 1):
                M = H * (1 + L) if l3 == 0 else H
                for l1 in range(L + 1):
                    for l2 in range(L + 1):
                        if abs(l1 - l2) <= l3 <= l1 + l2 and (l1 + l2 + l3) % 2 == 0:
                            fl += 2 * n[l1] * M * min(2 * l1 + 1, 2 * l3 + 1)
        return fl

    def refresh_row_max(self, state, h: torch.Tensor, rows: torch.Tensor, in_scale: torch.Tensor | None):
        premix = state[1]
        N = h.shape[0]
        ud = premix.numel() // N - 1
        hmax = premix[N * ud:]
        if rows.numel():
            a = h[rows].float().abs()
            m = torch.where(a < float("inf"), a, 0.0).amax(1)
        else:
            m = h.new_zeros(0, dtype=torch.float32)
        if in_scale is not None and h.dtype == torch.float32:
            m = m * in_scale[0]
        hmax[rows] = m
        return m.max() if m.numel() else torch.zeros((), device=h.device)

    def executed_flops_per_edge(self) -> int:
        H, L = self.hidden, self.lmax
        fl = 0
        for _tp in (1, 2):
            for l3 in range(L + 1):
                M = H * (1 + L) if l3 == 0 else H
                for l1 in range(L + 1):
                    for l2 in range(L + 1):
                        if abs(l1 - l2) <= l3 <= l1 + l2 and (l1 + l2 + l3) % 2 == 0:
                            groups = 1 if (l3 == 0 and l1 > 0) else (2 * l1 + 1)
                            fl += 2 * H * M * groups
        return fl

    def forward(self, h: torch.Tensor, g: RadiusGraph, msg1, msg2, in_scale: torch.Tensor | None = None, edges=None,
                cont=None, return_state: bool = False):
        if not h.is_cuda or not self.supports(h.dtype):
            raise RuntimeError(f"fused message: ROCm tensor in float32 (or bfloat16 for hidden >= 32) required, got "
                               f"{h.dtype} on {h.device} (no CPU path)")
        io, code, esz = h.dtype, _lib.dtype_code(h.dtype), h.element_size()
        N, W = h.shape
        if W != self.width or N != g.rowptr.numel() - 1:
            raise RuntimeError(f"fused message: h must be [{g.rowptr.numel() - 1}, {self.width}], got {tuple(h.shape)}")
        if h.stride(-1) != 1 or (h.stride(0) * esz) % 16 or h.data_ptr() % 16:
            h = h.contiguous()
        dev = h.device
        lib = _lib.load()
        src, dst = (g.src, g.dst) if edges is None else edges
        E = int(src.numel())
        assert src.dtype == torch.int32 and dst.dtype == torch.int32 and dst.numel() == E
        if cont is None:
            out = torch.empty((N, W), dtype=torch.float32, device=dev)
        else:
            out = cont[0]
        if N == 0:
            return (out.to(io), None) if return_state else out.to(io)
        with torch.cuda.device(dev):
            packed = self.packed(msg1, msg2, dev, io)
            if in_scale is None and io == torch.float32:
                from . import ops
                in_scale = ops.pow2_scale([h])
            sc = in_scale.data_ptr() if (in_scale is not None and io == torch.float32) else None
            hd = self._plans.handle(dev)
            stream = torch.cuda.current_stream(dev).cuda_stream
            mode = "<bf16 storage, bf16 MFMA>" if io == torch.bfloat16 else "<fp16x3 split MFMA>"
            ud = int(lib.e3_msg_premix_floats_per_node(hd))
            if cont is not None:
                premix = cont[1]
            else:
                premix = torch.empty(N * ud, dtype=torch.float32, device=dev)
                t0 = profiling.begin() if profiling.enabled() else None
                _lib.check(lib.e3_msg_premix(hd, h.data_ptr(), h.stride(0), N, packed.data_ptr(), sc,
                                             premix.data_ptr(), code, stream), "e3_msg_premix")
                if t0 is not None:
                    profiling.end(f"msg_premix lmax={self.lmax} H={self.hidden} N={N} {io}", N, N * (esz * W + 4 * ud), t0,
                                  flops=2 * self.hidden * ud * N, kernel="e3::msg_premix_kernel" + mode)
            t0 = profiling.begin() if profiling.enabled() else None
            args = (hd, h.data_ptr(), h.stride(0), N, g.pos4.data_ptr(), src.data_ptr(), dst.data_ptr(), E,
                    packed.data_ptr(), sc, premix.data_ptr(), out.data_ptr(), out.stride(0), code,
                    0 if cont is None else 1, int(self.tiles_per_block))
            if g.cell is not None:
                _lib.check(lib.e3_msg_forward_cell(*args, g.cell_arg, stream), "e3_msg_forward_cell")
            elif g.box is not None:
                _lib.check(lib.e3_msg_forward_pbc(*args, g.box_arg, stream), "e3_msg_forward_pbc")
            else:
                _lib.check(lib.e3_msg_forward(*args, stream), "e3_msg_forward")
            if t0 is not None:
                nb = esz * N * W + 16 * N + 8 * E + 4 * N * W
                ws = bool(self.lmax == 2 and self.hidden == 32 and int(self.tiles_per_block) >= 0)
                profiling.end(f"msg_fused lmax={self.lmax} H={self.hidden} E={E} {io}", E, nb, t0,
                              flops=self.flops_per_edge() * E,
                              kernel=("e3::msg_ws_kernel" if ws else "e3::msg_fused_kernel") + mode,
                              executed_flops=self.executed_flops_per_edge() * E)
        return (out, (out, premix)) if return_state else out
```

Measured before the change: 11.59 million particles/s.

## Precompute per-node fp16 hi/lo split features in premix for the ws message kernel

The premix kernel now also writes a per-node fp16 hi/lo split image of the node features into an extra region of the premix buffer. The warp-specialized message kernel reads these pre-split features and builds its LDS image from them, instead of loading and splitting f32 rows per edge. A row-refresh kernel is added to keep the split region and row maxima in sync when rows change. This trades extra premix memory and writes for less per-edge conversion work and LDS traffic in the message kernel.

```diff
diff --git a/include/e3gnn.h b/include/e3gnn.h
--- a/include/e3gnn.h
+++ b/include/e3gnn.h
@@ -199,6 +199,10 @@
                         const void* const w2[3], const void* const n2[3], int dtype, void* packed, void* stream);
 int e3_msg_premix(e3_msg_plan* plan, const void* h, int64_t ld_h, int64_t N, const void* packed,
                   const float* in_scale, float* premix, int dtype, void* stream);
+int e3_msg_premix_regions(const e3_msg_plan* plan, int64_t N, int64_t* split_offset, int64_t* split_floats_per_node,
+                          int64_t* row_max_offset);
+int e3_msg_refresh_rows(e3_msg_plan* plan, const void* h, int64_t ld_h, int64_t N, const int64_t* rows, int64_t n_rows,
+                        const float* in_scale, float* premix, int dtype, void* stream);
 int e3_msg_forward(e3_msg_plan* plan, const void* h, int64_t ld_h, int64_t N, const float* pos4,
                    const int32_t* src, const int32_t* dst, int64_t E, const void* packed, const float* in_scale,
                    const float* premix, float* out, int64_t ld_out, int dtype, int accumulate, int tiles_per_block,
diff --git a/scalable-e3-gnn_amd/_lib.py b/scalable-e3-gnn_amd/_lib.py
--- a/scalable-e3-gnn_amd/_lib.py
+++ b/scalable-e3-gnn_amd/_lib.py
@@ -84,6 +84,9 @@
     "e3_msg_pack_weights": (c_int, [c_void_p, c_void_p * 3, c_void_p * 3, c_void_p * 3, c_void_p * 3, c_int, c_void_p,
                                     c_void_p]),
     "e3_msg_premix": (c_int, [c_void_p, c_void_p, c_int64, c_int64, c_void_p, c_void_p, c_void_p, c_int, c_void_p]),
+    "e3_msg_premix_regions": (c_int, [c_void_p, c_int64, POINTER(c_int64), POINTER(c_int64), POINTER(c_int64)]),
+    "e3_msg_refresh_rows": (c_int, [c_void_p, c_void_p, c_int64, c_int64, c_void_p, c_int64, c_void_p, c_void_p, c_int,
+                                    c_void_p]),
     "e3_msg_forward": (c_int, [c_void_p, c_void_p, c_int64, c_int64, c_void_p, c_void_p, c_void_p, c_int64, c_void_p,
                                c_void_p, c_void_p, c_void_p, c_int64, c_int, c_int, c_int, c_void_p]),
     "e3_edge_geometry_backward": (c_int, [c_void_p, c_void_p, c_void_p, c_int64, c_int, c_void_p, c_void_p, c_void_p,
diff --git a/scalable-e3-gnn_amd/csrc/e3_msg_common.h b/scalable-e3-gnn_amd/csrc/e3_msg_common.h
--- a/scalable-e3-gnn_amd/csrc/e3_msg_common.h
+++ b/scalable-e3-gnn_amd/csrc/e3_msg_common.h
@@ -44,6 +44,19 @@
   static constexpr int lds_tab = 2 * NS * 16 + WD;
   static constexpr int lds_wave = 16 * (D + 4);
 };
+
+template <int LMAX>
+struct MsgSplit {
+  static constexpr int NC = (LMAX + 1) * (LMAX + 1);
+  static constexpr int UNITS = NC * 8;
+  static constexpr int FLOATS = UNITS * 4;
+  static constexpr int BYTES = UNITS * 16;
+  static constexpr int unit(int f, int half, int g) { return 8 * f + 4 * half + g; }
+};
+struct MsgPremixLayout { int64_t split, hmax, per_node; };
+constexpr MsgPremixLayout msg_premix_layout(int ud, int split_floats, int64_t N) {
+  return {N * ud, N * ((int64_t)ud + split_floats), (int64_t)ud + split_floats + 1};
+}
 
 __host__ __device__ constexpr int kperm(int g, int jj) { return 16 * (jj >> 2) + 4 * g + (jj & 3); }
 
diff --git a/scalable-e3-gnn_amd/csrc/e3_msg_fused.hip b/scalable-e3-gnn_amd/csrc/e3_msg_fused.hip
--- a/scalable-e3-gnn_amd/csrc/e3_msg_fused.hip
+++ b/scalable-e3-gnn_amd/csrc/e3_msg_fused.hip
@@ -346,11 +346,50 @@
 }
 
 
+template <int LMAX, int TT, bool IO16, int L1, bool FINITE>
+__device__ __forceinline__ void split_degree(const char* row, const int g, const float xs, float& rowmax,
+                                             uint4 (&xh)[MsgGeom<LMAX, TT>::KS][2 * L1 + 1],
+                                             uint4 (&xl)[MsgGeom<LMAX, TT>::KS][2 * L1 + 1]) {
+  using G = MsgGeom<LMAX, TT>;
+  constexpr int D1 = 2 * L1 + 1, ES = IO16 ? 2 : 4;
+#pragma unroll
+  for (int ks = 0; ks < G::KS; ++ks) {
+    float x[8][D1];
+#pragma unroll
+    for (int p = 0; p < 2; ++p) {
+      if (16 * (2 * ks + p) < G::H)
+        read_piece<D1, IO16>(row + (G::col0(L1) + (32 * ks + 16 * p + 4 * g) * D1) * ES, p, xs, x);
+      else
+        zero_piece<D1>(p, x);
+    }
+#pragma unroll
+    for (int i = 0; i < 8; ++i)
+#pragma unroll
+      for (int aa = 0; aa < D1; ++aa) rowmax = FINITE ? fmax_finite(rowmax, x[i][aa]) : fmaxf(rowmax, fabsf(x[i][aa]));
+#pragma unroll
+    for (int a = 0; a < D1; ++a) {
+      float f[8];
+#pragma unroll
+      for (int i = 0; i < 8; ++i) f[i] = x[i][a];
+      split8<IO16>(f, xh[ks][a], xl[ks][a]);
+    }
+  }
+}
+template <int LMAX, int L1>
+__device__ __forceinline__ void store_split_degree(uint4* noderow, const int g, const uint4 (&xh)[2 * L1 + 1],
+                                                   const uint4 (&xl)[2 * L1 + 1]) {
+#pragma unroll
+  for (int a = 0; a < 2 * L1 + 1; ++a) {
+    noderow[MsgSplit<LMAX>::unit(L1 * L1 + a, 0, g)] = xh[a];
+    noderow[MsgSplit<LMAX>::unit(L1 * L1 + a, 1, g)] = xl[a];
+  }
+}
+
 template <int LMAX, int TT, bool IO16>
 __global__ __launch_bounds__(256) void msg_premix_kernel(const void* __restrict__ hv, int64_t ldh, int64_t N,
                                                          const float* __restrict__ packed,
                                                          const float* __restrict__ in_scale, float* __restrict__ U,
-                                                         float* __restrict__ hmax) {
+                                                         uint4* __restrict__ split, float* __restrict__ hmax) {
   using G = MsgGeom<LMAX, TT>;
   constexpr int ES = IO16 ? 2 : 4;
   const int lane = threadIdx.x & 63, j = lane & 15, g = lane >> 4;
@@ -374,27 +413,9 @@
     auto per_l1 = [&](auto l1tag) {
       constexpr int L1 = decltype(l1tag)::value, D1 = 2 * L1 + 1;
       uint4 xh[G::KS][D1], xl[G::KS][D1];
-#pragma unroll
-      for (int ks = 0; ks < G::KS; ++ks) {
-        float x[8][D1];
-#pragma unroll
-        for (int p = 0; p < 2; ++p) {
-          if (16 * (2 * ks + p) < G::H)
-            read_piece<D1, IO16>(row + (G::col0(L1) + (32 * ks + 16 * p + 4 * g) * D1) * ES, p, xs, x);
-          else
-            zero_piece<D1>(p, x);
-        }
-#pragma unroll
-        for (int i = 0; i < 8; ++i)
-#pragma unroll
-          for (int aa = 0; aa < D1; ++aa) rowmax = fmaxf(rowmax, fabsf(x[i][aa]));
-#pragma unroll
-        for (int a = 0; a < D1; ++a) {
-          float f[8];
-#pragma unroll
-          for (int i = 0; i < 8; ++i) f[i] = x[i][a];
-          split8<IO16>(f, xh[ks][a], xl[ks][a]);
-        }
+      split_degree<LMAX, TT, IO16, L1, false>(row, g, xs, rowmax, xh, xl);
+      if constexpr (!IO16 && G::KS == 1) {
+        if (split && ok) store_split_degree<LMAX, L1>(split + n * MsgSplit<LMAX>::UNITS, g, xh[0], xl[0]);
       }
       auto per_path = [&](auto l2tag, auto l3tag) {
         constexpr int L2 = decltype(l2tag)::value, L3 = decltype(l3tag)::value;
@@ -462,6 +483,37 @@
     rowmax = fmaxf(rowmax, __shfl_xor(rowmax, 32));
     if (hmax && ok && lane < 16) hmax[n] = rowmax;
   }
+}
+
+template <int LMAX, int TT, bool IO16>
+__global__ __launch_bounds__(256) void msg_refresh_rows_kernel(const void* __restrict__ hv, int64_t ldh, int64_t N,
+                                                               const int64_t* __restrict__ rows, int64_t n_rows,
+                                                               const float* __restrict__ in_scale, uint4* __restrict__ split,
+                                                               float* __restrict__ hmax) {
+  constexpr int ES = IO16 ? 2 : 4;
+  const int lane = threadIdx.x & 63, j = lane & 15, g = lane >> 4;
+  const int64_t tile = (blockIdx.x * (int64_t)blockDim.x + threadIdx.x) >> 6;
+  const int64_t idx = tile * 16 + j;
+  if (tile * 16 >= n_rows) return;
+  const int64_t n = rows[idx < n_rows ? idx : n_rows - 1];
+  const bool ok = idx < n_rows && n >= 0 && n < N;
+  const float xs = (!IO16 && in_scale) ? in_scale[0] : 1.0f;
+  const char* row = reinterpret_cast<const char*>(hv) + (ok ? n : 0) * ldh * ES;
+  float rowmax = 0.f;
+  auto per_l1 = [&](auto l1tag) {
+    constexpr int L1 = decltype(l1tag)::value, D1 = 2 * L1 + 1;
+    uint4 xh[MsgGeom<LMAX, TT>::KS][D1], xl[MsgGeom<LMAX, TT>::KS][D1];
+    split_degree<LMAX, TT, IO16, L1, true>(row, g, xs, rowmax, xh, xl);
+    if constexpr (!IO16 && MsgGeom<LMAX, TT>::KS == 1) {
+      if (split && ok) store_split_degree<LMAX, L1>(split + n * MsgSplit<LMAX>::UNITS, g, xh[0], xl[0]);
+    }
+  };
+  per_l1(std::integral_constant<int, 0>{});
+  per_l1(std::integral_constant<int, 1>{});
+  if constexpr (LMAX == 2) per_l1(std::integral_constant<int, 2>{});
+  rowmax = fmaxf(rowmax, __shfl_xor(rowmax, 16));
+  rowmax = fmaxf(rowmax, __shfl_xor(rowmax, 32));
+  if (ok && lane < 16) hmax[n] = rowmax;
 }
 
 constexpr int msg_waves_per_simd(int lmax, int tt) {
@@ -883,6 +935,7 @@
   const void* premix[2];
   int64_t total_floats;
   int UD, D, lds_tab, lds_wave, nblk, NS, WD, o_norm1, o_norm2, o_wd, o_w, waves_per_simd;
+  const void* refresh[2];
 };
 template <int LMAX, int TT>
 static MsgKernels make_entry() {
@@ -892,12 +945,14 @@
                   {(const void*)msg_fused_kernel<LMAX, TT, false, kCell>, nullptr},
                   {(const void*)msg_premix_kernel<LMAX, TT, false>, nullptr}, G::total_floats,
                   G::UD, G::D, G::lds_tab, G::lds_wave, G::nblk(), G::NS, G::WD, G::o_norm1, G::o_norm2, G::o_wd, G::o_w,
-                  msg_waves_per_simd(LMAX, TT)};
+                  msg_waves_per_simd(LMAX, TT),
+                  {(const void*)msg_refresh_rows_kernel<LMAX, TT, false>, nullptr}};
   if constexpr (TT >= 2) {
     k.fused[1] = (const void*)msg_fused_kernel<LMAX, TT, true, kOpen>;
     k.fused_pbc[1] = (const void*)msg_fused_kernel<LMAX, TT, true, kBox>;
     k.fused_cell[1] = (const void*)msg_fused_kernel<LMAX, TT, true, kCell>;
     k.premix[1] = (const void*)msg_premix_kernel<LMAX, TT, true>;
+    k.refresh[1] = (const void*)msg_refresh_rows_kernel<LMAX, TT, true>;
   }
   return k;
 }
@@ -1030,7 +1085,19 @@
 }
 
 int64_t e3_msg_packed_bytes(const e3_msg_plan* P) { return P ? (P->k->total_floats * 4 + 255) / 256 * 256 : -1; }
-int64_t e3_msg_premix_floats_per_node(const e3_msg_plan* P) { return P ? P->k->UD + 1 : -1; }
+static MsgPremixLayout premix_layout(const e3_msg_plan* P, int64_t N) {
+  return msg_premix_layout(P->k->UD, msg_ws_split_floats(P->lmax, P->H), N);
+}
+int64_t e3_msg_premix_floats_per_node(const e3_msg_plan* P) { return P ? premix_layout(P, 0).per_node : -1; }
+int e3_msg_premix_regions(const e3_msg_plan* P, int64_t N, int64_t* split_offset, int64_t* split_floats_per_node,
+                          int64_t* row_max_offset) {
+  if (!P || N < 0) return E3_ERR_INVALID_ARG;
+  const MsgPremixLayout L = premix_layout(P, N);
+  if (split_offset) *split_offset = L.split;
+  if (split_floats_per_node) *split_floats_per_node = msg_ws_split_floats(P->lmax, P->H);
+  if (row_max_offset) *row_max_offset = L.hmax;
+  return E3_OK;
+}
 int e3_msg_weight_shape(const e3_msg_plan* P, int tp, int l3, int* rows, int* cols) {
   if (!P || !rows || !cols || l3 < 0 || l3 > 2 || (tp != 1 && tp != 2)) return E3_ERR_INVALID_ARG;
   *rows = tp == 1 ? P->K1[l3] : P->K2[l3];
@@ -1089,9 +1156,33 @@
   if (st != E3_OK) return st;
   const int64_t ntiles = (N + 15) / 16;
   const int grid = (int)std::min<int64_t>((ntiles + 3) / 4, 2048);
-  float* hmax = premix + (size_t)N * k.UD;
-  void* args[] = {&h, &ld_h, &N, &packed, &in_scale, &premix, &hmax};
+  const MsgPremixLayout L = premix_layout(P, N);
+  float* hmax = premix + L.hmax;
+  uint4* split = (L.hmax > L.split && msg_ws_supported(P->lmax, P->H, dtype) && !io) ? reinterpret_cast<uint4*>(premix + L.split)
+                                                                                  : nullptr;
+  void* args[] = {&h, &ld_h, &N, &packed, &in_scale, &premix, &split, &hmax};
   if (hipLaunchKernel(k.premix[io], dim3(grid), dim3(256), args, 0, (hipStream_t)stream) != hipSuccess) return E3_ERR_HIP;
+  return E3_OK;
+}
+
+int e3_msg_refresh_rows(e3_msg_plan* P, const void* h, int64_t ld_h, int64_t N, const int64_t* rows, int64_t n_rows,
+                        const float* in_scale, float* premix, int dtype, void* stream) {
+  if (!P || N < 0 || n_rows < 0) return E3_ERR_INVALID_ARG;
+  if (!e3_msg_supports(P, dtype)) return E3_ERR_UNSUPPORTED;
+  const MsgKernels& k = *P->k;
+  const int io = dtype == E3_BF16 ? 1 : 0, es = io ? 2 : 4;
+  if (N == 0 || n_rows == 0) return E3_OK;
+  if (!h || !rows || !premix || ld_h < k.D) return E3_ERR_INVALID_ARG;
+  if ((ld_h * es & 15) || ((uintptr_t)h & 15) || ((uintptr_t)premix & 15)) return E3_ERR_INVALID_ARG;
+  const int64_t nblocks = ((n_rows + 15) / 16 + 3) / 4;
+  if (nblocks > 0x7fffffffLL) return E3_ERR_INVALID_ARG;
+  const MsgPremixLayout L = premix_layout(P, N);
+  float* hmax = premix + L.hmax;
+  uint4* split = (L.hmax > L.split && msg_ws_supported(P->lmax, P->H, dtype) && !io) ? reinterpret_cast<uint4*>(premix + L.split)
+                                                                                  : nullptr;
+  void* args[] = {&h, &ld_h, &N, &rows, &n_rows, &in_scale, &split, &hmax};
+  if (hipLaunchKernel(k.refresh[io], dim3((int)nblocks), dim3(256), args, 0, (hipStream_t)stream) != hipSuccess)
+    return E3_ERR_HIP;
   return E3_OK;
 }
 
diff --git a/scalable-e3-gnn_amd/csrc/e3_msg_ws.h b/scalable-e3-gnn_amd/csrc/e3_msg_ws.h
--- a/scalable-e3-gnn_amd/csrc/e3_msg_ws.h
+++ b/scalable-e3-gnn_amd/csrc/e3_msg_ws.h
@@ -4,6 +4,7 @@
 namespace e3 {
 struct PbcCell;
 bool msg_ws_supported(int lmax, int hidden, int dtype);
+int msg_ws_split_floats(int lmax, int hidden);
 int msg_ws_launch(int lmax, int hidden, int dtype, const void* h, int64_t ldh, int64_t N, const float* pos4, const int32_t* src,
                   const int32_t* dst, int64_t E, const void* packed, const float* in_scale, const float* premix, float* out,
                   int64_t ldo, int chunk_edges, hipStream_t stream, const float* box = nullptr,
diff --git a/scalable-e3-gnn_amd/csrc/e3_msg_ws.hip b/scalable-e3-gnn_amd/csrc/e3_msg_ws.hip
--- a/scalable-e3-gnn_amd/csrc/e3_msg_ws.hip
+++ b/scalable-e3-gnn_amd/csrc/e3_msg_ws.hip
@@ -52,14 +52,94 @@
   static constexpr int z_y = 0, z_112 = 12, z_121 = 28, z_211 = 40, z_222 = 56, ZT = LMAX == 2 ? 84 : 12;
   static constexpr int o_zt = o_srow + 2 * 64;
   static constexpr int o_init = o_zt + 2 * 16 * ZT * 4;
+  static constexpr bool PRE = !IO16;
+  static constexpr int P_AROW = (NC - 1) * 128;
+  static constexpr int P_ASTRIDE = P_AROW + 32;
+  static constexpr int P_ALANES = P_AROW / 16;
+  static constexpr int o_pz = 16 * P_ASTRIDE, o_pf = o_pz + 2048;
+  static constexpr int P_IMG = o_pf + LMAX * 2048;
+  static constexpr int p_asrc(int lane) { return 128 + 16 * lane; }
+  static constexpr int p_alds(int row, int lane) { return row * P_ASTRIDE + 16 * lane; }
+  static constexpr int p_zrow(int piece, int lane) { return 8 * piece + (lane & 7); }
+  static constexpr int p_zsrc(int lane) { return 64 * ((lane >> 5) & 1) + 16 * (2 * ((lane >> 4) & 1) + ((lane >> 3) & 1)); }
+  static constexpr int p_zlds(int piece, int lane) { return o_pz + 1024 * piece + 16 * lane; }
+  static constexpr int p_zpos(int lane) {
+    return 1024 * ((lane & 15) >> 3) + 256 * (lane >> 5) + 128 * ((lane >> 4) & 1) + 16 * (lane & 7);
+  }
+  static constexpr int p_abase(int lane) { return (lane & 15) * P_ASTRIDE + 16 * (lane >> 4); }
+  static constexpr int p_zbase(int lane) { return o_pz + p_zpos(lane); }
+  static constexpr bool p_on_a(int fr) { return fr >= 1 && fr < NC; }
+  static constexpr int p_off(int fr, int half) {
+    return p_on_a(fr) ? 128 * (fr - 1) + 64 * half : (fr == 0 ? 0 : 2048 * (1 + fr - NC)) + 512 * half;
+  }
+  static constexpr int p_read(int fr, int half, int lane) { return (p_on_a(fr) ? p_abase(lane) : p_zbase(lane)) + p_off(fr, half); }
   static constexpr int o_g = o_init + G::T(0) * 1024;
-  static constexpr int o_b1 = o_g + G_BYTES;
-  static constexpr int o_b2 = o_b1 + NFR * FRB;
+  static constexpr int o_b1 = o_g + (PRE ? 2 * P_IMG : G_BYTES);
+  static constexpr int o_b2 = o_b1 + (PRE ? 0 : NFR * FRB);
   static constexpr int o_o = o_b2 + NFR * FRB;
   static constexpr int o_u = o_o + 16 * RS * 4;
   static constexpr int total = o_u + 4 * U_ROW;
   static_assert(total <= 160 * 1024, "LDS image exceeds the CU");
 };
+
+template <int LMAX, int TT>
+struct WsImageCheck {
+  using L = Ws<LMAX, TT, false>;
+  static constexpr int NU = L::o_pf / 16;
+  static constexpr int group_lane(int grp, int i) {
+    const int base = 32 * (grp >> 1), odd = grp & 1;
+    const int k = odd ? (i < 8 ? 4 + i : (i < 12 ? 16 + (i - 8) : 28 + (i - 12))) : (i < 4 ? i : (i < 8 ? 12 + (i - 4) : 20 + (i - 8)));
+    return base + k;
+  }
+  static constexpr bool run() {
+    int owner_row[NU] = {}, owner_unit[NU] = {}, count[NU] = {};
+    for (int r = 0; r < 16; ++r)
+      for (int l = 0; l < L::P_ALANES; ++l) {
+        const int u = L::p_alds(r, l) / 16;
+        if (L::p_alds(r, l) % 16 || u < 0 || u >= NU) return false;
+        ++count[u]; owner_row[u] = r; owner_unit[u] = L::p_asrc(l) / 16;
+      }
+    for (int p = 0; p < 2; ++p)
+      for (int l = 0; l < 64; ++l) {
+        const int u = L::p_zlds(p, l) / 16;
+        if (u < 0 || u >= NU) return false;
+        ++count[u]; owner_row[u] = L::p_zrow(p, l); owner_unit[u] = L::p_zsrc(l) / 16;
+      }
+    int written = 0;
+    for (int u = 0; u < NU; ++u) {
+      if (count[u] > 1) return false;
+      written += count[u];
+    }
+    if (written != 16 * MsgSplit<LMAX>::UNITS) return false;
+    for (int fr = 0; fr < L::NC; ++fr)
+      for (int half = 0; half < 2; ++half) {
+        for (int lane = 0; lane < 64; ++lane) {
+          const int a = L::p_read(fr, half, lane), u = a / 16;
+          if (a % 16 || u < 0 || u >= NU || count[u] != 1) return false;
+          if (owner_row[u] != (lane & 15) || owner_unit[u] != MsgSplit<LMAX>::unit(fr, half, lane >> 4)) return false;
+        }
+      }
+    for (int fr = 0; fr < L::NFR; ++fr)
+      for (int half = 0; half < 2; ++half)
+        for (int grp = 0; grp < 4; ++grp) {
+          bool seen[16] = {};
+          for (int i = 0; i < 16; ++i) {
+            const int a = L::p_read(fr, half, group_lane(grp, i));
+            if (a < 0 || a + 16 > L::P_IMG) return false;
+            const int slot = (a % 256) / 16;
+            if (seen[slot]) return false;
+            seen[slot] = true;
+          }
+        }
+    for (int fr = L::NC; fr < L::NFR; ++fr)
+      for (int half = 0; half < 2; ++half)
+        for (int lane = 0; lane < 64; ++lane)
+          for (int l2 = lane + 1; l2 < 64; ++l2)
+            if (L::p_read(fr, half, lane) == L::p_read(fr, half, l2) || L::p_read(fr, half, lane) < L::o_pf) return false;
+    return true;
+  }
+};
+static_assert(WsImageCheck<2, 2>::run() && WsImageCheck<1, 2>::run(), "pre-split image: coverage, read map or bank conflicts");
 
 struct TileInfo { int e0, n, n0, node0, node1, sl0, sl1; };
 
@@ -110,6 +190,14 @@
     *reinterpret_cast<uint2*>(dst + 1024) = uint2{l0, l1};
   }
 }
+template <int HI>
+__device__ __forceinline__ float fma_mix_h(const float z, const uint32_t pair, const float acc) {
+  float d;
+  if constexpr (HI) asm("v_fma_mix_f32 %0, %1, %2, %3 op_sel:[0,1,0] op_sel_hi:[0,1,0]" : "=v"(d) : "v"(z), "v"(pair), "v"(acc));
+  else asm("v_fma_mix_f32 %0, %1, %2, %3 op_sel:[0,0,0] op_sel_hi:[0,1,0]" : "=v"(d) : "v"(z), "v"(pair), "v"(acc));
+  return d;
+}
+__device__ __forceinline__ uint32_t u4_word(const uint4& v, const int i) { return i == 0 ? v.x : i == 1 ? v.y : i == 2 ? v.z : v.w; }
 template <class F>
 __device__ __forceinline__ void sfor3(F&& f) {
   f(std::integral_constant<int, 0>{}); f(std::integral_constant<int, 1>{}); f(std::integral_constant<int, 2>{});
@@ -215,8 +303,11 @@
   static constexpr int LV = O::LV, t = O::t, tG = O::tG, tS = O::tS;
   static constexpr bool SC = tG >= 0 || tS >= 0;
 
+  static constexpr bool PIMG = FIRST && L::PRE;
   const RoleW<O::NW>& w;
   const unsigned char* bfr;
+  const unsigned char* bfz;
+  int lane;
   const float* zt;
   const float* urow;
   const float* wd;
@@ -246,9 +337,20 @@
       constexpr int L1 = IT::l1(I), a = IT::a(I), slot = I % (WS_PF + 1);
       constexpr int fr = a >= 0 ? L::frag(L1, a) : L::frag_ff(L1);
       if constexpr (a >= 0 || SC) {
-        bh[slot] = *reinterpret_cast<const uint4*>(bfr + fr * L::FRB);
-        if constexpr (!IO16) bl[slot] = *reinterpret_cast<const uint4*>(bfr + fr * L::FRB + 1024);
-        else bl[slot] = uint4{0, 0, 0, 0};
+        if constexpr (PIMG) {
+          const unsigned char* b = bfr;
+          if constexpr (!L::p_on_a(fr)) {
+            int l = lane;
+            asm volatile("" : "+v"(l));
+            b = bfz + L::p_zbase(l);
+          }
+          bh[slot] = *reinterpret_cast<const uint4*>(b + L::p_off(fr, 0));
+          bl[slot] = *reinterpret_cast<const uint4*>(b + L::p_off(fr, 1));
+        } else {
+          bh[slot] = *reinterpret_cast<const uint4*>(bfr + fr * L::FRB);
+          if constexpr (!IO16) bl[slot] = *reinterpret_cast<const uint4*>(bfr + fr * L::FRB + 1024);
+          else bl[slot] = uint4{0, 0, 0, 0};
+        }
       }
       const f32x4 zero4 = {0.f, 0.f, 0.f, 0.f};
       if constexpr (a >= 0) {
@@ -373,10 +475,11 @@
 };
 
 template <int LMAX, int TT, int ROLE, bool FIRST, bool IO16>
-__device__ __forceinline__ void ws_tp(const RoleW<Own<LMAX, TT, ROLE>::NW>& w, const unsigned char* bfr, const float* zt,
+__device__ __forceinline__ void ws_tp(const RoleW<Own<LMAX, TT, ROLE>::NW>& w, const unsigned char* bfr,
+                                      const unsigned char* bfz, const int lane, const float* zt,
                                       const float* urow, const float* wd, const f32x4* init,
                                       f32x4 (&accV)[5], f32x4& accG, f32x4& accS, float (&y)[10], uint32_t* tpmarks = nullptr) {
-  TpRun<LMAX, TT, ROLE, FIRST, IO16> r{w, bfr, zt, urow, wd, init, accV, accG, accS};
+  TpRun<LMAX, TT, ROLE, FIRST, IO16> r{w, bfr, bfz, lane, zt, urow, wd, init, accV, accG, accS};
 #if E3_WS_STAMP
   r.tpm = tpmarks;
   r.tpm0 = (uint32_t)__builtin_readcyclecounter();
@@ -390,7 +493,7 @@
 struct WsArgsT {
   const void* h; int64_t ldh;
   const float4* pos4; const int32_t* src; const int32_t* dst; int64_t E;
-  const float* packed; const float* U; const float* hmax; const float* in_scale; float* out; int64_t ldo;
+  const float* packed; const float* U; const void* split; const float* hmax; const float* in_scale; float* out; int64_t ldo;
   int chunk;
   BOX box;
 };
@@ -404,8 +507,9 @@
   constexpr bool TEAM1 = W >= 4;
   constexpr int ROLE = W & 3;
   constexpr int SX = TEAM1 ? -1 : ((W + WS_XROT) & 3);
-  constexpr int ITB = SX < 0 ? 0 : (WS_INITMAP ? (SX == 3 ? 0 : 4) : 2 * SX);
-  constexpr int ITE0 = SX < 0 ? 0 : (WS_INITMAP ? (SX == 3 ? 4 : (SX == 2 ? 6 : 4)) : (SX <= 2 ? 2 * SX + 2 : 2 * SX));
+  constexpr int ITB = SX < 0 ? 0 : L::PRE ? (SX == 2 ? 4 : 0) : (WS_INITMAP ? (SX == 3 ? 0 : 4) : 2 * SX);
+  constexpr int ITE0 = SX < 0 ? 0 : L::PRE ? (SX == 1 ? 4 : (SX == 2 ? 6 : 0))
+                                           : (WS_INITMAP ? (SX == 3 ? 4 : (SX == 2 ? 6 : 4)) : (SX <= 2 ? 2 * SX + 2 : 2 * SX));
   constexpr int ITE = ITE0 < G::T(0) ? ITE0 : G::T(0);
   constexpr int SY = TEAM1 ? ((W + WS_YROT) & 3) : -1;
   using O = Own<LMAX, TT, ROLE>;
@@ -454,6 +558,22 @@
 
   auto gather_part = [&](const int tile, const int part) {
     const int* ids = reinterpret_cast<const int*>(smem + L::o_ids) + (tile & 3) * 32;
+    if constexpr (L::PRE) {
+      const uint32_t ib = lds0 + L::o_g + (tile & 1) * L::P_IMG;
+      const char* sp = reinterpret_cast<const char*>(A.split);
+      const int myid = ids[lane & 15];
+      const int zid = ids[L::p_zrow(part, lane)];
+      asm volatile("s_waitcnt lgkmcnt(0)" ::: "memory");
+#pragma unroll
+      for (int k = 0; k < 8; ++k) {
+        const int r = 8 * part + k;
+        const int rid = part == 0 ? __builtin_amdgcn_readlane(myid, k) : __builtin_amdgcn_readlane(myid, 8 + k);
+        const char* rowp = sp + (int64_t)rid * MsgSplit<LMAX>::BYTES;
+        if (L::P_ALANES >= 64 || lane < L::P_ALANES) dma16(rowp + L::p_asrc(lane), sgpr((int)(ib + L::p_alds(r, 0))));
+      }
+      dma16(sp + (int64_t)zid * MsgSplit<LMAX>::BYTES + L::p_zsrc(lane), sgpr((int)(ib + L::p_zlds(part, 0))));
+      return;
+    }
     const uint32_t gb = lds0 + L::o_g;
     static_assert(L::GA_ROW % 16 == 0 && L::GA_ROW <= 1024 && (L::GB_ROW == 128 || L::GB_ROW == 64), "copy shapes of the image");
     constexpr int LA = L::GA_ROW / 16;
@@ -488,7 +608,9 @@
     if (pok && lane < 32) {
       int e = pe0 + (lane & 15);
       e = e < Ei ? e : Ei - 1;
-      const int32_t* p = (lane < 16 ? A.src : A.dst) + e;
+      int l = lane;
+      asm volatile("" : "+v"(l));
+      const int32_t* p = (l < 16 ? A.src : A.dst) + e;
       dma4(p, sgpr((int)(lds0 + L::o_ids + (tile & 3) * 128)));
     }
   };
@@ -595,7 +717,48 @@
     WS_PM0
     if constexpr (SX == 3) cut(s + 1);
     if constexpr (!TEAM1) {
-      if (SX <= 1 && t0.n > 0) {
+      if constexpr (L::PRE) {
+        if (SX == 0 && t0.n > 0) {
+          const unsigned char* img = smem + L::o_g + (s & 1) * L::P_IMG;
+          const unsigned char* ba = img + L::p_abase(lane);
+          unsigned char* bz = smem + L::o_g + (s & 1) * L::P_IMG + L::p_zbase(lane);
+          const float4* pp = reinterpret_cast<const float4*>(smem + L::o_pos + (s & 1) * 512);
+          const float4 ps = pp[j], pd = pp[16 + j];
+          uint4 xh[L::NC - 1], xl[L::NC - 1];
+#pragma unroll
+          for (int f = 1; f < L::NC; ++f) {
+            xh[f - 1] = *reinterpret_cast<const uint4*>(ba + L::p_off(f, 0));
+            xl[f - 1] = *reinterpret_cast<const uint4*>(ba + L::p_off(f, 1));
+          }
+          __builtin_amdgcn_sched_barrier(0);
+          float y[9], dist;
+          if constexpr (LMAX == 2) edge_sh<PBC>(ps, pd, y, dist, A.box); else edge_sh1<PBC>(ps, pd, y, dist, A.box);
+          auto degree = [&](auto ltag) {
+            constexpr int L1 = decltype(ltag)::value, D1 = 2 * L1 + 1, F0 = L1 * L1 - 1;
+            float zz[D1][1];
+            make_z<L1, L1, 0>(y, zz);
+            float f[8];
+#pragma unroll
+            for (int k = 0; k < 8; ++k) {
+              float sum = 0.f;
+#pragma unroll
+              for (int a = 0; a < D1; ++a) {
+                const uint32_t ph = u4_word(xh[F0 + a], k >> 1), pl = u4_word(xl[F0 + a], k >> 1);
+                if (k & 1) { sum = fma_mix_h<1>(zz[a][0], ph, sum); sum = fma_mix_h<1>(zz[a][0], pl, sum); }
+                else { sum = fma_mix_h<0>(zz[a][0], ph, sum); sum = fma_mix_h<0>(zz[a][0], pl, sum); }
+              }
+              f[k] = sum;
+            }
+            uint32_t h[4], l[4];
+#pragma unroll
+            for (int q = 0; q < 4; ++q) split2_f16_scaled(f[2 * q], f[2 * q + 1], 1.0f, h[q], l[q]);
+            *reinterpret_cast<uint4*>(bz + L::p_off(L::frag_ff(L1), 0)) = uint4{h[0], h[1], h[2], h[3]};
+            *reinterpret_cast<uint4*>(bz + L::p_off(L::frag_ff(L1), 1)) = uint4{l[0], l[1], l[2], l[3]};
+          };
+          if constexpr (LMAX == 2) degree(I2{});
+          degree(I1{});
+        }
+      } else if (SX <= 1 && t0.n > 0) {
         const int j8 = lane & 7, gg = (lane >> 3) & 3, pc = lane >> 5, row = 8 * SX + j8;
         const unsigned char* gimg = smem + L::o_g;
         unsigned char* b1 = smem + L::o_b1 + (16 * gg + row) * 16 + 8 * pc;
@@ -606,13 +769,7 @@
           const unsigned char* r2 = gimg + row * L::GA_STRIDE + (LMAX == 2 ? (3 * H + (16 * pc + 4 * gg) * 5) * ES : 0);
           const unsigned char* r1 = gimg + row * L::GA_STRIDE + (16 * pc + 4 * gg) * 3 * ES;
           const unsigned char* r0 = gimg + L::GA_BYTES + row * L::GB_ROW + (16 * pc + 4 * gg) * ES;
-          if constexpr (!IO16) {
-#pragma unroll
-            for (int u = 0; u < (LMAX == 2 ? 5 : 0); ++u) { const f32x4 v = reinterpret_cast<const f32x4*>(r2)[u]; q2[4 * u] = v[0]; q2[4 * u + 1] = v[1]; q2[4 * u + 2] = v[2]; q2[4 * u + 3] = v[3]; }
-#pragma unroll
-            for (int u = 0; u < 3; ++u) { const f32x4 v = reinterpret_cast<const f32x4*>(r1)[u]; q1[4 * u] = v[0]; q1[4 * u + 1] = v[1]; q1[4 * u + 2] = v[2]; q1[4 * u + 3] = v[3]; }
-            { const f32x4 v = reinterpret_cast<const f32x4*>(r0)[0]; q0[0] = v[0]; q0[1] = v[1]; q0[2] = v[2]; q0[3] = v[3]; }
-          } else {
+          {
             auto widen = [](const uint2 v, float* o) {
               o[0] = __builtin_bit_cast(float, v.x << 16); o[1] = __builtin_bit_cast(float, v.x & 0xffff0000u);
               o[2] = __builtin_bit_cast(float, v.y << 16); o[3] = __builtin_bit_cast(float, v.y & 0xffff0000u);
@@ -739,7 +896,7 @@
         f32x4 accV[5], accG, accS;
         __builtin_amdgcn_s_setprio(WS_PRIO);
         WS_PM(5)
-        ws_tp<LMAX, TT, ROLE, false, IO16>(w, smem + L::o_b2 + lane * 16, ztr, nullptr, nullptr, nullptr, accV, accG, accS, y, tpmk);
+        ws_tp<LMAX, TT, ROLE, false, IO16>(w, smem + L::o_b2 + lane * 16, nullptr, lane, ztr, nullptr, nullptr, nullptr, accV, accG, accS, y, tpmk);
         WS_PM0
         const f32x4* nt = reinterpret_cast<const f32x4*>(n2tab) + g;
         float* orow = reinterpret_cast<float*>(smem + L::o_o) + j * L::RS;
@@ -796,7 +953,9 @@
         f32x4 accV[5], accG, accS;
         __builtin_amdgcn_s_setprio(WS_PRIO1);
         WS_PM(5)
-        ws_tp<LMAX, TT, ROLE, true, IO16>(w, smem + L::o_b1 + lane * 16, ztr, urow, wdtab + 4 * g,
+        const unsigned char* img = smem + L::o_g + (L::PRE ? (s & 1) * L::P_IMG : 0);
+        ws_tp<LMAX, TT, ROLE, true, IO16>(w, L::PRE ? img + L::p_abase(lane) : smem + L::o_b1 + lane * 16,
+                                          L::PRE ? img : nullptr, lane, ztr, urow, wdtab + 4 * g,
                                           reinterpret_cast<const f32x4*>(smem + L::o_init) + lane, accV, accG, accS, y, tpmk);
         WS_PM0
         const float dsc = y[9];
@@ -945,6 +1104,11 @@
 bool msg_ws_supported(int lmax, int hidden, int dtype) {
   return (lmax == 2 || (lmax == 1 && WS_LMAX1)) && hidden == 32 && (dtype == E3_F32 || dtype == E3_BF16);
 }
+
+int msg_ws_split_floats(int lmax, int hidden) {
+  return msg_ws_supported(lmax, hidden, E3_F32) ? (lmax + 1) * (lmax + 1) * 32 : 0;
+}
+static_assert(MsgSplit<2>::FLOATS == 9 * 32 && MsgSplit<1>::FLOATS == 4 * 32, "msg_ws_split_floats");
 
 int msg_ws_launch(int lmax, int hidden, int dtype, const void* h, int64_t ldh, int64_t N, const float* pos4, const int32_t* src,
                   const int32_t* dst, int64_t E, const void* packed, const float* in_scale, const float* premix, float* out,
@@ -993,10 +1157,12 @@
   const int64_t nchunks = (E + chunk - 1) / chunk;
   int nwg = (int)std::min<int64_t>(cus, nchunks);
   nwg = std::max(8, (nwg + 7) / 8 * 8);
-  const float* hmax = premix + (size_t)N * ud;
+  const MsgPremixLayout lay = msg_premix_layout(ud, msg_ws_split_floats(lmax, hidden), N);
+  const float* split = premix + lay.split;
+  const float* hmax = premix + lay.hmax;
   auto launch = [&](const auto& pbc) {
     WsArgsT<std::decay_t<decltype(pbc)>> a = {h, ldh, reinterpret_cast<const float4*>(pos4), src, dst, E,
-                                              static_cast<const float*>(packed), premix, hmax, in_scale, out, ldo, chunk, pbc};
+                                              static_cast<const float*>(packed), premix, split, hmax, in_scale, out, ldo, chunk, pbc};
     void* args[] = {&a};
     return hipLaunchKernel(kern, dim3(nwg), dim3(512), args, lds, stream) == hipSuccess ? E3_OK : E3_ERR_HIP;
   };
diff --git a/scalable-e3-gnn_amd/message.py b/scalable-e3-gnn_amd/message.py
--- a/scalable-e3-gnn_amd/message.py
+++ b/scalable-e3-gnn_amd/message.py
@@ -95,17 +95,28 @@
     def refresh_row_max(self, state, h: torch.Tensor, rows: torch.Tensor, in_scale: torch.Tensor | None):
         premix = state[1]
         N = h.shape[0]
-        ud = premix.numel() // N - 1
-        hmax = premix[N * ud:]
-        if rows.numel():
-            a = h[rows].float().abs()
-            m = torch.where(a < float("inf"), a, 0.0).amax(1)
-        else:
-            m = h.new_zeros(0, dtype=torch.float32)
-        if in_scale is not None and h.dtype == torch.float32:
-            m = m * in_scale[0]
-        hmax[rows] = m
-        return m.max() if m.numel() else torch.zeros((), device=h.device)
+        if N == 0 or rows.numel() == 0:
+            return torch.zeros((), device=h.device)
+        if h.stride(-1) != 1 or (h.stride(0) * h.element_size()) % 16 or h.data_ptr() % 16:
+            h = h.contiguous()
+        dev = h.device
+        rows = rows.to(device=dev, dtype=torch.int64).contiguous()
+        lib = _lib.load()
+        with torch.cuda.device(dev):
+            hd = self._plans.handle(dev)
+            sc = in_scale.data_ptr() if (in_scale is not None and h.dtype == torch.float32) else None
+            _lib.check(lib.e3_msg_refresh_rows(hd, h.data_ptr(), h.stride(0), N, rows.data_ptr(), rows.numel(), sc,
+                                               premix.data_ptr(), _lib.dtype_code(h.dtype),
+                                               torch.cuda.current_stream(dev).cuda_stream), "e3_msg_refresh_rows")
+        return self.premix_regions(dev, premix, N)[2][rows].max()
+
+    def premix_regions(self, device, premix: torch.Tensor, N: int):
+        off_s, per, off_m = ctypes.c_int64(), ctypes.c_int64(), ctypes.c_int64()
+        _lib.check(_lib.load().e3_msg_premix_regions(self._plans.handle(device), N, ctypes.byref(off_s), ctypes.byref(per),
+                                                     ctypes.byref(off_m)), "e3_msg_premix_regions")
+        table = premix[:off_s.value].view(N, -1) if N else premix[:0]
+        split = premix[off_s.value:off_m.value].view(N, per.value) if N else premix[:0]
+        return table, split, premix[off_m.value:off_m.value + N]
 
     def executed_flops_per_edge(self) -> int:
         H, L = self.hidden, self.lmax
```

Measured after the change: 11.79 million particles/s (median of 6 runs). 1.02x the previous value.
